# SolverForge/solverforge

Hardware: AMD Instinct MI355X
Metric: moves-evaluated/sec, CVRP-1000 (nearby-list selector, LateAcceptance(400)+AcceptedCount(256)) (higher is better)
Workload: dtype int64 score / int32 trial deltas (u16 matrix copy)

## Files before the change

### solverforge_amd/csrc/sf_api.hip

```cpp
#include <hip/hip_runtime.h>

#include <algorithm>
#include <chrono>
#include <cmath>
#include <cstddef>
#include <cstdio>
#include <cstdlib>
#include <cstring>
#include <map>
#include <string>
#include <vector>

#define SF_TU_MAIN 1
#include "../../include/solverforge_amd.h"
#include "sf_launch.h"
#include "sf_construct.hip"
#include "sf_clarke_wright.hip"
#include "sf_kopt_tw.hip"
#include "sf_precedence.hip"
#include "sf_scalar_construct.h"
#include "sf_mat_facts.h"
#include "sf_nbr_facts.h"

using namespace sf;

static std::string g_create_error;

struct Fact {
    int type = 0;
    void* d0 = nullptr;
    void* d1 = nullptr;
    int rows = 0, cols = 0;
    int64_t max_finite = 0;
    bool symmetric = false;
    bool all_finite = false;
    int64_t abs_sum = 0;
};
struct ConstraintSpec {
    int kind, desc, var, fact;
    int64_t param;
    int level;
    int64_t weight;
    std::vector<sf_pair_term> terms;
    std::vector<sf_uni_term> uterms;
    sf_uni_weight uweight{0, -1, -1, -1};
};
constexpr int SF_C_PAIR_JOIN_ = 100;
constexpr int SF_C_UNI_PROGRAM_ = 101;
struct UniComponent {
    size_t constraint_index;
    std::vector<int64_t> cost;
    std::vector<uint8_t> pass;
};
struct SelectorSpec {
    int kind, desc, var, max_nearby, fact;
    int min_size = 1, max_size = 3;
    int moves_per_step = 10, max_source_len = 0, skip_empty = 0;
    std::string variable_name;
    int value_limit = -1, recreate = 0;
    int64_t limit = -1;
};
struct NearbyScalarSource {
    bool present = false;
    std::vector<uint32_t> off;
    std::vector<int32_t> val;
    uint32_t* d_off = nullptr;
    int32_t* d_val = nullptr;
};
struct PrecSpec {
    bool on = false;
    int desc = 0, var = 0, hard_level = 0, mk_level = 1;
    std::vector<int32_t> dur, owner;
    std::vector<uint32_t> succ_off, succ;
    bool has_owner = false;
};
struct ClassSpec {
    int n_rows = 0;
    bool has_scalar = false;
    int var_index = 0, n_values = 0, allows_unassigned = 0;
    std::vector<int32_t> scalar_init;
    std::vector<uint32_t> value_off;
    std::vector<int32_t> value_list;
    bool has_list = false;
    std::vector<uint32_t> list_off, list_vals;
    int element_capacity = 0, element_bound = 0;
};

struct sf_ctx {
    int device = 0;
    hipStream_t stream = nullptr;
    int levels = 2, hard_levels = 1, R = 1;
    std::string err;
    std::map<int, ClassSpec> classes;
    std::map<int, Fact> facts;
    std::vector<ConstraintSpec> constraints;
    std::vector<SelectorSpec> selectors;
    bool initialized = false;
    bool has_list_model = false;
    int list_desc = -1;
    ListModel lm{};
    NearbyScalarSource nearby_scalar[2];
    int nearby_scalar_dynamic = 0;
    struct TwSpec {
        bool set = false, uploaded = false, force_walk = false, gate_ok = false;
        int desc = -1, n = 0;
        std::vector<int64_t> lo, hi, service, travel;
        int64_t departure = 0;
        int64_t *d_lo = nullptr, *d_hi = nullptr, *d_service = nullptr, *d_travel = nullptr;
        int32_t* d_ran = nullptr;
    } tw;
    PrecSpec prec;
    PrecModel pm{};
    bool prec_policy = false;
    PlfModel plf{};
    NbrIndex nbr{nullptr};
    NbrFacts nbr_facts{};
    ListModel lm_wave{};
    NbrIndex nbr_wave{nullptr};
    bool wave_renumbered = false;
    int32_t mat16_sym = 0;
    int last_wave_mode = -1;
    int32_t wave_spec_state = 0, wave_spec_reason = 0, wave_spec_key[23] = {};
    int n_cus = 0;
    int32_t last_generic_flags = -1;
    int32_t last_scalar_value_bytes = 0;
    int xown_level = -1;
    int64_t xown_weight = 0;
    std::vector<UniComponent> uni_components;
    uint16_t* d_xown_tab = nullptr;
    int64_t* d_xown_delta = nullptr;
    std::vector<std::pair<int, std::string>> providers;
    uint32_t* d_node_tab32 = nullptr;
    struct WaveFix {
        const uint16_t *perm, *inv, *mat16;
        const int32_t* demand;
        int32_t depot;
    } lm_wave_fix{};
    bool lm_small = false;
    int engine = SF_ENGINE_AUTO;
    bool has_scalar_model = false;
    int scalar_desc = -1;
    ScalarModel sm{};
    sf_solver_config cfg{SF_ACCEPT_LATE_ACCEPTANCE, 400, SF_FORAGER_ACCEPTED_COUNT, 256, 1, SF_ORDER_RANDOM, 0};
    SearchParams sp{};
    bool search_alloc = false;
    sf_annealing_config anneal{SF_ANNEAL_CALIBRATED, 0, 128, 0, {0, 0, 0, 0}, 0.999985, 1.0e-9, 0.80, 1.0, 0};
    bool anneal_seed_set = false;
    double dla_tolerance = 0.01;
    double gd_rain_speed = 0.001;
    uint64_t sc_step_count_limit = 100;
    uint64_t tabu_tenure[4] = {0, 0, 10, 0};
    int tabu_aspire = 1;
    bool tabu_configured = false;
    uint64_t* d_tabu_arena = nullptr;
    uint64_t tabu_arena_cap = 0;
    bool vnd = false;
    int vnd_n = -1;
    int64_t union_limit = -1;
    struct HoodTable {
        std::vector<int32_t> first, order;
        std::vector<int64_t> limit;
    } hoods_cfg, hoods;
    int vnd_leaves = -1;
    uint64_t* d_explicit = nullptr;
    int64_t n_explicit = 0;
    int32_t* d_trace_moves = nullptr;
    int64_t* d_trace_scores = nullptr;
    int32_t* d_trace_flags = nullptr;
    int64_t* d_trace_count = nullptr;
    int32_t* d_trace_applied = nullptr;
    int64_t trace_cap = 0;
    int64_t* d_each = nullptr;
    uint64_t* d_kopt_scratch = nullptr;
    uint64_t* d_ruin_rng = nullptr;
    uint64_t* d_sruin_rng = nullptr;
    int32_t* d_sruin_table = nullptr;
    uint32_t* d_mixed_ring = nullptr;
    uint8_t* d_mixed_ringx = nullptr;
    int32_t* d_mixed_ringd = nullptr;
    int union_order = -1;
    std::vector<int32_t> union_weights;
    int64_t* d_scores_out = nullptr;
    int32_t* d_ok = nullptr;
    std::vector<std::pair<hipEvent_t, hipEvent_t>> events;
    double prof_ms = 0;
    int64_t prof_launches = 0;
    std::vector<void*> allocs;
    void* rccl = nullptr;
};

static constexpr size_t SF_LDS_BUDGET = 160 * 1024 - 1024;

#define HIPCHK(ctx, expr)                                                                   \
    do {                                                                                    \
        hipError_t _e = (expr);                                                             \
        if (_e != hipSuccess) {                                                             \
            (ctx)->err = std::string(#expr) + ": " + hipGetErrorString(_e);                 \
            return SF_ERR_HIP;                                                              \
        }                                                                                   \
    } while (0)

struct DeviceGuard {
    int prev = -1;
    bool switched = false;
    explicit DeviceGuard(const sf_ctx* ctx) {
        if (!ctx) return;
        if (hipGetDevice(&prev) != hipSuccess) prev = -1;
        if (prev != ctx->device) switched = hipSetDevice(ctx->device) == hipSuccess;
    }
    ~DeviceGuard() {
        if (switched && prev >= 0) (void)hipSetDevice(prev);
    }
    DeviceGuard(const DeviceGuard&) = delete;
    DeviceGuard& operator=(const DeviceGuard&) = delete;
};

static int fail(sf_ctx* ctx, int code, const std::string& msg) {
    if (ctx) ctx->err = msg;
    return code;
}

template <class T>
static int dalloc(sf_ctx* ctx, T** out, size_t n) {
    void* p = nullptr;
    HIPCHK(ctx, hipMalloc(&p, n * sizeof(T) + 16));
    ctx->allocs.push_back(p);
    HIPCHK(ctx, hipMemsetAsync(p, 0, n * sizeof(T) + 16, ctx->stream));
    *out = (T*)p;
    return SF_OK;
}
template <class T>
static int upload(sf_ctx* ctx, T** out, const T* src, size_t n) {
    int rc = dalloc(ctx, out, n ? n : 1);
    if (rc) return rc;
    if (n) HIPCHK(ctx, hipMemcpyAsync(*out, src, n * sizeof(T), hipMemcpyHostToDevice, ctx->stream));
    HIPCHK(ctx, hipStreamSynchronize(ctx->stream));
    return SF_OK;
}

static int hip_rc(sf_ctx* ctx, hipError_t e) { return e == hipSuccess ? SF_OK : fail(ctx, SF_ERR_HIP, hipGetErrorString(e)); }

template <class T>
struct Scratch {
    T* p = nullptr;
    Scratch() = default;
    Scratch(const Scratch&) = delete;
    Scratch& operator=(const Scratch&) = delete;
    ~Scratch() { (void)hipFree(p); }
    int alloc(sf_ctx* ctx, size_t n) {
        return hip_rc(ctx, hipMalloc((void**)&p, (n ? n : 1) * sizeof(T)));
    }
    int upload(sf_ctx* ctx, const T* src, size_t n) {
        if (int rc = alloc(ctx, n)) return rc;
        return n ? hip_rc(ctx, hipMemcpyAsync(p, src, n * sizeof(T), hipMemcpyHostToDevice, ctx->stream)) : SF_OK;
    }
};

extern "C" {

int32_t sf_device_count(void) {
    int n = 0;
    if (hipGetDeviceCount(&n) != hipSuccess) return 0;
    return n;
}

int32_t sf_ctx_create(int32_t device_id, int32_t score_levels, int32_t hard_levels, int32_t n_replicas,
                      sf_ctx** out) {
    if (!out) return SF_ERR_INVALID;
    *out = nullptr;
    if (score_levels < 1 || score_levels > SF_MAX_LEVELS || hard_levels < 0 || hard_levels > score_levels ||
        n_replicas < 1) {
        g_create_error = "invalid score levels / replica count";
        return SF_ERR_INVALID;
    }
    int n = 0;
// ... 553 lines not shown
        for (auto& cs : ctx->constraints)
            if (cs.kind == SF_C_ROUTE_CAPACITY && cs.desc == d && ctx->facts[cs.fact].rows < m.dim) return false;
        return true;
    };
    for (auto& s : ctx->selectors)
        if ((s.kind == SF_SEL_NEARBY_LIST_CHANGE || s.kind == SF_SEL_NEARBY_LIST_SWAP) && s.desc == d) {
            if (!ctx->facts.count(s.fact) || ctx->facts[s.fact].type != 1) return fail(ctx, SF_ERR_INVALID, "nearby selector needs an i64 matrix meter");
            Fact& f = ctx->facts[s.fact];
            if (f.max_finite >= MAX_PACKED_DISTANCE) return fail(ctx, SF_ERR_UNSUPPORTED, "matrix values >= 2^40 (packed top-k keys)");
            if (m.mat && m.mat != (const int64_t*)f.d0) return fail(ctx, SF_ERR_UNSUPPORTED, "meter matrix must be the distance matrix");
            if (!m.mat) {
                m.mat = (const int64_t*)f.d0;
                m.dim = f.rows;
            }
            if (s.max_nearby < 1 || s.max_nearby > 64) return fail(ctx, SF_ERR_UNSUPPORTED, "max_nearby must be 1..64");
        }
    if (m.dim > 65535 * 16) return fail(ctx, SF_ERR_UNSUPPORTED, "node id bound too large");
    if (!demand_rows_ok()) return fail(ctx, SF_ERR_INVALID, "demand column shorter than the distance matrix (every matrix node needs a demand row)");
    const int R = ctx->R;
    int rc;
    if ((rc = dalloc(ctx, &m.visits, (size_t)R * m.n_cap))) return rc;
    if ((rc = dalloc(ctx, &m.off, (size_t)R * (m.V + 1)))) return rc;
    if ((rc = dalloc(ctx, &m.load, (size_t)R * m.V))) return rc;
    if ((rc = dalloc(ctx, &m.score, (size_t)R * 4))) return rc;
    if ((rc = dalloc(ctx, &m.best_visits, (size_t)R * m.n_cap))) return rc;
    if ((rc = dalloc(ctx, &m.best_off, (size_t)R * (m.V + 1)))) return rc;
    if ((rc = dalloc(ctx, &m.best_score, (size_t)R * 4))) return rc;
    HIPCHK(ctx, hipMemcpyAsync(m.visits, c.list_vals.data(), c.list_vals.size() * 4, hipMemcpyHostToDevice, ctx->stream));
    HIPCHK(ctx, hipMemcpyAsync(m.off, c.list_off.data(), c.list_off.size() * 4, hipMemcpyHostToDevice, ctx->stream));
    for (size_t k = 1; k < (size_t)R; k *= 2) {
        const size_t nrep = std::min(k, (size_t)R - k);
        HIPCHK(ctx, hipMemcpyAsync(m.visits + k * m.n_cap, m.visits, nrep * m.n_cap * 4, hipMemcpyDeviceToDevice, ctx->stream));
        HIPCHK(ctx, hipMemcpyAsync(m.off + k * (m.V + 1), m.off, nrep * (m.V + 1) * 4, hipMemcpyDeviceToDevice, ctx->stream));
    }
    HIPCHK(ctx, hipStreamSynchronize(ctx->stream));
    ctx->has_list_model = true;
    ctx->list_desc = d;
    ctx->pm = PrecModel{};
    if (ctx->prec.on) {
        PrecSpec& ps = ctx->prec;
        if (ps.desc != d) return fail(ctx, SF_ERR_INVALID, "list precedence: descriptor is not the list class");
        const int n = (int)ps.dur.size();
        if (c.element_bound > n) return fail(ctx, SF_ERR_INVALID, "list precedence: element ids must be < node_count");
        std::vector<char> seen((size_t)n, 0);
        for (uint32_t x : c.list_vals) {
            if (seen[x]) return fail(ctx, SF_ERR_UNSUPPORTED, "list precedence: an element appears in more than one list position");
            seen[x] = 1;
        }
        for (auto& sel : ctx->selectors)
            if (sel.kind == SF_SEL_LIST_RUIN && (m.dist_level >= 0 || m.cap_level >= 0))
                return fail(ctx, SF_ERR_UNSUPPORTED, "list ruin leaf on a precedence model with distance / capacity constraints");
        PrecModel& pm = ctx->pm;
        pm.on = 1;
        pm.hard_level = ps.hard_level;
        pm.mk_level = ps.mk_level;
        pm.n = n;
        std::vector<uint32_t> soff((size_t)n + 1, 0), sval, poff((size_t)n + 1, 0), pval;
        std::vector<int32_t> indeg((size_t)n, 0);
        int64_t invalid = 0;
        for (int i = 0; i < n; ++i) {
            for (uint32_t t = ps.succ_off[i]; t < ps.succ_off[i + 1]; ++t) {
                const uint32_t to = ps.succ[t];
                if (to < (uint32_t)n) {
                    sval.push_back(to);
                    indeg[to] += 1;
                } else
                    ++invalid;
            }
            soff[i + 1] = (uint32_t)sval.size();
        }
        pm.const_penalty = invalid;
        pm.n_edges = (int32_t)sval.size();
        {
            for (int i = 0; i < n; ++i) poff[(size_t)i + 1] = poff[(size_t)i] + (uint32_t)indeg[(size_t)i];
            pval.resize(sval.size());
            std::vector<uint32_t> fill(poff.begin(), poff.end() - 1);
            for (int i = 0; i < n; ++i)
                for (uint32_t t = soff[(size_t)i]; t < soff[(size_t)i + 1]; ++t) pval[fill[sval[t]]++] = (uint32_t)i;
        }
        int32_t* d_dur = nullptr;
        uint32_t *d_soff = nullptr, *d_sval = nullptr;
        int32_t *d_indeg = nullptr, *d_owner = nullptr;
        if ((rc = upload(ctx, &d_dur, ps.dur.data(), (size_t)n))) return rc;
        if ((rc = upload(ctx, &d_soff, soff.data(), soff.size()))) return rc;
        if ((rc = upload(ctx, &d_sval, sval.data(), sval.size()))) return rc;
        if ((rc = upload(ctx, &d_indeg, indeg.data(), (size_t)n))) return rc;
        if (ps.has_owner && (rc = upload(ctx, &d_owner, ps.owner.data(), (size_t)n))) return rc;
        pm.dur = d_dur;
        pm.succ_off = d_soff;
        pm.succ = d_sval;
        pm.indeg0 = d_indeg;
        pm.owner = ps.has_owner ? d_owner : nullptr;
        {
            if (n >= 0xFFFFFF) return fail(ctx, SF_ERR_UNSUPPORTED, "list precedence: node ids are 24 bits in the node records");
            std::vector<uint32_t> nd((size_t)n * 2);
            for (int i = 0; i < n; ++i) {
                const uint32_t dg = soff[(size_t)i + 1] - soff[(size_t)i];
                nd[(size_t)i * 2] = (uint32_t)ps.dur[(size_t)i];
                nd[(size_t)i * 2 + 1] = ((dg < 255u ? dg : 255u) << 24) | (dg ? sval[soff[(size_t)i]] : 0xFFFFFFu);
            }
            uint32_t* d_nd = nullptr;
            if ((rc = upload(ctx, &d_nd, nd.data(), nd.size()))) return rc;
            pm.nd = d_nd;
        }
        const size_t words = (size_t)R * (n ? n : 1);
        if ((rc = dalloc(ctx, &pm.earliest, words))) return rc;
        if ((rc = dalloc(ctx, &pm.indeg, words))) return rc;
        if ((rc = dalloc(ctx, &pm.queue, words))) return rc;
        if ((rc = dalloc(ctx, &pm.lsucc, words))) return rc;
        if ((rc = dalloc(ctx, &pm.state, (size_t)R * 2))) return rc;
        uint32_t *d_poff = nullptr, *d_pval = nullptr;
        if ((rc = upload(ctx, &d_poff, poff.data(), poff.size()))) return rc;
        if ((rc = upload(ctx, &d_pval, pval.data(), pval.size()))) return rc;
        pm.pred_off = d_poff;
        pm.pred = d_pval;
        if ((rc = dalloc(ctx, &pm.lpred, words))) return rc;
        if ((rc = dalloc(ctx, &pm.stamp_e, words))) return rc;
        if ((rc = dalloc(ctx, &pm.stamp_q, words))) return rc;
        if ((rc = dalloc(ctx, &pm.changed, words))) return rc;
        if ((rc = dalloc(ctx, &pm.queue2, words))) return rc;
        if ((rc = dalloc(ctx, &pm.pos, words))) return rc;
        if ((rc = dalloc(ctx, &pm.rnd, words))) return rc;
        if ((rc = dalloc(ctx, &pm.rec, words * 16))) return rc;
        if ((rc = dalloc(ctx, &pm.roff, words + (size_t)R))) return rc;
        if ((rc = dalloc(ctx, &pm.pmax, words + (size_t)R))) return rc;
        pm.has_zero_duration = 0;
        {
            int64_t dsum = 0;
            for (int32_t dv : ps.dur) {
                if (dv <= 0) pm.has_zero_duration = 1;
                dsum += dv > 0 ? dv : 0;
            }
            if (dsum >= ((int64_t)1 << 27)) pm.has_zero_duration = 1;
        }
    }
    for (auto& kv : ctx->facts)
        if (kv.second.type == 1 && kv.second.d0 == (void*)m.mat && kv.second.max_finite < 0xFFFFFFFFLL) {
            uint32_t* m32 = nullptr;
            const size_t n = (size_t)m.dim * m.dim;
            if ((rc = dalloc(ctx, &m32, n))) return rc;
            hipLaunchKernelGGL(k_mat_compress, dim3(1024), dim3(256), 0, ctx->stream, m.mat, n, m32);
            HIPCHK(ctx, hipGetLastError());
            m.mat32 = m32;
            static const bool no16 = std::getenv("SF_AMD_NO_MAT16") != nullptr;
            if (kv.second.max_finite < 0xFFFF && !no16) {
                uint16_t* m16 = nullptr;
                if ((rc = dalloc(ctx, &m16, n))) return rc;
                hipLaunchKernelGGL(k_mat_compress16, dim3(1024), dim3(256), 0, ctx->stream, m.mat, n, m16);
                HIPCHK(ctx, hipGetLastError());
                m.mat16 = m16;
            }
        }
    ctx->mat16_sym = 0;
    if (m.mat16 && (size_t)m.dim * m.dim * 2 <= ((size_t)64 << 20)) {
        std::vector<uint16_t> h16((size_t)m.dim * m.dim);
        HIPCHK(ctx, hipMemcpyAsync(h16.data(), m.mat16, h16.size() * 2, hipMemcpyDeviceToHost, ctx->stream));
        HIPCHK(ctx, hipStreamSynchronize(ctx->stream));
        ctx->mat16_sym = mat16_symmetric(h16.data(), m.dim);
    }
    for (auto& kv : ctx->facts)
        if (kv.second.type == 1 && kv.second.d0 == (void*)m.mat) {
            m.mat_symmetric = kv.second.symmetric ? 1 : 0;
            m.leg16 = (kv.second.symmetric && m.mat32 && m.dist_level >= 0 && kv.second.max_finite < 0xFFFF && m.dim <= 65535) ? 1 : 0;
            const bool no16 = std::getenv("SF_AMD_NO_LEG16") != nullptr;
            if (no16) m.leg16 = 0;
        }
    {
        const int64_t lim = (int64_t)1 << 28;
        auto mag = [](int64_t v) { return v < 0 ? (v == INT64_MIN ? INT64_MAX : -v) : v; };
        bool ok = m.mat32 != nullptr && m.dist_level >= 0;
        int64_t max_leg = 0, dem = 0;
        for (auto& kv : ctx->facts) {
            if (kv.second.type == 1 && kv.second.d0 == (void*)m.mat) {
                ok = ok && kv.second.all_finite && kv.second.max_finite < ((int64_t)1 << 26);
                max_leg = kv.second.max_finite;
            }
            if (kv.second.type == 2 && kv.second.d0 == (void*)m.demand) dem = kv.second.abs_sum;
        }
        ok = ok && mag(m.dist_weight) < lim && mag(m.dist_weight) * 8 * (max_leg + 1) < ((int64_t)1 << 29);
        if (m.cap_level >= 0)
            ok = ok && dem < lim && mag(m.capacity) < lim && mag(m.cap_weight) < lim &&
                 mag(m.cap_weight) * 2 * (dem + mag(m.capacity) + 1) < ((int64_t)1 << 29);
        {
            static const bool off = std::getenv("SF_AMD_NO_SMALL") != nullptr;
            if (off) ok = false;
        }
        ctx->lm_small = ok;
        m.small32 = ok ? 1 : 0;
    }
    bool nearby = false;
    for (auto& s : ctx->selectors)
        if ((s.kind == SF_SEL_NEARBY_LIST_CHANGE || s.kind == SF_SEL_NEARBY_LIST_SWAP) && s.desc == d) nearby = true;
    int P = 2;
    while (P < m.dim) P <<= 1;
    if (nearby && m.mat && (size_t)P * 8 <= 128 * 1024) {
        uint16_t* keys = nullptr;
        if ((rc = dalloc(ctx, &keys, (size_t)m.dim * m.dim))) return rc;
        HIPCHK(ctx, hipFuncSetAttribute((const void*)k_nbr_presort, hipFuncAttributeMaxDynamicSharedMemorySize, P * 8));
        hipLaunchKernelGGL(k_nbr_presort, dim3(m.dim), dim3(256), (size_t)P * 8, ctx->stream, m.mat, m.dim, P, keys);
        HIPCHK(ctx, hipGetLastError());
        HIPCHK(ctx, hipStreamSynchronize(ctx->stream));
        ctx->nbr = NbrIndex{keys};
        NbrFacts nf{0, 1};
        const int64_t rows_per = std::max<int64_t>(1, ((int64_t)4 << 20) / m.dim);
        std::vector<uint16_t> part((size_t)std::min<int64_t>(rows_per, m.dim) * m.dim);
        for (int64_t r0 = 0; r0 < m.dim; r0 += rows_per) {
            const int64_t n = std::min<int64_t>(rows_per, m.dim - r0);
            HIPCHK(ctx, hipMemcpyAsync(part.data(), keys + (size_t)r0 * m.dim, (size_t)n * m.dim * 2, hipMemcpyDeviceToHost, ctx->stream));
            HIPCHK(ctx, hipStreamSynchronize(ctx->stream));
            nbr_facts_rows(part.data(), n, m.dim, nf);
        }
        ctx->nbr_facts = nf;
    }
    ctx->wave_renumbered = false;
    {
        const char* env = std::getenv("SF_AMD_RENUMBER");
        const bool want = env ? std::atoi(env) != 0 : (size_t)m.dim * m.dim * 2 > (size_t)1024 * 1024;
        if (want && ctx->nbr.keys && m.mat16 && ctx->lm_small && m.dim <= 0x7FFF && m.depot >= 0 && m.depot < m.dim) {
            const int dim = m.dim;
            std::vector<uint16_t> hk((size_t)dim * dim);
            HIPCHK(ctx, hipMemcpyAsync(hk.data(), ctx->nbr.keys, hk.size() * 2, hipMemcpyDeviceToHost, ctx->stream));
            HIPCHK(ctx, hipStreamSynchronize(ctx->stream));
            std::vector<uint16_t> perm((size_t)dim), inv((size_t)dim);
            std::vector<uint8_t> seen((size_t)dim, 0);
            std::vector<int> ptr((size_t)dim, 0);
            int cur = m.depot, low = 0;
            for (int n = 0; n < dim; ++n) {
                perm[(size_t)cur] = (uint16_t)n;
                inv[(size_t)n] = (uint16_t)cur;
                seen[(size_t)cur] = 1;
                if (n + 1 == dim) break;
                int nx = -1;
                const uint16_t* row = hk.data() + (size_t)cur * dim;
                for (int& t = ptr[(size_t)cur]; t < dim; ++t) {
                    const uint32_t e = row[t];
                    if (e == 0xFFFFu) break;
                    if (!seen[e & 0x7FFFu]) {
                        nx = (int)(e & 0x7FFFu);
                        break;
                    }
                }
                if (nx < 0) {
                    while (seen[(size_t)low]) ++low;
                    nx = low;
                }
                cur = nx;
            }
            uint16_t *d_perm = nullptr, *d_inv = nullptr, *d_m16 = nullptr, *d_keys = nullptr;
            int32_t* d_dem = nullptr;
            if ((rc = upload(ctx, &d_perm, perm.data(), perm.size()))) return rc;
            if ((rc = upload(ctx, &d_inv, inv.data(), inv.size()))) return rc;
            if ((rc = dalloc(ctx, &d_m16, (size_t)dim * dim))) return rc;
            if ((rc = dalloc(ctx, &d_keys, (size_t)dim * dim))) return rc;
            hipLaunchKernelGGL(k_mat16_renumber, dim3(dim), dim3(256), 0, ctx->stream, m.mat16, d_inv, dim, d_m16);
            hipLaunchKernelGGL(k_nbr_renumber, dim3(dim), dim3(256), 0, ctx->stream, ctx->nbr.keys, d_inv, d_perm, dim, d_keys);
            if (m.demand) {
                if ((rc = dalloc(ctx, &d_dem, (size_t)dim))) return rc;
                hipLaunchKernelGGL(k_i32_renumber, dim3((dim + 255) / 256), dim3(256), 0, ctx->stream, m.demand, d_inv, dim, d_dem);
            }
            HIPCHK(ctx, hipGetLastError());
            HIPCHK(ctx, hipStreamSynchronize(ctx->stream));
            ctx->lm_wave_fix = {d_perm, d_inv, d_m16, d_dem, (int32_t)perm[(size_t)m.depot]};
            ctx->nbr_wave = NbrIndex{d_keys};
            ctx->wave_renumbered = true;
        }
    }
    return SF_OK;
}

#include "sf_wave_plan.h"
#include "sf_wave_spec.h"

static WaveShape wave_shape(const sf_ctx* ctx) {
    WaveShape s{};
    const ListModel& m = ctx->lm;
    s.nbr_index = ctx->nbr.keys != nullptr, s.V = m.V, s.n_cap = m.n_cap, s.dim = m.dim, s.max_nearby = 1;
    for (auto& sel : ctx->selectors)
        if (sel.desc == ctx->list_desc && (sel.kind == SF_SEL_NEARBY_LIST_CHANGE || sel.kind == SF_SEL_NEARBY_LIST_SWAP) && sel.max_nearby > s.max_nearby)
            s.max_nearby = sel.max_nearby;
    s.levels = ctx->levels, s.mat32 = m.mat32 != nullptr, s.mat16 = m.mat16 != nullptr, s.small = ctx->lm_small, s.dist_level = m.dist_level;
    return s;
}
static bool wave_engine_possible(sf_ctx* ctx) { return wave_engine_fits(wave_shape(ctx)); }
static bool use_wave_engine(sf_ctx* ctx) {
    if (ctx->engine == SF_ENGINE_BLOCK) return false;
    if (ctx->engine == SF_ENGINE_WAVE) return true;
    return wave_engine_default(wave_shape(ctx));
}

static int build_scalar_model(sf_ctx* ctx, int d);
static size_t scalar_table_bytes(sf_ctx* ctx);
static int launch_scalar_search(sf_ctx* ctx, SearchParams& p, int grid, bool trace);

static int alloc_search(sf_ctx* ctx) {
    if (ctx->search_alloc) return SF_OK;
    SearchParams& p = ctx->sp;
    const int R = ctx->R;
    int rc;
    int la = ctx->cfg.late_acceptance_size > 0 ? ctx->cfg.late_acceptance_size : 1;
    if ((rc = dalloc(ctx, &p.last_step_score, (size_t)R * 4))) return rc;
    if ((rc = dalloc(ctx, &p.la_hist, (size_t)R * la * 4))) return rc;
    if ((rc = dalloc(ctx, &p.la_idx, (size_t)R))) return rc;
    if ((rc = dalloc(ctx, &p.step_index, (size_t)R))) return rc;
    if ((rc = dalloc(ctx, &p.seed_draws, (size_t)R))) return rc;
    if ((rc = dalloc(ctx, &p.stats, (size_t)R * SF_STATS_WORDS))) return rc;
    if ((rc = dalloc(ctx, &p.has_best, (size_t)R))) return rc;
    if ((rc = dalloc(ctx, &ctx->d_trace_count, 1))) return rc;
    if ((rc = dalloc(ctx, &ctx->d_trace_applied, 8))) return rc;
    if ((rc = dalloc(ctx, &ctx->d_ok, 4))) return rc;
    if ((rc = dalloc(ctx, &p.sa.state, (size_t)R * SA_WORDS))) return rc;
    if ((rc = dalloc(ctx, &p.dla_best, (size_t)R * 4))) return rc;
    p.la_size = la;
    ctx->search_alloc = true;
    return SF_OK;
}

static int ensure_trace(sf_ctx* ctx, int64_t cap) {
    if (cap <= ctx->trace_cap) return SF_OK;
    int rc;
    if ((rc = dalloc(ctx, &ctx->d_trace_moves, (size_t)cap * 6))) return rc;
    if ((rc = dalloc(ctx, &ctx->d_trace_scores, (size_t)cap * 4))) return rc;
    if ((rc = dalloc(ctx, &ctx->d_trace_flags, (size_t)cap))) return rc;
    ctx->trace_cap = cap;
    return SF_OK;
}

static int search_kind(const sf_ctx* ctx) { return ctx->vnd ? (int)VND_KIND : ctx->cfg.acceptor; }

static void fill_search_params(sf_ctx* ctx, SearchParams& p) {
    p.acceptor = ctx->cfg.acceptor;
    p.dla_tolerance = ctx->dla_tolerance;
    p.forager = ctx->cfg.forager;
    p.limit = ctx->cfg.accepted_count_limit > 0 ? ctx->cfg.accepted_count_limit : 1;
    if (ctx->cfg.forager == SF_FORAGER_FIRST_LAST_STEP_SCORE_IMPROVING && ctx->cfg.accepted_count_limit <= 0) p.limit = 0;
    p.random_ties = ctx->cfg.random_ties;
    p.order = ctx->cfg.selection_order;
    if (ctx->vnd) {
        p.acceptor = VND_KIND;
        p.forager = SF_FORAGER_BEST_SCORE;
        p.limit = 1;
        p.random_ties = 0;
        p.order = SF_ORDER_ORIGINAL;
    }
    p.random_seed = ctx->cfg.random_seed;
    p.dry_run = 0;
    {
        static const bool legacy = std::getenv("SF_AMD_LEGACY_EVAL") != nullptr;
        p.legacy_eval = legacy ? 1 : 0;
    }
    p.replica_base = 0;
    p.explicit_seeds = ctx->d_explicit;
    p.n_explicit = ctx->n_explicit;
    p.trace_replica = -1;
    p.trace_moves = ctx->d_trace_moves;
    p.trace_scores = ctx->d_trace_scores;
    p.trace_flags = ctx->d_trace_flags;
    p.trace_cap = ctx->trace_cap;
    p.trace_count = ctx->d_trace_count;
    p.trace_applied = ctx->d_trace_applied;
}

static int fill_list_leaves(sf_ctx* ctx, SearchParams& p) {
    p.n_leaves = 0;
    for (int kind : {SF_SEL_NEARBY_LIST_CHANGE, SF_SEL_NEARBY_LIST_SWAP})
        for (auto& s : ctx->selectors)
            if (s.kind == kind && s.desc == ctx->list_desc) {
                if (p.n_leaves >= MAX_LEAVES) return fail(ctx, SF_ERR_UNSUPPORTED, "more than two list leaves");
                p.leaf[p.n_leaves++] = LeafSpec{s.kind, s.max_nearby, s.desc};
            }
    if (p.n_leaves == 0) return fail(ctx, SF_ERR_INVALID, "no list selector configured");
    return SF_OK;
}

static SearchLaunch make_launch(sf_ctx* ctx, const SearchParams* p, int grid, int block, size_t lds, const GLeaves* gl = nullptr) {
    return SearchLaunch{grid, block, lds, ctx->stream, &ctx->lm, &ctx->sm, gl, p, ctx->has_list_model ? 1 : 0, ctx->has_scalar_model ? 1 : 0, ctx->nbr};
}
template <int L>
static int launch_list_search_t(sf_ctx* ctx, const SearchParams& p, int grid, bool trace) {
    Carve<L> cv(ctx->lm.V, ctx->lm.n_cap, ctx->lm.dim);
    size_t lds = cv.total;
    if (lds > SF_LDS_BUDGET) return fail(ctx, SF_ERR_UNSUPPORTED, "problem does not fit the 160 KiB LDS of one CU");
    HIPCHK(ctx, launch_tu_list_block<L>(trace, make_launch(ctx, &p, grid, 1024, lds)));
    return SF_OK;
}
static int launch_list_wave(sf_ctx* ctx, const SearchParams& p, int n_replicas, bool trace) {
    WaveShape s = wave_shape(ctx);
    s.acceptor = p.acceptor, s.forager = p.forager, s.order = p.order, s.dry_run = p.dry_run, s.n_leaves = p.n_leaves;
    for (int l = 0; l < p.n_leaves && l < MAX_LEAVES; ++l) s.kind[l] = p.leaf[l].kind;
    s.n_replicas = n_replicas, s.trace = trace;
    const WavePlan pl = plan_wave_launch(s, wave_knobs());
    if (pl.err) return fail(ctx, pl.err, pl.msg);
    if (pl.nodeg && !ctx->lm.node_tab)
        if (int rc = dalloc(ctx, &ctx->lm.node_tab, (size_t)ctx->R * ctx->lm.dim)) return rc;
    SearchParams q = p;
    q.n_launch = n_replicas;
    SearchLaunch la = make_launch(ctx, &q, pl.grid, pl.block, (size_t)pl.lds);
    ctx->last_wave_mode = pl.mode;
    if (pl.compact && ctx->wave_renumbered) {
        ctx->lm_wave = ctx->lm;
        ctx->lm_wave.perm = ctx->lm_wave_fix.perm, ctx->lm_wave.inv = ctx->lm_wave_fix.inv, ctx->lm_wave.mat16 = ctx->lm_wave_fix.mat16;
        if (ctx->lm.demand) ctx->lm_wave.demand = ctx->lm_wave_fix.demand;
        ctx->lm_wave.depot = ctx->lm_wave_fix.depot;
        la.lm = &ctx->lm_wave;
        la.nb = ctx->nbr_wave;
    }
    if (!ctx->n_cus) HIPCHK(ctx, hipDeviceGetAttribute(&ctx->n_cus, hipDeviceAttributeMultiprocessorCount, ctx->device));
    const WaveSpecGate gate{pl.mode, q.move_budget != 0, (int32_t)std::min<int64_t>(std::max<int64_t>(q.n_steps, 0), INT32_MAX), n_replicas, pl.resident, ctx->n_cus, wave_spec_knob()};
    const WaveSpecKey key = wave_spec_key(pl.levels, pl.wpe, *la.lm, q, ctx->nbr_facts, ctx->mat16_sym, wave_spec_extras());
    ctx->wave_spec_state = SF_WSPEC_AOT, ctx->wave_spec_reason = wave_spec_wanted(gate);
    std::memcpy(ctx->wave_spec_key, &key, sizeof key);
    if (ctx->wave_spec_reason == SF_WSPEC_R_NONE) {
        hipFunction_t fn = nullptr;
        if ((ctx->wave_spec_reason = wave_spec_get(key, ctx->device, la.lds, &fn)) == SF_WSPEC_R_NONE) {
            WaveArgs args{*la.lm, q, la.nb};
            size_t n_args = sizeof args;
            void* cfg[] = {HIP_LAUNCH_PARAM_BUFFER_POINTER, &args, HIP_LAUNCH_PARAM_BUFFER_SIZE, &n_args, HIP_LAUNCH_PARAM_END};
            HIPCHK(ctx, hipModuleLaunchKernel(fn, (unsigned)la.grid, 1, 1, (unsigned)la.block, 1, 1, (unsigned)la.lds, la.stream, nullptr, cfg));
            ctx->wave_spec_state = SF_WSPEC_SPECIALISED;
            return SF_OK;
        }
        ctx->wave_spec_state = SF_WSPEC_FELL_BACK;
    }
    HIPCHK(ctx, pl.levels == 2 ? launch_tu_list_wave<2>(trace, pl.mode, la) : launch_tu_list_wave<4>(trace, pl.mode, la));
    return SF_OK;
}
static int launch_list_search(sf_ctx* ctx, const SearchParams& p, int grid, bool trace) {
    if (use_wave_engine(ctx)) return launch_list_wave(ctx, p, grid, trace);
    if (p.acceptor == SF_ACCEPT_DIVERSIFIED_LATE_ACCEPTANCE) return fail(ctx, SF_ERR_UNSUPPORTED, "DiversifiedLateAcceptance: wave, scalar and generic engines only");
    if (ctx->levels <= 2) return launch_list_search_t<2>(ctx, p, grid, trace);
    return launch_list_search_t<4>(ctx, p, grid, trace);
}

static int download_scores(sf_ctx* ctx, const int64_t* d_src4, int64_t* out) {
    std::vector<int64_t> tmp((size_t)ctx->R * 4);
    HIPCHK(ctx, hipMemcpyAsync(tmp.data(), d_src4, tmp.size() * 8, hipMemcpyDeviceToHost, ctx->stream));
    HIPCHK(ctx, hipStreamSynchronize(ctx->stream));
    for (int r = 0; r < ctx->R; ++r)
        for (int k = 0; k < ctx->levels; ++k) out[(size_t)r * ctx->levels + k] = tmp[(size_t)r * 4 + k];
    return SF_OK;
}

static int run_evaluate_all(sf_ctx* ctx, int64_t* out, int commit, int64_t* d_parts = nullptr) {
    int rc;
    if (!ctx->d_scores_out && (rc = dalloc(ctx, &ctx->d_scores_out, (size_t)ctx->R * 4))) return rc;
    if (!ctx->has_list_model && !ctx->has_scalar_model) return fail(ctx, SF_ERR_INVALID, "no planning variable configured");
    if (ctx->has_list_model) {
        size_t lds = ((size_t)ctx->lm.dim + 31) / 32 * 4 + 16;
        hipLaunchKernelGGL(k_list_evaluate_all, dim3(ctx->R), dim3(256), lds, ctx->stream, ctx->lm,
                           ctx->d_scores_out, commit, d_parts);
    }
    if (ctx->has_scalar_model)
        HIPCHK(ctx, launch_with_lds(k_scalar_evaluate_all, dim3(ctx->R), dim3(256), scalar_table_bytes(ctx), ctx->stream, ctx->sm, ctx->d_scores_out, commit,
                                    ctx->has_list_model ? 1 : 0, d_parts));
    if (ctx->xown_level >= 0)
        hipLaunchKernelGGL(k_cross_owner_evaluate_all, dim3(ctx->R), dim3(256), 0, ctx->stream, ctx->lm, ctx->sm.vals, ctx->sm.n, ctx->xown_level, ctx->xown_weight,
                           ctx->d_scores_out, commit, d_parts);
    if (ctx->has_list_model && ctx->pm.on)
        hipLaunchKernelGGL(k_prec_evaluate_all, dim3(ctx->R), dim3(64), 0, ctx->stream, ctx->lm, ctx->pm, ctx->d_scores_out, commit, d_parts);
    HIPCHK(ctx, hipGetLastError());
    if (out) {
        std::vector<int64_t> tmp((size_t)ctx->R * ctx->levels);
        HIPCHK(ctx, hipMemcpyAsync(tmp.data(), ctx->d_scores_out, tmp.size() * 8, hipMemcpyDeviceToHost, ctx->stream));
        HIPCHK(ctx, hipStreamSynchronize(ctx->stream));
        std::memcpy(out, tmp.data(), tmp.size() * 8);
    } else
        HIPCHK(ctx, hipStreamSynchronize(ctx->stream));
    return SF_OK;
}

static int tw_upload(sf_ctx* ctx) {
    auto& tw = ctx->tw;
    const ListModel& m = ctx->lm;
    if (!ctx->has_list_model || tw.desc != ctx->list_desc) return fail(ctx, SF_ERR_INVALID, "time windows need the list variable's class");
    if (tw.n != m.dim) return fail(ctx, SF_ERR_INVALID, "time windows: n_nodes must equal the list variable's element id bound (the matrix dimension when a matrix is attached)");
    const size_t n = (size_t)tw.n;
    for (int64_t** p : {&tw.d_lo, &tw.d_hi, &tw.d_service, &tw.d_travel}) {
        if (!*p) continue;
        auto it = std::find(ctx->allocs.begin(), ctx->allocs.end(), (void*)*p);
        if (it != ctx->allocs.end()) ctx->allocs.erase(it);
        (void)hipFree(*p);
        *p = nullptr;
    }
    tw.uploaded = false;
    int rc;
    if (!tw.d_ran && (rc = dalloc(ctx, &tw.d_ran, 1))) return rc;
    HIPCHK(ctx, hipMemsetAsync(tw.d_ran, 0, 4, ctx->stream));
    if ((rc = upload(ctx, &tw.d_lo, tw.lo.data(), n))) return rc;
    if ((rc = upload(ctx, &tw.d_hi, tw.hi.data(), n))) return rc;
    if ((rc = upload(ctx, &tw.d_service, tw.service.data(), n))) return rc;
    if ((rc = upload(ctx, &tw.d_travel, tw.travel.data(), n * n))) return rc;
    const auto mag = [](int64_t v) { return v < 0 ? -(__int128)v : (__int128)v; };
    __int128 max_t = 0, max_s = 0, max_w = 0;
    for (int64_t v : tw.travel)
        if (v >= 0 && v != UNREACHABLE && v > max_t) max_t = v;
    for (int64_t v : tw.service)
        if (v > max_s) max_s = v;
    for (size_t i = 0; i < n; ++i) max_w = std::max(max_w, std::max(mag(tw.lo[i]), mag(tw.hi[i])));
    const __int128 bound = mag(tw.departure) + ((__int128)m.n_cap + 1) * (max_t + max_s) + max_w;
    tw.gate_ok = bound < (__int128)TW_GATE;
    tw.uploaded = true;
    std::vector<int64_t>().swap(tw.lo), std::vector<int64_t>().swap(tw.hi), std::vector<int64_t>().swap(tw.service), std::vector<int64_t>().swap(tw.travel);
    return SF_OK;
}
static TwTables tw_tables(const sf_ctx* ctx) {
    const auto& tw = ctx->tw;
    return TwTables{tw.d_lo, tw.d_hi, tw.d_service, tw.d_travel, tw.departure, (tw.gate_ok && !tw.force_walk) ? 1 : 0, tw.d_ran};
}

extern "C" {

int32_t sf_initialize(sf_ctx* ctx, int64_t* out_scores) {
    DeviceGuard _dev(ctx);
    if (!ctx) return SF_ERR_INVALID;
    if (!ctx->initialized) {
        int n_list = 0, n_scalar = 0, ld = -1, sd = -1;
        for (auto& kv : ctx->classes) {
            if (kv.second.has_list) {
                ++n_list;
                ld = kv.first;
            }
            if (kv.second.has_scalar) {
                ++n_scalar;
                sd = kv.first;
            }
        }
        if (n_list + n_scalar == 0) return fail(ctx, SF_ERR_INVALID, "no planning variable configured");
        if (n_list > 1 || n_scalar > 1)
            return fail(ctx, SF_ERR_UNSUPPORTED, "at most one list class and one scalar class per context");
        int rc;
        if (n_list && (rc = build_list_model(ctx, ld))) return rc;
        if (n_scalar && (rc = build_scalar_model(ctx, sd))) return rc;
        if (n_list && n_scalar) {
            ctx->sm.score = ctx->lm.score;
            ctx->sm.best_score = ctx->lm.best_score;
        }
        for (auto& cs : ctx->constraints) {
            if (cs.kind != SF_C_CROSS_OWNER_MATCH) continue;
            if (!n_list || !n_scalar || cs.desc != sd || (int)cs.param != ld)
                return fail(ctx, SF_ERR_INVALID, "owner match: a join of the scalar class (descriptor_index) with the list class (param) of a mixed model");
            if (ctx->xown_level >= 0) return fail(ctx, SF_ERR_UNSUPPORTED, "one join of the two planning classes per context");
            if (ctx->sm.n_values != ctx->lm.V) return fail(ctx, SF_ERR_INVALID, "owner match: the scalar variable's values must be the list owner indices (n_values == owners)");
            if (ctx->lm.dim > ctx->sm.n) return fail(ctx, SF_ERR_INVALID, "owner match: the list elements must be entity ids of the scalar class");
            if (ctx->sm.n > 65534) return fail(ctx, SF_ERR_UNSUPPORTED, "owner match: more than 65534 entities");
            ctx->xown_level = cs.level;
            ctx->xown_weight = cs.weight;
            if ((rc = dalloc(ctx, &ctx->d_xown_tab, (size_t)ctx->R * ctx->sm.n))) return rc;
        }
        if (ctx->tw.set && (rc = tw_upload(ctx))) return rc;
        ctx->initialized = true;
    }
    return run_evaluate_all(ctx, out_scores, 1);
}

int32_t sf_evaluate_all(sf_ctx* ctx, int64_t* out_scores) {
    DeviceGuard _dev(ctx);
    if (!ctx || !ctx->initialized) return fail(ctx, SF_ERR_INVALID, "sf_initialize first");
    return run_evaluate_all(ctx, out_scores, 0);
}

int32_t sf_evaluate_each(sf_ctx* ctx, int32_t replica, int64_t* out_scores, int64_t* out_match_counts) {
    DeviceGuard _dev(ctx);
// ... 776 lines not shown

int32_t sf_get_stats(sf_ctx* ctx, int32_t replica, sf_stats* out) {
    DeviceGuard _dev(ctx);
    if (!ctx || !ctx->search_alloc || !out || replica < 0 || replica >= ctx->R) return fail(ctx, SF_ERR_INVALID, "bad sf_get_stats");
    static_assert(sizeof(sf_stats) == SF_STATS_WORDS * 8, "sf_stats layout");
    HIPCHK(ctx, hipMemcpyAsync(out, ctx->sp.stats + (size_t)replica * SF_STATS_WORDS, sizeof(sf_stats), hipMemcpyDeviceToHost, ctx->stream));
    HIPCHK(ctx, hipStreamSynchronize(ctx->stream));
    return SF_OK;
}

int32_t sf_get_stats_sum(sf_ctx* ctx, sf_stats* out) {
    DeviceGuard _dev(ctx);
    if (!ctx || !ctx->search_alloc || !out) return fail(ctx, SF_ERR_INVALID, "bad sf_get_stats_sum");
    std::vector<uint64_t> all((size_t)ctx->R * SF_STATS_WORDS);
    HIPCHK(ctx, hipMemcpyAsync(all.data(), ctx->sp.stats, all.size() * 8, hipMemcpyDeviceToHost, ctx->stream));
    HIPCHK(ctx, hipStreamSynchronize(ctx->stream));
    uint64_t sum[SF_STATS_WORDS] = {0};
    for (int r = 0; r < ctx->R; ++r)
        for (int k = 0; k < SF_STATS_WORDS; ++k) sum[k] += all[(size_t)r * SF_STATS_WORDS + k];
    std::memcpy(out, sum, sizeof(sf_stats));
    return SF_OK;
}

int32_t sf_get_best_scores(sf_ctx* ctx, int64_t* out) {
    DeviceGuard _dev(ctx);
    if (!ctx || !ctx->initialized || !out) return fail(ctx, SF_ERR_INVALID, "sf_initialize first");
    return download_scores(ctx, ctx->has_list_model ? ctx->lm.best_score : ctx->sm.best_score, out);
}

int32_t sf_portfolio_migrate_local(sf_ctx* ctx, int32_t n_elite, int32_t n_replace, int32_t* out_adopted) {
    DeviceGuard _dev(ctx);
    if (!ctx || !ctx->initialized) return fail(ctx, SF_ERR_INVALID, "sf_initialize first");
    if (!ctx->search_alloc) return fail(ctx, SF_ERR_INVALID, "sf_phase_start first");
    if (!ctx->has_list_model || ctx->has_scalar_model)
        return fail(ctx, SF_ERR_UNSUPPORTED, "elite migration: list-only models (the adopted state is the list class's best solution)");
    if (ctx->vnd)
        return fail(ctx, SF_ERR_UNSUPPORTED, "elite migration: not under variable neighborhood descent");
    if (ctx->cfg.acceptor != SF_ACCEPT_HILL_CLIMBING && ctx->cfg.acceptor != SF_ACCEPT_LATE_ACCEPTANCE &&
        ctx->cfg.acceptor != SF_ACCEPT_DIVERSIFIED_LATE_ACCEPTANCE)
        return fail(ctx, SF_ERR_UNSUPPORTED, "elite migration: HillClimbing / LateAcceptance / DiversifiedLateAcceptance (an annealing replica keeps a temperature schedule, a great deluge its water level, a step count its best step score, a tabu search its memories)");
    if (n_elite < 1 || n_replace < 0 || (int64_t)n_elite + n_replace > ctx->R)
        return fail(ctx, SF_ERR_INVALID, "elite migration: n_elite >= 1, n_replace >= 0, n_elite + n_replace <= replicas");
    if (out_adopted) *out_adopted = 0;
    if (n_replace == 0) return SF_OK;
    HIPCHK(ctx, hipStreamSynchronize(ctx->stream));
    std::vector<int64_t> bs((size_t)ctx->R * ctx->levels);
    if (int rc = download_scores(ctx, ctx->lm.best_score, bs.data())) return rc;
    std::vector<int32_t> order(ctx->R), src(ctx->R);
    for (int r = 0; r < ctx->R; ++r) order[r] = src[r] = r;
    const int L = ctx->levels;
    std::stable_sort(order.begin(), order.end(), [&](int32_t a, int32_t b) {
        for (int k = 0; k < L; ++k) {
            const int64_t x = bs[(size_t)a * L + k], y = bs[(size_t)b * L + k];
            if (x != y) return x > y;
        }
        return false;
    });
    int adopted = 0;
    for (int i = 0; i < n_replace; ++i) {
        const int32_t adopter = order[(size_t)ctx->R - 1 - i], elite = order[(size_t)(i % n_elite)];
        bool same = true;
        for (int k = 0; k < L; ++k) same = same && bs[(size_t)adopter * L + k] == bs[(size_t)elite * L + k];
        if (same) continue;
        src[adopter] = elite;
        adopted += 1;
    }
    if (adopted) {
        Scratch<int32_t> d_src;
        if (int rc = d_src.upload(ctx, src.data(), (size_t)ctx->R)) return rc;
        hipLaunchKernelGGL(k_list_migrate, dim3(ctx->R), dim3(256), 0, ctx->stream, ctx->lm, ctx->sp, d_src.p);
        hipError_t e = hipGetLastError();
        if (e == hipSuccess) e = hipStreamSynchronize(ctx->stream);
        if (int rc = hip_rc(ctx, e)) return rc;
    }
    if (out_adopted) *out_adopted = adopted;
    return SF_OK;
}

int32_t sf_download_list(sf_ctx* ctx, int32_t replica, int32_t d, uint32_t* out_off, uint32_t* out_vals, int32_t best) {
    DeviceGuard _dev(ctx);
    if (!ctx || !ctx->has_list_model || d != ctx->list_desc || replica < 0 || replica >= ctx->R)
        return fail(ctx, SF_ERR_INVALID, "bad sf_download_list");
    const ListModel& m = ctx->lm;
    const uint32_t* so = (best ? m.best_off : m.off) + (size_t)replica * (m.V + 1);
    const uint32_t* sv = (best ? m.best_visits : m.visits) + (size_t)replica * m.n_cap;
    HIPCHK(ctx, hipMemcpyAsync(out_off, so, (size_t)(m.V + 1) * 4, hipMemcpyDeviceToHost, ctx->stream));
    HIPCHK(ctx, hipStreamSynchronize(ctx->stream));
    uint32_t total = out_off[m.V];
    if (total) HIPCHK(ctx, hipMemcpyAsync(out_vals, sv, (size_t)total * 4, hipMemcpyDeviceToHost, ctx->stream));
    HIPCHK(ctx, hipStreamSynchronize(ctx->stream));
    return SF_OK;
}

int32_t sf_download_scalar(sf_ctx* ctx, int32_t replica, int32_t d, int32_t var, int32_t* out, int32_t best) {
    DeviceGuard _dev(ctx);
    if (!ctx || !ctx->has_scalar_model || d != ctx->scalar_desc || replica < 0 || replica >= ctx->R)
        return fail(ctx, SF_ERR_INVALID, "bad sf_download_scalar");
    (void)var;
    const ScalarModel& m = ctx->sm;
    const int32_t* src = (best ? m.best_vals : m.vals) + (size_t)replica * m.n;
    HIPCHK(ctx, hipMemcpyAsync(out, src, (size_t)m.n * 4, hipMemcpyDeviceToHost, ctx->stream));
    HIPCHK(ctx, hipStreamSynchronize(ctx->stream));
    return SF_OK;
}

}

extern "C" int32_t sf_debug_generic_plan(const int32_t* shape, int32_t n_shape, const int32_t* knobs, int32_t n_knobs, int32_t* plan, int32_t n_plan, const char** msg) {
    constexpr size_t plan_bytes = offsetof(GenericPlan, msg);
    if (!shape || !knobs || !plan || n_shape * 4 != (int)sizeof(GenericShape) || n_knobs * 4 != (int)sizeof(GenericKnobs) || n_plan * 4 != (int)plan_bytes)
        return SF_ERR_INVALID;
    GenericShape s;
    GenericKnobs k;
    std::memcpy(&s, shape, sizeof s);
    std::memcpy(&k, knobs, sizeof k);
    if (s.n_leaves < 0 || s.n_leaves > GL) return SF_ERR_INVALID;
    const GenericPlan pl = plan_generic_launch(s, k);
    std::memcpy(plan, &pl, plan_bytes);
    if (msg) *msg = pl.msg;
    return pl.err;
}
extern "C" int32_t sf_debug_wave_plan(const int32_t* shape, int32_t n_shape, const int32_t* knobs, int32_t n_knobs, int32_t* plan, int32_t n_plan, const char** msg, int32_t* fits) {
    constexpr size_t plan_bytes = offsetof(WavePlan, msg);
    if (!shape || !knobs || !plan || n_shape * 4 != (int)sizeof(WaveShape) || n_knobs * 4 != (int)sizeof(WaveKnobs) || n_plan * 4 != (int)plan_bytes)
        return SF_ERR_INVALID;
    WaveShape s;
    WaveKnobs k;
    std::memcpy(&s, shape, sizeof s);
    std::memcpy(&k, knobs, sizeof k);
    const WavePlan pl = plan_wave_launch(s, k);
    std::memcpy(plan, &pl, plan_bytes);
    if (msg) *msg = pl.msg;
    if (fits) fits[0] = wave_engine_fits(s), fits[1] = wave_engine_default(s);
    return pl.err;
}

extern "C" int32_t sf_debug_wave_spec(const sf_ctx* ctx, int32_t* out, int32_t n_out) {
    static_assert(sizeof(WaveSpecKey) == sizeof(sf_ctx::wave_spec_key), "WaveSpecKey");
    if (!out || (n_out != 4 + SF_WSPEC_KEY_WORDS_V2 && n_out != 4 + SF_WSPEC_KEY_WORDS_V1)) return SF_ERR_INVALID;
    std::memset(out, 0, (size_t)n_out * 4);
    if (ctx) out[0] = ctx->wave_spec_state, out[1] = ctx->wave_spec_reason, std::memcpy(out + 4, ctx->wave_spec_key, (size_t)(n_out - 4) * 4);
    WaveSpecCache& c = wave_spec_cache();
    std::lock_guard<std::mutex> lock(c.mu);
    out[2] = c.compiles, out[3] = (int32_t)std::ceil(c.last_ms);
    return SF_OK;
}
extern "C" int32_t sf_debug_wave_spec_legs(const sf_ctx* ctx, int32_t* out, int32_t n_out) {
    if (!ctx || !out || n_out != 2) return SF_ERR_INVALID;
    WaveSpecKey k;
    std::memcpy(&k, ctx->wave_spec_key, sizeof k);
    out[0] = k.mat_sym, out[1] = k.index_x & SF_WSPEC_X_LEG_ALL;
    return SF_OK;
}
extern "C" int32_t sf_debug_mat_sym(const int64_t* mat, int32_t dim, int32_t* out, int32_t n_out) {
    if (!mat || !out || dim < 1 || dim > 16384 || n_out != 1) return SF_ERR_INVALID;
    std::vector<uint16_t> w((size_t)dim * dim);
    for (size_t t = 0; t < w.size(); ++t) w[t] = mat16_word(mat[t]);
    out[0] = mat16_symmetric(w.data(), dim);
    return SF_OK;
}
extern "C" int32_t sf_debug_wave_spec_leg_gate(int32_t mat_sym) { return wave_spec_leg_allowed(mat_sym != 0); }
extern "C" int32_t sf_debug_late_acceptance(sf_ctx* ctx, int32_t replica, int64_t* out, int32_t n_slots, int32_t* cursor) {
    if (!ctx || !out || !cursor || !ctx->search_alloc || replica < 0 || replica >= ctx->R || n_slots != ctx->sp.la_size) return SF_ERR_INVALID;
    DeviceGuard guard(ctx);
    HIPCHK(ctx, hipStreamSynchronize(ctx->stream));
    HIPCHK(ctx, hipMemcpy(out, ctx->sp.la_hist + (size_t)replica * n_slots * 4, (size_t)n_slots * 32, hipMemcpyDeviceToHost));
    HIPCHK(ctx, hipMemcpy(cursor, ctx->sp.la_idx + replica, 4, hipMemcpyDeviceToHost));
    return SF_OK;
}
extern "C" int32_t sf_debug_wave_spec_gate(const int32_t* gate, int32_t n_gate) {
    if (!gate || n_gate * 4 != (int)sizeof(WaveSpecGate)) return SF_ERR_INVALID;
    WaveSpecGate g;
    std::memcpy(&g, gate, sizeof g);
    return wave_spec_wanted(g);
}
extern "C" int32_t sf_debug_nbr_facts(const uint16_t* keys, int32_t rows, int32_t dim, int32_t* out, int32_t n_out) {
    if (!keys || !out || rows < 1 || dim < 1 || n_out != 2) return SF_ERR_INVALID;
    NbrFacts f{0, 1};
    nbr_facts_rows(keys, rows, dim, f);
    out[0] = f.tie_max, out[1] = f.rows_full;
    return SF_OK;
}
extern "C" int32_t sf_debug_wave_spec_index_gate(const int32_t* in, int32_t n_in) {
    if (!in || n_in != 5 || in[0] < 1 || in[1] < 1 || in[2] < 0) return SF_ERR_INVALID;
    return wave_spec_index_allowed(WaveSpecIndexGate{in[0], in[1], in[2], in[3] >= 64, in[3] >= 2, in[4] != 0});
}
extern "C" int32_t sf_debug_wave_spec_compile(const int32_t* key, int32_t n_key, const char* arch, const char* out_path, char* opts, int32_t n_opts, char* log, int32_t n_log, double* ms) {
    if (!key || (n_key * 4 != (int)sizeof(WaveSpecKey) && n_key != SF_WSPEC_KEY_WORDS_V2 && n_key != SF_WSPEC_KEY_WORDS_V1) || !arch) return SF_ERR_INVALID;
    WaveSpecKey k{};
    std::memcpy(&k, key, (size_t)n_key * 4);
    if (!wave_spec_key_ok(k)) return SF_ERR_INVALID;
    const std::string csrc = wave_spec_csrc();
    auto put = [](char* dst, int32_t n, const std::string& s) {
        if (dst && n > 0) std::snprintf(dst, (size_t)n, "%s", s.c_str());
    };
    std::string o;
    for (auto& x : wave_spec_options(k, arch, csrc, wave_spec_rtc().include_dir)) o += x + "\n";
    put(opts, n_opts, o);
    if (!out_path) return SF_WSPEC_R_NONE;
    const WaveSpecBuild b = wave_spec_compile(k, arch, csrc);
    put(log, n_log, b.log);
    if (ms) *ms = b.ms;
    if (!b.reason) {
        std::ofstream f(out_path, std::ios::binary);
        f.write(b.code.data(), (std::streamsize)b.code.size());
        if (!f) return SF_ERR_INVALID;
    }
    return b.reason;
}

extern "C" int32_t sf_debug_step_arith(int32_t what, uint32_t start, uint32_t stride, uint32_t V, const uint32_t* k, int64_t n_k, uint32_t* out) {
    if (!k || !out || n_k < 0 || V < 2 || V > 1022 || (what != 0 && what != 1)) return SF_ERR_INVALID;
    const uint32_t rc = (uint32_t)(0x100000000ull / V);
    const FastMod fm = make_fastmod(V);
    for (int64_t i = 0; i < n_k; ++i)
        out[i] = what == 0 ? perm_index_recip(start, stride, k[i], V, rc) : fastmod_u64((uint64_t)start + (uint64_t)k[i] * stride, fm);
    return SF_OK;
}

#ifdef SF_PHASE_PROFILE
extern "C" int32_t sf_debug_ruin_phases(uint64_t* out8) {
    if (hipMemcpyFromSymbol(out8, HIP_SYMBOL(sf::g_rphase), 64) != hipSuccess) return SF_ERR_HIP;
    uint64_t z[8] = {0, 0, 0, 0, 0, 0, 0, 0};
    (void)hipMemcpyToSymbol(HIP_SYMBOL(sf::g_rphase), z, 64);
    return SF_OK;
}
extern "C" int32_t sf_debug_phases(uint64_t* out8) {
    if (hipMemcpyFromSymbol(out8, HIP_SYMBOL(sf::g_phase), 64) != hipSuccess) return SF_ERR_HIP;
    unsigned long long z[8] = {0};
    (void)hipMemcpyToSymbol(HIP_SYMBOL(sf::g_phase), z, 64);
    return SF_OK;
}
#endif

#include "sf_api_scalar.inc"
#include "sf_api_moves.inc"
#include "sf_api_construct.inc"
#include "sf_api_scalar_construct.inc"
#include "sf_portfolio.inc"
#include "sf_candidate_trace.inc"
#include "sf_api_anneal_debug.inc"
#include "sf_api_acceptor_debug.inc"
#include "sf_api_tabu.inc"
#include "sf_api_vnd.inc"
```

### solverforge_amd/csrc/sf_list_wave.hip

```cpp
#pragma once
#include <hip/hip_runtime.h>
#include <stdint.h>

#include <type_traits>

#include "sf_list_model.h"

namespace sf {

constexpr uint32_t RC_MAX = 128;
constexpr uint32_t RC_SMALL = 64;
constexpr uint32_t NBR_NODE_MASK = 0x7FFFu;
constexpr uint32_t NBR_SAME_FLAG = 0x8000u;
constexpr uint32_t NBR_END = 0xFFFFu;
#ifndef SF_WPB
#define SF_WPB 4
#endif
constexpr int WPB = SF_WPB;

#ifndef SF_SPEC_V
#define SF_SPEC_V(x) (x)
#endif
#ifndef SF_SPEC_DIM
#define SF_SPEC_DIM(x) (x)
#endif
#ifndef SF_SPEC_NCAP
#define SF_SPEC_NCAP(x) (x)
#endif
#ifndef SF_SPEC_K0
#define SF_SPEC_K0(x) (x)
#endif
#ifndef SF_SPEC_K1
#define SF_SPEC_K1(x) (x)
#endif
#ifndef SF_SPEC_LA_SIZE
#define SF_SPEC_LA_SIZE(x) (x)
#endif
#ifndef SF_SPEC_LIMIT
#define SF_SPEC_LIMIT(x) (x)
#endif
#ifndef SF_SPEC_HAS_PERM
#define SF_SPEC_HAS_PERM(x) (x)
#endif
#ifndef SF_SPEC_HAS_EXPLICIT
#define SF_SPEC_HAS_EXPLICIT(x) (x)
#endif
#ifdef SF_SPEC_L
#define SF_SPEC_OWN_LANE(v) asm volatile("" : "+v"(v))
#else
#define SF_SPEC_OWN_LANE(v)
#endif
#ifdef SF_SPEC_NO_WIDE
#define SF_SPEC_WIDE_TIES(x) false
#else
#define SF_SPEC_WIDE_TIES(x) (x)
#endif
#ifdef SF_SPEC_NO_TIES
#define SF_SPEC_TIES(x) 0ULL
#else
#define SF_SPEC_TIES(x) (x)
#endif
#ifdef SF_SPEC_ROWS_FULL
#define SF_SPEC_ROW_HAVE(x) true
#define SF_SPEC_ROW_HAVEMASK(x) (~0ULL)
#else
#define SF_SPEC_ROW_HAVE(x) (x)
#define SF_SPEC_ROW_HAVEMASK(x) (x)
#endif


__device__ __forceinline__ void wave_sync() {
    __builtin_amdgcn_fence(__ATOMIC_RELEASE, "wavefront");
    __builtin_amdgcn_wave_barrier();
    __builtin_amdgcn_fence(__ATOMIC_ACQUIRE, "wavefront");
}

SF_PLAIN_KERNEL
__global__ __launch_bounds__(256) void k_nbr_presort(const int64_t* __restrict__ mat, int dim, int P,
                                                     uint16_t* __restrict__ keys) {
    extern __shared__ __attribute__((aligned(16))) unsigned char smem[];
    uint64_t* sk = (uint64_t*)smem;
    const int row = blockIdx.x;
    const int64_t* rp = mat + (size_t)row * dim;
    for (int t = threadIdx.x; t < P; t += blockDim.x) {
        uint64_t k = ~0ULL;
        if (t < dim) {
            const int64_t v = rp[t];
            if (v >= 0 && v != UNREACHABLE) k = ((uint64_t)v << 24) | (uint64_t)(uint32_t)t;
        }
        sk[t] = k;
    }
    __syncthreads();
    for (int size = 2; size <= P; size <<= 1)
        for (int stride = size >> 1; stride > 0; stride >>= 1) {
            for (int t = threadIdx.x; t < (P >> 1); t += blockDim.x) {
                const int lo = (t / stride) * 2 * stride + (t % stride);
                const int hi = lo + stride;
                const bool up = (lo & size) == 0;
                const uint64_t a = sk[lo], b = sk[hi];
                if ((a > b) == up) {
                    sk[lo] = b;
                    sk[hi] = a;
                }
            }
            __syncthreads();
        }
    for (int t = threadIdx.x; t < dim; t += blockDim.x) {
        const uint64_t k = sk[t];
        uint32_t e = NBR_END;
        if (k != ~0ULL) {
            e = (uint32_t)k & NBR_NODE_MASK;
            if (t > 0 && (sk[t - 1] >> 24) == (k >> 24)) e |= NBR_SAME_FLAG;
        }
        keys[(size_t)row * dim + t] = (uint16_t)e;
    }
}

struct WCarve {
    size_t load, off, node, ring, visits, rtab, routeat, total;
    uint32_t rc;
    __host__ __device__ WCarve(int V, int n_cap, int dim, int max_k, bool compact = false, bool node_global = false) {
        rc = max_k <= 32 ? RC_SMALL : RC_MAX;
        size_t o = 0;
        load = o;
        o = align_up(o + (compact ? sizeof(int32_t) : sizeof(int64_t)) * V, 16);
        off = o;
        o = align_up(o + (node_global ? sizeof(uint16_t) : sizeof(uint32_t)) * (V + 1), 16);
        node = o;
        o = align_up(o + (node_global ? 0 : (compact ? sizeof(uint16_t) : sizeof(uint32_t)) * dim), 16);
        ring = o;
        o = align_up(o + sizeof(uint32_t) * 2 * rc * MAX_LEAVES, 16);
        visits = o;
        o = align_up(o + sizeof(uint16_t) * n_cap, 16);
        rtab = o;
        o = align_up(o + (node_global ? 0 : sizeof(uint32_t) * V * MAX_LEAVES), 16);
        routeat = o;
        o = align_up(o + (compact ? 0 : sizeof(uint16_t) * V * MAX_LEAVES), 16);
        total = o;
    }
};

template <bool COMPACT>
struct NodeSlotT;
template <>
struct NodeSlotT<false> {
    uint32_t* p;
    __device__ __forceinline__ NodeSlotT(unsigned char* base, int, const uint16_t*, const void*, bool = false) : p((uint32_t*)base) {}
    __device__ __forceinline__ void clear(uint32_t node) const { p[node] = NODE_NONE; }
    __device__ __forceinline__ void set(uint32_t node, uint32_t route, uint32_t pos) const { p[node] = (route << 16) | pos; }
    __device__ __forceinline__ uint32_t get(uint32_t node) const { return p[node]; }
    __device__ __forceinline__ uint32_t word(uint32_t node) const { return p[node]; }
    __device__ __forceinline__ uint32_t wide(uint32_t s, uint32_t) const { return s; }
    __device__ __forceinline__ uint32_t wide_short(uint32_t s) const { return s; }
};
template <>
struct NodeSlotT<true> {
    uint16_t* p;
    const uint16_t* visits;
    const void* off;
    bool off16;
    uint32_t pb, pmax;
    __device__ __forceinline__ uint32_t off_at(uint32_t i) const { return off16 ? (uint32_t)((const uint16_t*)off)[i] : ((const uint32_t*)off)[i]; }
    __device__ __forceinline__ NodeSlotT(unsigned char* base, int V, const uint16_t* visits_, const void* off_, bool off16_ = false)
        : p((uint16_t*)base), visits(visits_), off(off_), off16(off16_) {
        uint32_t rb = 1;
        while ((1u << rb) - 1u < (uint32_t)V) ++rb;
        pb = 16u - rb;
        pmax = (1u << pb) - 1u;
    }
    __device__ __forceinline__ void clear(uint32_t node) const { p[node] = 0xFFFFu; }
    __device__ __forceinline__ void set(uint32_t node, uint32_t route, uint32_t pos) const {
        p[node] = (uint16_t)((route << pb) | (pos < pmax ? pos : pmax));
    }
    __device__ __forceinline__ uint32_t get(uint32_t node) const { return wide(p[node], node); }
    __device__ __forceinline__ uint32_t word(uint32_t node) const { return p[node]; }
    __device__ __forceinline__ uint32_t wide(uint32_t s, uint32_t node) const {
        const bool none = s == 0xFFFFu;
        const uint32_t route = s >> pb;
        uint32_t pos = s & pmax;
        if (__ballot(!none && pos == pmax) != 0ull) {
            if (!none && pos == pmax) {
                const uint32_t o = off_at(route), len = off_at(route + 1) - o;
                while (pos + 1 < len && (uint32_t)visits[o + pos] != node) ++pos;
            }
        }
        return none ? NODE_NONE : ((route << 16) | pos);
    }
    __device__ __forceinline__ uint32_t wide_short(uint32_t s) const {
        const uint32_t w = ((s >> pb) << 16) | (s & pmax);
        return s == 0xFFFFu ? NODE_NONE : w;
    }
};
__host__ __device__ inline bool node_slot_compact_ok(int V) { return V >= 1 && V <= 1022; }

struct NearbyItem {
    uint32_t w;
    uint32_t ord;
    uint32_t pay0;
    uint32_t pay1;
};

__device__ __forceinline__ NearbyItem nearby_item(bool is_change, uint32_t slot, uint32_t se, uint32_t sp,
                                                  uint32_t len, uint32_t k, const uint32_t* s_off,
                                                  const uint16_t* sb, const uint16_t* ro) {
    const bool some = slot != NODE_NONE;
    const uint32_t r2 = some ? slot >> 16 : 0u, dp = slot & 0xFFFFu;
    const uint32_t len2 = s_off[r2 + 1] - s_off[r2];
    const uint32_t rk = ro[r2];
    const uint32_t inter_ord = ORD_INTER_BASE + (uint32_t)sb[rk] + dp;
    const bool intra = r2 == se;
    const uint32_t end_pay = (r2 << 16) | len2;
    NearbyItem it;
    if (is_change) {
        const bool v0 = !intra || (dp != sp && dp != sp + 1);
        const bool v1 = dp + 1 == len2 && (!intra || len != sp + 1);
        it.w = some ? (uint32_t)v0 + (uint32_t)v1 : 0u;
        it.ord = intra ? (v0 ? dp : len) : inter_ord;
        it.pay0 = v0 ? slot : end_pay;
        it.pay1 = end_pay;
    } else {
        const bool v = intra ? dp > sp : rk > k;
        it.w = (some && v) ? 1u : 0u;
        it.ord = intra ? dp : inter_ord;
        it.pay0 = slot;
        it.pay1 = 0;
    }
    return it;
}

struct RouteTab {
    const uint32_t* rt;
    static constexpr int KEY_SHIFT = 24;
    __device__ __forceinline__ uint32_t word(uint32_t route) const { return rt[route]; }
    __device__ __forceinline__ static uint32_t rank(uint32_t w) { return w & 0xFFFFu; }
    __device__ __forceinline__ static uint32_t inter_ord(uint32_t w, uint32_t dp) { return ORD_INTER_BASE + (w >> 16) + dp; }
};
#ifdef SF_SPEC_TIE_KEY
static_assert(SF_SPEC_RB >= 1 && SF_SPEC_PB >= 1 && SF_SPEC_RB + SF_SPEC_PB <= 22, "SF_SPEC_TIE_KEY: the packed word does not fit 32 bits");
constexpr uint32_t ORD_ARITH_BASE = 1u << (SF_SPEC_RB + SF_SPEC_PB);
constexpr int ORD_ARITH_SHIFT = SF_SPEC_PB;
#else
constexpr uint32_t ORD_ARITH_BASE = 1u << 26;
constexpr int ORD_ARITH_SHIFT = 16;
#endif
struct RouteArith {
    uint32_t st, inv, V, recip;
    static constexpr int KEY_SHIFT = 28;
    __device__ __forceinline__ uint32_t word(uint32_t route) const {
        uint32_t x = route + V - st;
        x = x >= V ? x - V : x;
        const uint32_t y = x * inv;
        uint32_t rk = y - __umulhi(y, recip) * V;
        return rk >= V ? rk - V : rk;
    }
    __device__ __forceinline__ static uint32_t rank(uint32_t w) { return w; }
    __device__ __forceinline__ static uint32_t inter_ord(uint32_t w, uint32_t dp) { return ORD_ARITH_BASE + (w << ORD_ARITH_SHIFT) + dp; }
};
struct RouteRank {
    const uint32_t* rt;
    static constexpr int KEY_SHIFT = RouteArith::KEY_SHIFT;
    __device__ __forceinline__ uint32_t word(uint32_t route) const { return rt[route]; }
    __device__ __forceinline__ static uint32_t rank(uint32_t w) { return w; }
    __device__ __forceinline__ static uint32_t inter_ord(uint32_t w, uint32_t dp) { return RouteArith::inter_ord(w, dp); }
};
template <class OT, class RT>
__device__ __forceinline__ NearbyItem nearby_item_rt(bool is_change, uint32_t slot, uint32_t se, uint32_t sp,
                                                     uint32_t len, uint32_t k, const OT* s_off, const RT& rt) {
    const bool some = slot != NODE_NONE;
    const uint32_t r2 = some ? slot >> 16 : 0u, dp = slot & 0xFFFFu;
    const uint32_t len2 = s_off[r2 + 1] - s_off[r2];
    const uint32_t t = rt.word(r2);
    const uint32_t rk = RT::rank(t);
    const uint32_t inter_ord = RT::inter_ord(t, dp);
    const bool intra = r2 == se;
    const uint32_t end_pay = (r2 << 16) | len2;
    NearbyItem it;
    if (is_change) {
        const bool v0 = !intra || (dp != sp && dp != sp + 1);
        const bool v1 = dp + 1 == len2 && (!intra || len != sp + 1);
        it.w = some ? (uint32_t)v0 + (uint32_t)v1 : 0u;
        it.ord = intra ? (v0 ? dp : len) : inter_ord;
        it.pay0 = v0 ? slot : end_pay;
        it.pay1 = end_pay;
    } else {
        const bool v = intra ? dp > sp : rk > k;
        it.w = (some && v) ? 1u : 0u;
        it.ord = intra ? dp : inter_ord;
        it.pay0 = slot;
        it.pay1 = 0;
    }
    return it;
}

__device__ __forceinline__ uint32_t mbcnt64(uint64_t mask) {
    return __builtin_amdgcn_mbcnt_hi((uint32_t)(mask >> 32), __builtin_amdgcn_mbcnt_lo((uint32_t)mask, 0u));
}
#ifdef SF_SPEC_TIE_KEY
__device__ __forceinline__ int32_t tie_key_fix(uint64_t startmask, uint64_t nonstart, uint32_t ord, uint32_t wc) {
    const uint32_t q = (mbcnt64(startmask >> 1) << (SF_SPEC_RB + SF_SPEC_PB + 3)) | (ord << 2) | wc;
    uint32_t q_dn = q, q_up = q;
    int32_t fix = 0;
    uint64_t run = nonstart;
    for (uint32_t d = 1; run != 0; ++d) {
        q_dn = (uint32_t)__builtin_amdgcn_update_dpp(0, (int)q_dn, 0x130, 0xf, 0xf, true);
        q_up = (uint32_t)__builtin_amdgcn_update_dpp(0, (int)q_up, 0x138, 0xf, 0xf, true);
        fix += q_dn < q ? (int32_t)(q_dn & 3u) : 0;
        fix -= q_up > q ? (int32_t)(q_up & 3u) : 0;
        run &= nonstart << d;
    }
    return fix;
}
#endif

template <class LT, class OT, bool OWN_LANE = false>
__device__ __forceinline__ void apply_list_move_wave(const ListModel& m, uint16_t* visits, OT* off,
                                                     LT* load, int kind, uint32_t a, uint32_t i, uint32_t b,
                                                     uint32_t j, uint32_t ext = 0) {
    uint32_t lane = threadIdx.x & 63u;
    if constexpr (OWN_LANE) asm volatile("" : "+v"(lane));
    if (kind == 2) {
        const uint32_t P = off[a] + i, Q = off[b] + j;
        const uint32_t x = visits[P];
        wave_sync();
        if (P < Q) {
            for (uint32_t t0 = P; t0 < Q; t0 += 64) {
                const uint32_t t = t0 + lane;
                uint32_t nv = 0;
                if (t < Q) nv = (t + 1 < Q) ? (uint32_t)visits[t + 1] : x;
                wave_sync();
                if (t < Q) visits[t] = (uint16_t)nv;
                wave_sync();
            }
        } else if (P > Q) {
            for (uint32_t c0 = 0; c0 <= P - Q; c0 += 64) {
                const uint32_t dd = c0 + lane;
                const bool in = dd <= P - Q;
                const uint32_t t = P - (in ? dd : 0u);
                uint32_t nv = 0;
                if (in) nv = t > Q ? (uint32_t)visits[t - 1] : x;
                wave_sync();
                if (in) visits[t] = (uint16_t)nv;
                wave_sync();
            }
        }
        if (a != b) {
            for (uint32_t rr = lane; rr <= (uint32_t)SF_SPEC_V(m.V); rr += 64) {
                if (a < b && rr > a && rr <= b) off[rr] -= 1;
                if (a > b && rr > b && rr <= a) off[rr] += 1;
            }
            if (lane == 0 && m.demand) {
                const int64_t dx = (int64_t)m.demand[x];
                load[a] = (LT)wsub(load[a], dx);
                load[b] = (LT)wadd(load[b], dx);
            }
        }
    } else if (kind == 6) {
        const uint32_t za = ext & 0xFFFFu, zb = ext >> 16;
        const uint32_t PA = off[a] + i, PB = off[b] + j;
        const bool a_first = PA < PB;
        const uint32_t PX = a_first ? PA : PB, zx = a_first ? za : zb, PY = a_first ? PB : PA, zy = a_first ? zb : za;
        const uint32_t ox = a_first ? a : b, oy = a_first ? b : a;
        int64_t da = 0, db = 0;
        if (a != b && m.demand) {
            for (uint32_t t = 0; t < za; ++t) da = wadd(da, (int64_t)m.demand[visits[PA + t]]);
            for (uint32_t t = 0; t < zb; ++t) db = wadd(db, (int64_t)m.demand[visits[PB + t]]);
        }
        wave_sync();
        relocate_flat_segment(visits, PY, zy, PX, lane, 64u, [] { wave_sync(); });
        relocate_flat_segment(visits, PX + zy, zx, PY + zy, lane, 64u, [] { wave_sync(); });
        if (a != b) {
            for (uint32_t rr = lane; rr <= (uint32_t)SF_SPEC_V(m.V); rr += 64)
                if (rr > ox && rr <= oy) off[rr] = off[rr] + zy - zx;
            if (lane == 0 && m.demand) {
                load[a] = (LT)wadd(wsub(load[a], da), db);
                load[b] = (LT)wadd(wsub(load[b], db), da);
            }
        }
    } else if (kind == 5) {
        const uint32_t z = ext - i, P = off[a] + i;
        const uint32_t Q = a != b ? off[b] + j : (j <= i ? off[a] + j : off[a] + j + z);
        int64_t dsum = 0;
        if (a != b && m.demand)
            for (uint32_t t = 0; t < z; ++t) dsum = wadd(dsum, (int64_t)m.demand[visits[P + t]]);
        wave_sync();
        relocate_flat_segment(visits, P, z, Q, lane, 64u, [] { wave_sync(); });
        if (a != b) {
            for (uint32_t rr = lane; rr <= (uint32_t)SF_SPEC_V(m.V); rr += 64) {
                if (a < b && rr > a && rr <= b) off[rr] -= z;
                if (a > b && rr > b && rr <= a) off[rr] += z;
            }
            if (lane == 0 && m.demand) {
                load[a] = (LT)wsub(load[a], dsum);
                load[b] = (LT)wadd(load[b], dsum);
            }
        }
    } else if (kind == 4) {
        const uint32_t lo = off[a] + i, hi = off[a] + j;
        for (uint32_t t = lane; t < (hi - lo) / 2; t += 64) {
            const uint16_t x = visits[lo + t], y = visits[hi - 1 - t];
            visits[lo + t] = y;
            visits[hi - 1 - t] = x;
        }
    } else if (kind == 9) {
        const uint32_t base = off[a] + i, size = j - i;
        const uint32_t perm = nth_permutation_nibbles(size, ext);
        uint32_t nv = 0;
        if (lane < size) nv = visits[base + ((perm >> (4u * lane)) & 15u)];
        wave_sync();
        if (lane < size) visits[base + lane] = (uint16_t)nv;
    } else if (kind == 7) {
        const uint32_t base = off[a], c1 = i, c2 = b, c3 = j;
        const uint32_t mask = kopt_reverse_mask(ext);
        const bool rb = (mask >> 1) & 1u, rc = (mask >> 2) & 1u;
        auto reverse_range = [&](uint32_t lo, uint32_t hi) {
            for (uint32_t t = lane; t < (hi - lo) / 2; t += 64) {
                const uint16_t x = visits[base + lo + t], y = visits[base + hi - 1 - t];
                visits[base + lo + t] = y;
                visits[base + hi - 1 - t] = x;
            }
            wave_sync();
        };
        if (!kopt_swaps_segments(ext)) {
            if (rb) reverse_range(c1, c2);
            if (rc) reverse_range(c2, c3);
        } else {
            const uint32_t zc = c3 - c2;
            reverse_range(c1, c3);
            if (!rc) reverse_range(c1, c1 + zc);
            if (!rb) reverse_range(c1 + zc, c3);
        }
    } else if (kind == 3) {
        if (lane == 0) {
            const uint32_t pa = off[a] + i, pb = off[b] + j;
            const uint16_t x = visits[pa], y = visits[pb];
            visits[pa] = y;
            visits[pb] = x;
            if (a != b && m.demand) {
                const int64_t dx = (int64_t)m.demand[x], dy = (int64_t)m.demand[y];
                load[a] = (LT)wadd(wsub(load[a], dx), dy);
                load[b] = (LT)wadd(wsub(load[b], dy), dx);
            }
        }
    }
    wave_sync();
}

__device__ __forceinline__ uint32_t nearby_source_to_ring(const ListModel& m, const NbrIndex& nb, bool is_change, uint32_t se,
                                                          uint32_t sp, uint32_t len, uint32_t k, uint32_t sx,
                                                          const uint32_t* node_slot, const uint32_t* s_off, const uint16_t* sb,
                                                          const uint16_t* ro, uint32_t* rq, uint32_t RCM, uint32_t tl,
                                                          uint32_t key, uint32_t base, uint32_t need, uint32_t emitted) {
    const uint32_t lane = threadIdx.x & 63u;
    const uint64_t lanebit = 1ULL << lane;
    const uint32_t dim = (uint32_t)m.dim;
    const uint16_t* rowk = nb.keys + (size_t)sx * dim;
    const uint32_t mv0 = (se << 16) | sp;
    for (;;) {
        const bool have = key != NBR_END;
        const uint64_t havemask = __ballot(have);
        if (havemask == 0) break;
        NearbyItem it{0u, 0u, 0u, 0u};
        if (have) it = nearby_item(is_change, node_slot[key & NBR_NODE_MASK], se, sp, len, k, s_off, sb, ro);
        const uint64_t startmask = __ballot(have && (lane == 0 || !(key & NBR_SAME_FLAG)));
        const bool more = havemask == ~0ULL && base + 64 < dim;
        const uint32_t fo = 63u - (uint32_t)__clzll((unsigned long long)startmask);
        if (more && fo == 0) {
            TopK tk{~0ULL, 0u, ~0ULL};
            for (uint32_t b2 = base; b2 < dim; b2 += 64) {
                const uint32_t j2 = b2 + lane;
                const uint32_t ky = j2 < dim ? (uint32_t)rowk[j2] : NBR_END;
                NearbyItem i2{0u, 0u, 0u, 0u};
                uint64_t hk = 0;
                if (ky != NBR_END) {
                    const uint32_t y2 = ky & NBR_NODE_MASK;
                    i2 = nearby_item(is_change, node_slot[y2], se, sp, len, k, s_off, sb, ro);
                    hk = (uint64_t)m.mat[(size_t)sx * dim + y2] << 24;
                }
                if (!__ballot(ky != NBR_END)) break;
                topk_offer(tk, need, i2.w >= 1 ? (hk | i2.ord) : ~0ULL, i2.pay0);
                topk_offer(tk, need, i2.w == 2 ? (hk | (i2.ord + 1)) : ~0ULL, i2.pay1);
            }
            const uint32_t cnt = (uint32_t)__popcll(__ballot(lane < need && tk.key != ~0ULL));
            if (lane < cnt) {
                const uint32_t qi = (tl + emitted + lane) & RCM;
                rq[qi * 2] = mv0;
                rq[qi * 2 + 1] = tk.pay;
            }
            emitted += cnt;
            break;
        }
        const uint32_t nclosed = more ? fo : (uint32_t)__popcll(havemask);
        const uint64_t closedmask = nclosed >= 64 ? ~0ULL : ((1ULL << nclosed) - 1ULL);
        const bool closed = (closedmask & lanebit) != 0;
        const uint32_t wc = closed ? it.w : 0u;
        const uint64_t w1 = __ballot(wc == 1), w2 = __ballot(wc == 2);
        const uint32_t Wc = (uint32_t)__popcll(w1) + 2u * (uint32_t)__popcll(w2);
        if (Wc > 0) {
            int32_t pos = (int32_t)(mbcnt64(w1) + 2u * mbcnt64(w2));
            const uint64_t nonstart = ~startmask & closedmask;
            if (nonstart) {
                const uint32_t packed = (it.ord << 2) | wc;
                uint64_t run = nonstart;
                for (uint32_t d = 1; run != 0; ++d) {
                    const uint32_t p_dn = __shfl_down(packed, d), p_up = __shfl_up(packed, d);
                    const bool same_up = (run & lanebit) != 0;
                    const bool same_dn = ((run >> d) & lanebit) != 0;
                    if (same_dn && (p_dn >> 2) < it.ord) pos += (int32_t)(p_dn & 3u);
                    if (same_up && (p_up >> 2) > it.ord) pos -= (int32_t)(p_up & 3u);
                    run &= nonstart << d;
                }
            }
            if (wc >= 1 && (uint32_t)pos < need) {
                const uint32_t qi = (tl + emitted + (uint32_t)pos) & RCM;
                rq[qi * 2] = mv0;
                rq[qi * 2 + 1] = it.pay0;
            }
            if (wc == 2 && (uint32_t)pos + 1 < need) {
                const uint32_t qi = (tl + emitted + (uint32_t)pos + 1) & RCM;
                rq[qi * 2] = mv0;
                rq[qi * 2 + 1] = it.pay1;
            }
            const uint32_t ne = Wc < need ? Wc : need;
            emitted += ne;
            need -= ne;
        }
        if (need == 0 || !more) break;
        base += nclosed;
        const uint32_t jj = base + lane;
        key = jj < dim ? (uint32_t)rowk[jj] : NBR_END;
    }
    return emitted;
}

#ifndef SF_WAVE_SYM
#define SF_WAVE_SYM 1
#endif

#if defined(SF_PHASE_PROFILE) || defined(SF_GEN_COUNT)
#ifdef SF_GEN_COUNT
#define SF_PHASE_WORDS 10
#else
#define SF_PHASE_WORDS 8
#endif
__device__ unsigned long long g_phase[SF_PHASE_WORDS];
#endif
#ifdef SF_ISA_MARK
#define ISA_MARK(name) asm volatile("; SF_MARK " name)
#else
#define ISA_MARK(name)
#endif
#if defined(SF_PHASE_PROFILE) && !defined(SF_PHASE_PGRP)
#define PH_DECL uint64_t ph_t = clock64(), ph_acc[8] = {0, 0, 0, 0, 0, 0, 0, 0};
#define PH(i)                          \
    {                                  \
        const uint64_t _t = clock64(); \
        ph_acc[i] += _t - ph_t;        \
        ph_t = _t;                     \
    }
#define PH_DUMP \
    if (lane == 0) for (int _k = 0; _k < 8; ++_k) atomicAdd(&g_phase[_k], (unsigned long long)ph_acc[_k]);
#elif defined(SF_GEN_COUNT)
#define PH_DECL uint64_t ph_acc[SF_PHASE_WORDS] = {0, 0, 0, 0, 0, 0, 0, 0, 0, 0};
#define PH(i)
#define GC(i) ph_acc[i] += 1;
#define PH_DUMP \
    if (lane == 0) for (int _k = 0; _k < SF_PHASE_WORDS; ++_k) atomicAdd(&g_phase[_k], (unsigned long long)ph_acc[_k]);
#else
#define PH_DECL
#define PH(i)
#define PH_DUMP
#endif
#ifndef GC
#define GC(i)
#endif

__device__ __forceinline__ int32_t wave_max_i32(int32_t v) {
    const int lo = (int)0x80000000;
    v = max(v, __builtin_amdgcn_update_dpp(lo, v, 0x111, 0xf, 0xf, false));
    v = max(v, __builtin_amdgcn_update_dpp(lo, v, 0x112, 0xf, 0xf, false));
    v = max(v, __builtin_amdgcn_update_dpp(lo, v, 0x114, 0xf, 0xf, false));
    v = max(v, __builtin_amdgcn_update_dpp(lo, v, 0x118, 0xf, 0xf, false));
    v = max(v, __builtin_amdgcn_update_dpp(lo, v, 0x142, 0xa, 0xf, false));
    v = max(v, __builtin_amdgcn_update_dpp(lo, v, 0x143, 0xc, 0xf, false));
    return __builtin_amdgcn_readlane(v, 63);
}
template <int L>
__device__ __forceinline__ bool small_ge(const int32_t (&a)[L], const int32_t (&b)[L]) {
    bool ge = true;
#pragma unroll
    for (int k = L - 1; k >= 0; --k) ge = a[k] > b[k] || (a[k] == b[k] && ge);
    return ge;
}
template <int L>
__device__ __forceinline__ bool small_ge0(const int32_t (&a)[L]) {
    bool ge = true;
#pragma unroll
    for (int k = L - 1; k >= 0; --k) ge = a[k] > 0 || (a[k] == 0 && ge);
    return ge;
}
__device__ __forceinline__ int32_t clamp_i64_to_i32(int64_t v) {
    return v > 0x7FFFFFFFll ? 0x7FFFFFFF : v < -0x7FFFFFFFll - 1 ? (int32_t)0x80000000 : (int32_t)v;
}

template <int L, class LT, bool M16 = false, class OT = uint32_t>
__device__ __forceinline__ bool eval_list_move_small(const ListModel& m, const uint16_t* visits, const OT* off, const LT* load,
                                                     bool chg, uint32_t a, uint32_t i, uint32_t b, uint32_t j, int32_t (&dv)[L]) {
    const uint32_t oa = off[a], la = off[a + 1] - oa;
    const uint32_t ob = off[b], lb = off[b + 1] - ob;
    const bool intra = a == b;
    bool ok = i < la && (chg ? j <= lb : j < lb) && !(intra && (j == i || (chg && j == i + 1)));
    const bool flip = !chg && intra && i > j;
    const uint32_t i2 = ok ? (flip ? j : i) : 0u, j2 = ok ? (flip ? i : j) : 0u;
    const uint32_t la_ = ok ? la : 0u, lb_ = ok ? lb : 0u;
    const uint32_t depot = (uint32_t)m.depot;
    const uint32_t P = oa + i2, Q = ob + j2;
    const bool has_pa = i2 > 0, has_na = i2 + 1 < la_, has_q = j2 < lb_, has_pb = j2 > 0, has_nb = j2 + 1 < lb_;
    const uint32_t r_x = visits[P];
    const uint32_t x = ok ? r_x : depot;
    const uint32_t r_pa = visits[has_pa ? P - 1 : P], r_na = visits[has_na ? P + 1 : P];
    const uint32_t r_q = visits[has_q ? Q : P], r_pb = visits[has_pb ? Q - 1 : P], r_nb = visits[has_nb ? Q + 1 : P];
    const uint32_t pa = has_pa ? r_pa : depot, na = has_na ? r_na : depot;
    const uint32_t vq = has_q ? r_q : depot;
    const uint32_t pb = has_pb ? r_pb : depot, nb = has_nb ? r_nb : depot;
    ok = ok && (chg || x != vq);
    const bool adj = !chg && intra && j2 == i2 + 1;
    const bool ca = chg || adj;
    const bool src_single = la == 1, dst_empty = !intra && lb == 0;
    const uint32_t dim4 = (uint32_t)SF_SPEC_DIM(m.dim) * (M16 ? 2u : 4u);
    auto leg = [&](uint32_t f, uint32_t t) -> uint32_t {
        const uint32_t byte_off = f * dim4 + t * (M16 ? 2u : 4u);
        if (M16) return *(const uint16_t*)((const char*)m.mat16 + byte_off);
        return *(const uint32_t*)((const char*)m.mat32 + byte_off);
    };
    const uint32_t p0 = leg(pa, chg ? na : vq);
    const uint32_t p1 = leg(chg ? pb : vq, ca ? x : na);
    const uint32_t p2 = leg(ca ? x : pb, chg ? vq : (adj ? nb : x));
    const uint32_t p3 = leg(x, nb);
    const uint32_t m0 = leg(pa, x);
    const uint32_t m1 = leg(x, adj ? vq : na);
    const uint32_t m3 = leg(vq, nb);
    const uint32_t m2 = leg(adj ? vq : pb, adj ? nb : vq);
    int32_t d_cap = 0;
    if (m.cap_level >= 0) {
        const int32_t dx = m.demand[x];
        const int32_t dyq = m.demand[vq];
        const int32_t dy = chg ? 0 : dyq;
        const int32_t cap = (int32_t)m.capacity;
        const int32_t la0 = (int32_t)load[a], lb0 = (int32_t)load[b];
        const int32_t la1 = la0 - dx + dy, lb1 = lb0 - dy + dx;
        d_cap = max(la1 - cap, 0) + max(lb1 - cap, 0) - max(la0 - cap, 0) - max(lb0 - cap, 0);
        d_cap = intra ? 0 : d_cap;
    }
    const uint32_t plus = ((chg && src_single) ? 0u : p0) + p1 + p2 + (ca ? 0u : p3);
    const uint32_t minus = m0 + m1 + ((chg && dst_empty) ? 0u : m2) + (ca ? 0u : m3);
    const int32_t d_dist = (int32_t)(plus - minus);
    const int32_t cw = (int32_t)m.cap_weight, dw = (int32_t)m.dist_weight;
#pragma unroll
    for (int k = 0; k < L; ++k) {
        int32_t v = 0;
        if (k == m.cap_level) v -= cw * d_cap;
        if (k == m.dist_level) v -= dw * d_dist;
        dv[k] = ok ? v : 0;
    }
    return ok;
}

template <int L>
struct LevelWords {
    uint32_t wc[L], wd[L];
    uint32_t has_cap;
    int32_t cap, cw, dw;
    uint32_t depot;
};
template <int L, bool USED, bool KW>
__device__ __forceinline__ LevelWords<L> level_words(const ListModel& m) {
    LevelWords<L> w;
    w.cap = w.cw = w.dw = 0;
    w.depot = 0;
#ifdef SF_SPEC_MODEL_WORDS
    w.cap = SF_SPEC_CAPACITY, w.cw = SF_SPEC_CAP_WEIGHT, w.dw = SF_SPEC_DIST_WEIGHT, w.depot = SF_SPEC_DEPOT;
#pragma unroll
    for (int k = 0; k < L; ++k) w.wc[k] = k == SF_SPEC_CAP_LEVEL ? 0xFFFFFFFFu : 0u, w.wd[k] = k == SF_SPEC_DIST_LEVEL ? 0xFFFFFFFFu : 0u;
    w.has_cap = SF_SPEC_CAP_LEVEL >= 0 ? 1u : 0u;
    return w;
#endif
    if constexpr (KW) {
        auto word = [](uint32_t v) -> uint32_t {
            asm volatile("" : "+v"(v));
            return uni(v);
        };
        w.cap = (int32_t)word((uint32_t)m.capacity);
        w.cw = (int32_t)word((uint32_t)m.cap_weight);
        w.dw = (int32_t)word((uint32_t)m.dist_weight);
        w.depot = word((uint32_t)m.depot);
    }
#pragma unroll
    for (int k = 0; k < L; ++k) {
        w.wc[k] = uni(k == m.cap_level ? 0xFFFFFFFFu : 0u);
        w.wd[k] = uni(k == m.dist_level ? 0xFFFFFFFFu : 0u);
        if constexpr (USED) {
            asm volatile("" : "+s"(w.wc[k]));
            asm volatile("" : "+s"(w.wd[k]));
        }
    }
    w.has_cap = uni(m.cap_level >= 0 ? 1u : 0u);
    if constexpr (USED) asm volatile("" : "+s"(w.has_cap));
    return w;
}
template <int L, class LT, bool M16 = false, class OT = uint32_t, bool KW = false>
__device__ __forceinline__ void eval_generated_small(const ListModel& m, const LevelWords<L>& lw, const uint16_t* visits, const OT* off, const LT* load, uint32_t c,
                                                     uint32_t a, uint32_t i, uint32_t b, uint32_t j, int32_t (&dv)[L]) {
    const uint32_t oa = off[a], la = off[a + 1] - oa;
    const uint32_t ob = off[b], lb = off[b + 1] - ob;
    const uint32_t depot = KW ? lw.depot : (uint32_t)m.depot;
    const uint32_t P = oa + i, Q = ob + j;
    const uint32_t h_pa = min(i, 1u), h_na = min(la - 1u - i, 1u);
    const uint32_t h_q = min(lb - j, 1u), h_pb = min(j, 1u);
    const uint32_t h_nb = min(max(lb, j + 1u) - (j + 1u), 1u);
    const uint32_t x = visits[P];
    const uint32_t r_pa = visits[P - h_pa], r_na = visits[P + h_na];
    const uint32_t r_q = visits[Q - (1u - h_q)], r_pb = visits[Q - h_pb], r_nb = visits[Q + h_nb];
    const uint32_t pa = h_pa ? r_pa : depot, na = h_na ? r_na : depot;
    const uint32_t vq = h_q ? r_q : depot;
    const uint32_t pb = h_pb ? r_pb : depot, nb = h_nb ? r_nb : depot;
    const bool chg = c != 0;
    const bool intra = a == b;
    const bool adj = !chg && intra && j == i + 1;
    const bool ca = chg || adj;
    const uint32_t dim4 = (uint32_t)SF_SPEC_DIM(m.dim) * (M16 ? 2u : 4u);
    auto leg = [&](uint32_t f, uint32_t t) -> uint32_t {
        const uint32_t byte_off = __umul24(f, dim4) + t * (M16 ? 2u : 4u);
        if (M16) return *(const uint16_t*)((const char*)m.mat16 + byte_off);
        return *(const uint32_t*)((const char*)m.mat32 + byte_off);
    };
    const uint32_t p0 = leg(pa, chg ? na : vq);
#ifdef SF_SPEC_SYM_ROWS
    const uint32_t p1 = leg(ca ? x : na, chg ? pb : vq);
    const uint32_t p2 = leg(x, chg ? vq : (adj ? nb : pb));
#else
    const uint32_t p1 = leg(chg ? pb : vq, ca ? x : na);
    const uint32_t p2 = leg(ca ? x : pb, chg ? vq : (adj ? nb : x));
#endif
#ifdef SF_SPEC_LEG_REAIM
    const uint32_t o_m1 = __umul24(x, dim4) + (adj ? vq : na) * (M16 ? 2u : 4u);
    auto leg_at = [&](uint32_t byte_off) -> uint32_t {
        if (M16) return *(const uint16_t*)((const char*)m.mat16 + byte_off);
        return *(const uint32_t*)((const char*)m.mat32 + byte_off);
    };
    const uint32_t p3 = leg_at(ca ? o_m1 : __umul24(x, dim4) + nb * (M16 ? 2u : 4u));
    const uint32_t m0 = leg(pa, x);
    const uint32_t m1 = leg_at(o_m1);
    const uint32_t m3 = leg_at(ca ? o_m1 : __umul24(vq, dim4) + nb * (M16 ? 2u : 4u));
#else
    const uint32_t p3 = leg(x, nb);
    const uint32_t m0 = leg(pa, x);
    const uint32_t m1 = leg(x, adj ? vq : na);
    const uint32_t m3 = leg(vq, nb);
#endif
    const uint32_t m2 = leg(adj ? vq : pb, adj ? nb : vq);
    int32_t d_cap = 0;
    if (lw.has_cap != 0u) {
        const int32_t dx = m.demand[x];
#ifdef SF_SPEC_LEG_REAIM
        const int32_t dyq = m.demand[(chg || intra) ? x : vq];
#else
        const int32_t dyq = m.demand[vq];
#endif
        const int32_t dy = chg ? 0 : dyq;
        const int32_t cap = KW ? lw.cap : (int32_t)m.capacity;
        const int32_t la0 = (int32_t)load[a] - cap, lb0 = (int32_t)load[b] - cap;
        const int32_t sh = dx - dy;
        d_cap = max(la0 - sh, 0) + max(lb0 + sh, 0) - max(la0, 0) - max(lb0, 0);
        d_cap = intra ? 0 : d_cap;
    }
    const uint32_t plus = ((chg && la == 1) ? 0u : p0) + p1 + p2 + (ca ? 0u : p3);
    const uint32_t minus = m0 + m1 + ((chg && !intra && lb == 0) ? 0u : m2) + (ca ? 0u : m3);
    const int32_t d_dist = (int32_t)(plus - minus);
    const int32_t tc = -((KW ? lw.cw : (int32_t)m.cap_weight) * d_cap), td = -((KW ? lw.dw : (int32_t)m.dist_weight) * d_dist);
#pragma unroll
    for (int k = 0; k < L; ++k) dv[k] = (int32_t)(((uint32_t)tc & lw.wc[k]) + ((uint32_t)td & lw.wd[k]));
}

struct LeafCursor {
    uint32_t head, tail;
    uint32_t left;
    uint32_t k, o;
    uint32_t se, len, sp, sx;
    uint32_t vk, vbase;
    int ex;
    uint32_t pk;
    uint32_t pv;
    uint32_t cend;
};

struct WaveArgs {
    ListModel m;
    SearchParams p;
    NbrIndex nb;
};
typedef const __attribute__((address_space(4))) WaveArgs* ColdArgs;
__device__ __forceinline__ ColdArgs cold_args() {
    uint64_t u = (uint64_t)__builtin_amdgcn_kernarg_segment_ptr();
    asm volatile("" : "+s"(u));
    return (ColdArgs)u;
}

#ifndef SF_WAVES_PER_EU
#define SF_WAVES_PER_EU 4
#endif
template <int L, bool TRACE, int MODE, bool COMPACT = false, int WPE = SF_WAVES_PER_EU, bool NODEG = false>
__global__ __launch_bounds__(64 * WPB, WPE) void k_list_search_wave(ListModel m, SearchParams p, NbrIndex nb) {
    constexpr bool FAST = MODE >= 1, SMALL = MODE == 2;
    constexpr bool LEAN = FAST && SMALL;
    constexpr bool SAT = LEAN && COMPACT, RANKTAB = LEAN && COMPACT && !NODEG;
    constexpr bool RBATCH = LEAN && !NODEG;
#define SF_COLD_P(f) (SMALL ? cold_args()->p.f : p.f)
#define SF_COLD_M(f) (SMALL ? cold_args()->m.f : m.f)
    static_assert(!COMPACT || SMALL, "COMPACT stores loads in 32 bits: MODE 2 only");
    static_assert(!NODEG || COMPACT, "NODEG: the 16-bit table of the COMPACT layout");
    using LT = typename std::conditional<COMPACT, int32_t, int64_t>::type;
    using OT = typename std::conditional<NODEG, uint16_t, uint32_t>::type;
    extern __shared__ __attribute__((aligned(16))) unsigned char smem[];
    const uint32_t lane = threadIdx.x & 63u;
    const uint32_t wave_in_group = uni(threadIdx.x >> 6);
    const int rr = (int)(blockIdx.x * (blockDim.x >> 6) + wave_in_group);
    if (rr >= p.n_launch) return;
    const int r = rr + p.replica_base;
    const int V = SF_SPEC_V(m.V);
    const uint32_t dim = (uint32_t)SF_SPEC_DIM(m.dim);

    const int n_leaves = FAST ? 2 : p.n_leaves;
    const uint32_t K0 = (uint32_t)SF_SPEC_K0(p.leaf[0].max_nearby), K1 = n_leaves > 1 ? (uint32_t)SF_SPEC_K1(p.leaf[1].max_nearby) : 1u;
    const bool chg0 = FAST ? true : p.leaf[0].kind == 16, chg1 = FAST ? false : (n_leaves > 1 && p.leaf[1].kind == 16);
    const int acceptor = FAST ? 1 : p.acceptor, forager = FAST ? 0 : p.forager;
    const bool dry_run = FAST ? false : p.dry_run != 0;
    __shared__ uint64_t s_sa[FAST ? 1 : WPB][FAST ? 1 : SA_WORDS];
    uint64_t* saw = s_sa[FAST ? 0 : wave_in_group];
    const bool annealing = !FAST && acceptor == 3;
    if constexpr (!FAST)
        if (annealing) sa_load(saw, p.sa, r, lane);
    const int32_t desc0_w = p.leaf[0].descriptor, desc1_w = n_leaves > 1 ? p.leaf[1].descriptor : 0;
    const uint64_t desc0_q = SMALL ? 0 : (uint64_t)p.leaf[0].descriptor, desc1_q = (!SMALL && n_leaves > 1) ? (uint64_t)p.leaf[1].descriptor : 0;
    auto desc0 = [&]() -> uint64_t { return SMALL ? (uint64_t)(int64_t)desc0_w : desc0_q; };
    auto desc1 = [&]() -> uint64_t { return SMALL ? (uint64_t)(int64_t)desc1_w : desc1_q; };

    const WCarve cv(V, SF_SPEC_NCAP(m.n_cap), (int)dim, (int)(K0 > K1 ? K0 : K1), COMPACT, NODEG);
    const uint32_t RCM = cv.rc - 1;
    unsigned char* mem = smem + (size_t)wave_in_group * cv.total;
    LT* s_load = (LT*)(mem + cv.load);
    OT* s_off = (OT*)(mem + cv.off);
    uint32_t* ring = (uint32_t*)(mem + cv.ring);
    uint16_t* s_visits = (uint16_t*)(mem + cv.visits);
    const NodeSlotT<COMPACT> node_slot(NODEG ? (unsigned char*)(m.node_tab + (size_t)r * dim) : mem + cv.node, V, s_visits, (const void*)s_off, NODEG);
    auto node_sync = [&]() {
        if constexpr (NODEG) {
            __builtin_amdgcn_fence(__ATOMIC_RELEASE, "workgroup");
            __builtin_amdgcn_wave_barrier();
            __builtin_amdgcn_fence(__ATOMIC_ACQUIRE, "workgroup");
        } else {
            wave_sync();
        }
    };
    constexpr bool ARANK = NODEG;
    using RT = typename std::conditional<ARANK, RouteArith, typename std::conditional<RANKTAB, RouteRank, RouteTab>::type>::type;
    uint32_t* rtab = (uint32_t*)(mem + cv.rtab);
    uint16_t* route_at = (uint16_t*)(mem + cv.routeat);

    uint32_t* g_visits = m.visits + (size_t)r * SF_SPEC_NCAP(m.n_cap);
    uint32_t* g_off = m.off + (size_t)r * (V + 1);
    int64_t* g_load = m.load + (size_t)r * V;
    int64_t* g_score = m.score + (size_t)r * 4;
    const bool tracing = TRACE && r == p.trace_replica;

    for (uint32_t t = lane; t <= (uint32_t)V; t += 64) s_off[t] = (OT)g_off[t];
    for (uint32_t t = lane; t < (uint32_t)V; t += 64) s_load[t] = (LT)g_load[t];
    for (uint32_t t = lane; t < dim; t += 64) node_slot.clear(t);
    node_sync();
    const uint32_t total0 = uni(s_off[V]);
    if (COMPACT && SF_SPEC_HAS_PERM(m.perm != nullptr)) {
        for (uint32_t t = lane; t < total0; t += 64) s_visits[t] = m.perm[g_visits[t]];
    } else {
        for (uint32_t t = lane; t < total0; t += 64) s_visits[t] = (uint16_t)g_visits[t];
    }
    wave_sync();
    for (uint32_t v = lane; v < (uint32_t)V; v += 64) {
        const uint32_t o = s_off[v], len = s_off[v + 1] - o;
        for (uint32_t q = 0; q < len; ++q) node_slot.set(s_visits[o + q], v, q);
    }
    node_sync();

    uint32_t nsat = 0;
    if constexpr (SAT) {
        for (uint32_t base = 0; base < (uint32_t)V; base += 64) {
            const uint32_t v = base + lane;
            const bool lg = v < (uint32_t)V && (uint32_t)(s_off[v + 1] - s_off[v]) > node_slot.pmax;
            nsat += (uint32_t)__popcll(__ballot(lg));
        }
    }
    auto ext_id = [&](uint32_t x) -> uint32_t { return (COMPACT && SF_SPEC_HAS_PERM(m.inv != nullptr)) ? (uint32_t)m.inv[x] : x; };
    int64_t cur[L], best_sol[L];
#pragma unroll
    for (int k = 0; k < L; ++k) {
        cur[k] = (int64_t)uni64((uint64_t)g_score[k]);
        best_sol[k] = (int64_t)uni64((uint64_t)m.best_score[(size_t)r * 4 + k]);
    }
    uint32_t st_steps = 0, st_gen = 0, st_acc = 0, st_applied = 0, st_calc = 0, st_scored = 0, st_sources = 0;
    uint64_t steps_run = 0;
    auto flush_stats = [&]() {
        if (lane == 0) {
            uint64_t* gs = SF_COLD_P(stats) + (size_t)r * SF_STATS_WORDS;
            gs[0] += st_steps;
            gs[1] += st_gen;
            gs[2] += st_gen;
            gs[3] += st_acc;
            gs[4] += st_applied;
            gs[5] += st_calc;
            gs[6] += st_gen - st_calc;
            gs[7] += st_scored;
            gs[8] += st_sources;
        }
        if constexpr (!SMALL) steps_run += st_steps;
        st_steps = st_gen = st_acc = st_applied = st_calc = st_scored = st_sources = 0;
    };
    uint64_t trace_n = 0;
    const uint64_t step_index0 = dry_run ? 0 : p.step_index[r];
    const uint64_t seed_draws0 = dry_run ? 0 : p.seed_draws[r];
    const int la_idx0 = dry_run ? 0 : p.la_idx[r];
    int la_cursor = la_idx0;
    const uint64_t lanebit = 1ULL << lane;
    uint32_t hm = 0;
    if constexpr (LEAN) {
        hm = (uint32_t)((int32_t)(lane << 26) >> 31);
        asm volatile("" : "+v"(hm));
    }
    auto half = [&](uint32_t lo, uint32_t up) -> uint32_t { return (lo & ~hm) | (up & hm); };
    PH_DECL

    const LevelWords<L> lvl = level_words<L, SMALL, RBATCH>(m);
    bool best_pending = false;
    const FastMod fm_V = make_fastmod(V > 0 ? (uint32_t)V : 1u);
    const FastMod fm_V1 = make_fastmod(V > 1 ? (uint32_t)V - 1u : 1u);
    const uint32_t v_recip32 = V > 1 ? (uint32_t)(0x100000000ull / (uint32_t)V) : 0u;
    const bool use_cm = V >= 2 && V <= 128;
    const uint64_t cm_lo = use_cm ? __ballot(lane >= 1 && lane < (uint32_t)V && gcd_u32(lane, (uint32_t)V) == 1) : 0ull;
    const uint64_t cm_hi = use_cm ? __ballot(lane + 64 < (uint32_t)V && gcd_u32(lane + 64, (uint32_t)V) == 1) : 0ull;
    int64_t step = 0;
    for (; step < SF_COLD_P(n_steps); ++step) {
        PH(7)
        ISA_MARK("prologue_begin");
        uint64_t sidx, sseed;
        if (dry_run) {
            sidx = p.dry_step_index;
            sseed = p.dry_step_seed;
        } else {
            sidx = step_index0 + (uint64_t)step;
            const uint64_t draw = seed_draws0 + (uint64_t)step;
            const uint64_t* const explicit_seeds = SF_COLD_P(explicit_seeds);
            const int64_t n_explicit = SF_COLD_P(n_explicit);
            if (SF_SPEC_HAS_EXPLICIT(explicit_seeds != nullptr) && (int64_t)draw < n_explicit)
                sseed = explicit_seeds[(size_t)r * n_explicit + draw];
            else
                sseed = step_seed(SF_COLD_P(random_seed) + (uint64_t)r, draw);
        }
        sidx = uni64(sidx);
        sseed = uni64(sseed);
        const StreamCtx ctx{sidx, sseed, FAST ? 3 : p.order};
        ScoreV<L> late;
#pragma unroll
        for (int k = 0; k < L; ++k) late.v[k] = 0;
        const int la_slot = la_cursor;
        if (acceptor == 1 || acceptor == 4) {
            const int64_t* const lh = SF_COLD_P(la_hist) + ((size_t)r * SF_SPEC_LA_SIZE(SF_COLD_P(la_size)) + la_slot) * 4;
#pragma unroll
            for (int k = 0; k < L; ++k) late.v[k] = (int64_t)uni64((uint64_t)lh[k]);
        }
        ScoreV<L> dla_thr = late;
        if (acceptor == 4) {
            ScoreV<L> db;
#pragma unroll
            for (int k = 0; k < L; ++k) db.v[k] = (int64_t)uni64((uint64_t)p.dla_best[(size_t)r * 4 + k]);
            dla_thr = dla_threshold<L>(db, p.dla_tolerance);
        }
        [[maybe_unused]] bool thr_on = true;
        if constexpr (TRACE)
            if (acceptor == 5 || acceptor == 6) ax_step_begin<L>(acceptor, p.sa.state + (size_t)r * SA_WORDS, late, thr_on);
        [[maybe_unused]] TabuStep<L> tabu;
        [[maybe_unused]] const TabuScope tabu_scope{0u, 0u, 0u};
        if constexpr (TRACE)
            if (acceptor == 7) tabu_step_begin<L>(p.sa.state + (size_t)r * SA_WORDS, tabu);
        int has_best = 0;
        typename std::conditional<SMALL, uint32_t, uint64_t>::type equal_count = 0;
        uint32_t accepted = 0, pulls = 0;
        ScoreV<L> best;
#pragma unroll
        for (int k = 0; k < L; ++k) best.v[k] = 0;
        uint32_t best_m0 = 0, best_m1 = 0;
        int best_leaf = 0;
        uint64_t best_ti = 0;
        int32_t late_d[L], best_d[L];
#pragma unroll
        for (int k = 0; k < L; ++k) {
            late_d[k] = SMALL ? clamp_i64_to_i32(wsub(late.v[k], cur[k])) : 0;
            best_d[k] = 0;
        }
        int64_t acc_thr = 0, best_key = 0;
        if constexpr (SMALL && L == 2) {
            const int64_t lh = late_d[0] < -(1 << 30) ? -(int64_t)(1 << 30) : (int64_t)late_d[0];
            const int64_t late_key = lh * 4294967296ll + (int64_t)late_d[1];
            acc_thr = late_key < 0 ? late_key : 0;
        }
        const uint32_t total = uni(s_off[V]);
        uint32_t hashed = 0;
        const bool lane_hash = FAST && use_cm;
        if (lane_hash) {
            const uint64_t es0 = SALT_NEARBY_CHANGE_ENTITY ^ desc0(), es1 = SALT_NEARBY_SWAP_ENTITY ^ desc1();
            if constexpr (RBATCH && SF_WAVE_SYM != 0) {
                uint32_t hl = lane;
                asm volatile("" : "+v"(hl));
                const uint64_t salt = hl == 0 ? SALT_UNION_OFFSET : hl == 1 ? es0 : hl == 2 ? (es0 ^ STRIDE_SALT_MIX) : hl == 3 ? es1 : (es1 ^ STRIDE_SALT_MIX);
                const FastMod fm2 = make_fastmod(2u);
                FastMod f;
                f.M = hl == 0 ? fm2.M : ((hl & 1u) ? fm_V.M : fm_V1.M);
                f.n = hl == 0 ? fm2.n : ((hl & 1u) ? fm_V.n : fm_V1.n);
                hashed = fastmod_u64(ctx.mixed_seed(salt), f);
            } else {
                const uint64_t salt = lane == 0 ? SALT_UNION_OFFSET : lane == 1 ? es0 : lane == 2 ? (es0 ^ STRIDE_SALT_MIX) : lane == 3 ? es1 : (es1 ^ STRIDE_SALT_MIX);
                const FastMod fm2 = make_fastmod(2u);
                FastMod f;
                f.M = lane == 0 ? fm2.M : ((lane & 1u) ? fm_V.M : fm_V1.M);
                f.n = lane == 0 ? fm2.n : ((lane & 1u) ? fm_V.n : fm_V1.n);
                hashed = fastmod_u64(ctx.mixed_seed(salt), f);
            }
        }
        const uint32_t first_leaf = lane_hash ? (uint32_t)__builtin_amdgcn_readlane((int)hashed, 0)
                                              : (n_leaves > 1 ? ctx.random_index((uint32_t)n_leaves, SALT_UNION_OFFSET) : 0u);

        uint32_t perm_st0 = 0, perm_sd0 = 1, perm_st1 = 0, perm_sd1 = 1;
        uint32_t perm_inv0 = 0, perm_inv1 = 0;
        auto route_facts = [&](int l) -> RT {
            if constexpr (ARANK)
                return RouteArith{l ? perm_st1 : perm_st0, l ? perm_inv1 : perm_inv0, (uint32_t)V, v_recip32};
            else
                return RT{rtab + l * V};
        };
        auto resolve = [&](LeafCursor& c, int l) {
            const uint16_t* ra = route_at + l * V;
            uint32_t k = c.k, o = c.o, se = c.se, len = c.len;
            if (o >= c.cend) {
            ISA_MARK("resolve_slow_begin");
            if (k != c.vk || o >= len) {
                for (;;) {
                    if constexpr (COMPACT) {
                        const uint32_t xx = (l ? perm_st1 : perm_st0) + k * (l ? perm_sd1 : perm_sd0);
                        uint32_t rr_ = xx - __umulhi(xx, v_recip32) * (uint32_t)V;
                        rr_ = rr_ >= (uint32_t)V ? rr_ - (uint32_t)V : rr_;
                        se = uni(rr_);
                    } else
                        se = uni((uint32_t)ra[k]);
                    len = uni(s_off[se + 1] - s_off[se]);
                    if (o < len) break;
                    ++k;
                    o = 0;
                }
            }
            if (k != c.vk || (o & ~63u) != c.vbase) {
                const uint64_t src_salt = ((l ? chg1 : chg0) ? SALT_NEARBY_CHANGE_SOURCE : SALT_NEARBY_SWAP_SOURCE) ^
                                          (uint64_t)se ^ (l ? desc1() : desc0());
                const uint32_t oo = (o & ~63u) + lane;
                const uint32_t spl = oo < len ? ctx.selection_index(oo, len, src_salt) : 0u;
                const uint32_t sxl = oo < len ? (uint32_t)s_visits[s_off[se] + spl] : 0u;
                c.pv = spl | (sxl << 16);
                c.vk = k;
                c.vbase = o & ~63u;
            }
            c.cend = len < (o & ~63u) + 64u ? len : (o & ~63u) + 64u;
            c.k = k;
            c.se = se;
            c.len = len;
            ISA_MARK("resolve_slow_end");
            }
            const uint32_t pvv = (uint32_t)__builtin_amdgcn_readlane((int)c.pv, (int)(o & 63u));
            const uint32_t sp = pvv & 0xFFFFu, sx = pvv >> 16;
            c.o = o;
            c.sp = sp;
            c.sx = sx;
            const uint32_t ent = l ? ((lane + 32u) & 63u) : lane;
            const uint32_t entc = ent < dim ? ent : dim - 1u;
            const uint32_t pk_any = (uint32_t) * (const uint16_t*)((const char*)nb.keys + ((sx * dim + entc) << 1));
            if constexpr (LEAN)
                c.pk = pk_any;
            else
                c.pk = ent < dim ? pk_any : NBR_END;
        };
        auto row_key = [&](uint32_t raw, uint32_t e) -> uint32_t { return LEAN ? (e < dim ? raw : NBR_END) : raw; };

        PH(0)
        LeafCursor C0{0, 0, total, 0, 0, 0, 0, 0, 0, 0xFFFFFFFFu, 0, 0, NBR_END, 0, 0};
        LeafCursor C1{0, 0, n_leaves > 1 ? total : 0u, 0, 0, 0, 0, 0, 0, 0xFFFFFFFFu, 0, n_leaves > 1 ? 0 : 1, NBR_END, 0, 0};
        for (int l = 0; l < n_leaves; ++l) {
            const uint64_t ent_salt = ((l ? chg1 : chg0) ? SALT_NEARBY_CHANGE_ENTITY : SALT_NEARBY_SWAP_ENTITY) ^ (l ? desc1() : desc0());
            uint32_t pst, psd;
            if (lane_hash) {
                pst = (uint32_t)__builtin_amdgcn_readlane((int)hashed, l ? 3 : 1);
                psd = StreamCtx::first_coprime_from((uint32_t)__builtin_amdgcn_readlane((int)hashed, l ? 4 : 2) + 1u, cm_lo, cm_hi);
            } else if (use_cm)
                ctx.perm_params_fm(fm_V, fm_V1, ent_salt, pst, psd, cm_lo, cm_hi);
            else
                ctx.perm_params((uint32_t)V, ent_salt, pst, psd);
            pst = uni(pst);
            psd = uni(psd);
            if (l)
                perm_st1 = pst, perm_sd1 = psd;
            else
                perm_st0 = pst, perm_sd0 = psd;
            if constexpr (ARANK) {
                uint32_t inv = 0;
                for (uint32_t base = 0; base < (uint32_t)V; base += 64) {
                    const uint32_t c = base + lane;
                    const uint32_t xx = psd * c;
                    uint32_t rm = xx - __umulhi(xx, v_recip32) * (uint32_t)V;
                    rm = rm >= (uint32_t)V ? rm - (uint32_t)V : rm;
                    const uint64_t hit = __ballot(c < (uint32_t)V && rm == 1u);
                    if (hit) {
                        inv = base + (uint32_t)__ffsll((unsigned long long)hit) - 1u;
                        break;
                    }
                }
                if (l)
                    perm_inv1 = inv;
                else
                    perm_inv0 = inv;
                continue;
            }
            uint16_t* ra = route_at + l * V;
            uint32_t* rt = rtab + l * V;
            [[maybe_unused]] uint32_t carry = 0;
            for (uint32_t base = 0; base < (uint32_t)V; base += 64) {
                const uint32_t k = base + lane;
                if constexpr (RANKTAB) {
                    if (k < (uint32_t)V) rt[perm_index_recip(pst, psd, k, (uint32_t)V, v_recip32)] = k;
                } else {
                    uint32_t v = 0, e = 0;
                    if (k < (uint32_t)V) {
                        e = fastmod_u64((uint64_t)pst + (uint64_t)k * psd, fm_V);
                        if constexpr (!COMPACT) ra[k] = (uint16_t)e;
                        v = s_off[e + 1] - s_off[e] + 1;
                    }
                    const uint32_t inc = wave_incl_scan(v);
                    if (k < (uint32_t)V) rt[e] = k | ((carry + inc - v) << 16);
                    carry += __shfl(inc, 63);
                }
            }
        }
        wave_sync();
        if constexpr (SMALL) st_sources += C0.left + C1.left;
        if (total > 0) {
            resolve(C0, 0);
            if (n_leaves > 1) resolve(C1, 1);
        }
        ISA_MARK("prologue_end");

        PH(1)
        int done = 0;
        constexpr bool SYM = RBATCH && SF_WAVE_SYM != 0;
        [[maybe_unused]] bool lockstep = SYM && K0 == K1 && K0 <= 32u && total > 0;
        while (!done) {
            PH(4)
            auto gen_rest = [&](int l, uint32_t se, uint32_t sp, uint32_t len, uint32_t k, uint32_t sx, uint32_t tl,
                                uint32_t key, uint32_t base, uint32_t need, uint32_t emitted) -> uint32_t {
                const bool is_change = l ? chg1 : chg0;
                const RT rt = route_facts(l);
                uint32_t* rq = ring + (size_t)l * cv.rc * 2;
                const uint16_t* rowk = nb.keys + (size_t)sx * dim;
                const uint32_t mv0 = (se << 16) | sp;
                for (;;) {
                    const bool have = key != NBR_END;
                    const uint64_t havemask = __ballot(have);
                    if (havemask == 0) break;
                    NearbyItem it{0u, 0u, 0u, 0u};
                    if (have) it = nearby_item_rt(is_change, node_slot.get(key & NBR_NODE_MASK), se, sp, len, k, s_off, rt);
                    const uint64_t startmask = __ballot(have && (lane == 0 || !(key & NBR_SAME_FLAG)));
                    const bool more = havemask == ~0ULL && base + 64 < dim;
                    const uint32_t fo = 63u - (uint32_t)__clzll((unsigned long long)startmask);
                    if (SF_SPEC_WIDE_TIES(more && fo == 0)) {
                        TopK tk{~0ULL, 0u, ~0ULL};
                        for (uint32_t b2 = base; b2 < dim; b2 += 64) {
                            const uint32_t j2 = b2 + lane;
                            const uint32_t ky = j2 < dim ? (uint32_t)rowk[j2] : NBR_END;
                            NearbyItem i2{0u, 0u, 0u, 0u};
                            uint64_t hk = 0;
                            if (ky != NBR_END) {
                                const uint32_t y2 = ky & NBR_NODE_MASK;
                                i2 = nearby_item_rt(is_change, node_slot.get(y2), se, sp, len, k, s_off, rt);
                                hk = (uint64_t)m.mat[(size_t)ext_id(sx) * dim + ext_id(y2)] << RT::KEY_SHIFT;
                            }
                            if (!__ballot(ky != NBR_END)) break;
                            topk_offer(tk, need, i2.w >= 1 ? (hk | i2.ord) : ~0ULL, i2.pay0);
                            topk_offer(tk, need, i2.w == 2 ? (hk | (i2.ord + 1)) : ~0ULL, i2.pay1);
                        }
                        const uint32_t cnt = (uint32_t)__popcll(__ballot(lane < need && tk.key != ~0ULL));
                        if (lane < cnt) {
                            const uint32_t qi = (tl + emitted + lane) & RCM;
                            rq[qi * 2] = mv0;
                            rq[qi * 2 + 1] = tk.pay;
                        }
                        emitted += cnt;
                        break;
                    }
                    const uint32_t nclosed = more ? fo : (uint32_t)__popcll(havemask);
                    const uint64_t closedmask = nclosed >= 64 ? ~0ULL : ((1ULL << nclosed) - 1ULL);
                    const bool closed = (closedmask & lanebit) != 0;
                    const uint32_t wc = closed ? it.w : 0u;
                    const uint64_t w1 = __ballot(wc == 1), w2 = __ballot(wc == 2);
                    const uint32_t Wc = (uint32_t)__popcll(w1) + 2u * (uint32_t)__popcll(w2);
                    GC(l ? 6 : 5)
                    if (Wc == 0) { GC(7) }
                    if (Wc > 0) {
                        int32_t pos = (int32_t)(mbcnt64(w1) + 2u * mbcnt64(w2));
                        const uint64_t nonstart = SF_SPEC_TIES(~startmask & closedmask);
#ifdef SF_SPEC_TIE_KEY
                        if (nonstart) pos += tie_key_fix(startmask, nonstart, it.ord, wc);
#else
                        if (nonstart) {
                            const uint32_t packed = (it.ord << 2) | wc;
                            uint64_t run = nonstart;
                            uint32_t p_dn = packed, p_up = packed;
                            for (uint32_t d = 1; run != 0; ++d) {
                                p_dn = (uint32_t)__builtin_amdgcn_update_dpp(0, (int)p_dn, 0x130, 0xf, 0xf, false);
                                p_up = (uint32_t)__builtin_amdgcn_update_dpp(0, (int)p_up, 0x138, 0xf, 0xf, false);
                                const bool same_up = (run & lanebit) != 0;
                                const bool same_dn = ((run >> d) & lanebit) != 0;
                                if (same_dn && (p_dn >> 2) < it.ord) pos += (int32_t)(p_dn & 3u);
                                if (same_up && (p_up >> 2) > it.ord) pos -= (int32_t)(p_up & 3u);
                                run &= nonstart << d;
                            }
                        }
#endif
                        if (wc >= 1 && (uint32_t)pos < need) {
                            const uint32_t qi = (tl + emitted + (uint32_t)pos) & RCM;
                            rq[qi * 2] = mv0;
                            rq[qi * 2 + 1] = it.pay0;
                        }
                        if (wc == 2 && (uint32_t)pos + 1 < need) {
                            const uint32_t qi = (tl + emitted + (uint32_t)pos + 1) & RCM;
                            rq[qi * 2] = mv0;
                            rq[qi * 2 + 1] = it.pay1;
                        }
                        const uint32_t ne = Wc < need ? Wc : need;
                        emitted += ne;
                        need -= ne;
                    }
                    if (need == 0 || !more) break;
                    base += nclosed;
                    const uint32_t jj = base + lane;
                    key = jj < dim ? (uint32_t)rowk[jj] : NBR_END;
                }
                return emitted;
            };
            auto slot_of = [&](uint32_t word, uint32_t node) -> uint32_t {
                if constexpr (SAT) {
                    uint32_t ns = nsat;
                    asm volatile("" : "+s"(ns));
                    if (ns != 0) return node_slot.wide(word, node);
                    return node_slot.wide_short(word);
                } else
                    return node_slot.wide(word, node);
            };
            if constexpr (SYM) {
                if (lockstep) {
                    lockstep = false;
                    uint32_t sym_h = 0, sym_t = 0, sym_left = total, tA = 0, tB = 0;
                    for (;;) {
                        ISA_MARK("sym_fill_begin");
                        bool leave = false;
                        while (sym_t - sym_h < 32u) {
                            tA = tB = sym_t;
                            if (sym_left == 0) {
                                leave = true;
                                break;
                            }
                            ISA_MARK("pair_begin");
                            GC(0)
                            GC(8)
                            uint32_t sym_left1 = sym_left;
#define SF_PAIR_TAIL0 sym_t
#define SF_PAIR_TAIL1 sym_t
#define SF_PAIR_LEFT0 sym_left
#define SF_PAIR_LEFT1 sym_left1
#include "sf_wave_pair_pass.inc"
#undef SF_PAIR_TAIL0
#undef SF_PAIR_TAIL1
#undef SF_PAIR_LEFT0
#undef SF_PAIR_LEFT1
// ... 139 lines not shown
                        if (acceptor == 0)
                            acc = score_cmp<L>(sc, curv) > 0;
                        else if (acceptor == 1)
                            acc = score_cmp<L>(sc, curv) >= 0 || score_cmp<L>(sc, late) >= 0;
                        else if (acceptor == 4)
                            acc = score_cmp<L>(sc, curv) >= 0 || score_cmp<L>(sc, late) >= 0 || score_cmp<L>(sc, dla_thr) >= 0;
                    }
                    if constexpr (TRACE)
                        if (acceptor == 5 || acceptor == 6) acc = ax_accepts<L>(doable, sc, curv, late, thr_on);
                    if constexpr (TRACE)
                        if (acceptor == 7) {
                            TabuSig sig{{TABU_NO_TOKEN, TABU_NO_TOKEN}, {TABU_NO_TOKEN, TABU_NO_TOKEN}, {0, 0}, {0, 0}};
                            if (doable) {
                                const uint32_t a = m0 >> 16, i = m0 & 0xFFFFu, b = m1 >> 16, j = m1 & 0xFFFFu;
                                const uint32_t u = ext_id(s_visits[s_off[a] + i]);
                                if (lf ? chg1 : chg0)
                                    tabu_sig_list_change(tabu_scope, a, i, b, (a == b && j > i) ? j - 1 : j, u, sig);
                                else
                                    tabu_sig_list_swap(tabu_scope, a, i, u, b, j, ext_id(s_visits[s_off[b] + j]), sig);
                            }
                            acc = tabu_accepts<L>(tabu, doable, sc, sig);
                        }
                    SaChunk sach;
                    if constexpr (!FAST)
                        if (annealing) acc = sa_decide<L>(saw, p.sa, doable, sc, curv, lane, sach);
                    accmask = __ballot(acc);
                    ScoreV<L> forager_thr = curv;
                    if (forager == FORAGER_FIRST_BEST_IMPROVING) {
    #pragma unroll
                        for (int kk = 0; kk < L; ++kk) forager_thr.v[kk] = best_sol[kk];
                    }
                    nconsumed = forager_chunk_cut<L>(forager, (uint32_t)SF_SPEC_LIMIT(p.limit), accepted, acc, sc, forager_thr, nvalid, improving_pick);
                    consumed = lane < nconsumed;
                    if constexpr (!FAST)
                        if (annealing) sa_commit<L>(saw, p.sa, sach, nconsumed, lane);
                    acc = acc && consumed;
                    accmask = __ballot(acc);
                    if (accmask) {
                        if (improving_pick) {
                            const int sel = (int)nconsumed - 1;
    #pragma unroll
                            for (int kk = 0; kk < L; ++kk) best.v[kk] = (int64_t)uni64(shfl_u64((uint64_t)sc.v[kk], sel));
                            best_m0 = __shfl(m0, sel);
                            best_m1 = __shfl(m1, sel);
                            best_leaf = (int)__shfl(lf, sel);
                            if (TRACE) best_ti = trace_n + (uint64_t)sel;
                            equal_count = 1;
                            has_best = 1;
                        } else if (forager == 1) {
                            if (!has_best) {
                                const int sel = __ffsll((unsigned long long)accmask) - 1;
    #pragma unroll
                                for (int kk = 0; kk < L; ++kk) best.v[kk] = (int64_t)uni64(shfl_u64((uint64_t)sc.v[kk], sel));
                                best_m0 = __shfl(m0, sel);
                                best_m1 = __shfl(m1, sel);
                                best_leaf = (int)__shfl(lf, sel);
                                if (TRACE) best_ti = trace_n + (uint64_t)sel;
                                has_best = 1;
                            }
                        } else if (!has_best || __ballot(acc && score_cmp<L>(sc, best) >= 0)) {
                            const ScoreV<L> M = wave_max_score<L>(sc, acc);
                            const int cm = has_best ? score_cmp<L>(M, best) : 1;
                            if (cm >= 0) {
                                const bool newmax = cm > 0;
                                const uint64_t eq_base = newmax ? 0 : equal_count;
                                const bool in_eq = acc && score_cmp<L>(sc, M) == 0;
                                const uint64_t eq = __ballot(in_eq);
                                const uint32_t rank = mbcnt64(eq) + 1u;
                                const uint64_t cntq = eq_base + rank;
                                const bool pick = in_eq && ((newmax && rank == 1) ||
                                                            (p.random_ties && cntq > 1 && reservoir_pick(sseed, cntq)));
                                const uint64_t pm = __ballot(pick);
                                if (pm) {
                                    const int sel = 63 - __clzll((unsigned long long)pm);
                                    best_m0 = __shfl(m0, sel);
                                    best_m1 = __shfl(m1, sel);
                                    best_leaf = (int)__shfl(lf, sel);
                                    if (TRACE) best_ti = trace_n + (uint64_t)sel;
                                }
    #pragma unroll
                                for (int kk = 0; kk < L; ++kk) best.v[kk] = (int64_t)uni64((uint64_t)M.v[kk]);
                                equal_count = eq_base + (uint64_t)__popcll(eq);
                                has_best = 1;
                            }
                        }
                    }
                }
                const uint32_t nacc = (uint32_t)__popcll(accmask);
                accepted += nacc;
                if constexpr (!RBATCH) st_scored += nvalid;
                if constexpr (!SMALL) {
                    st_gen += nconsumed;
                    st_acc += nacc;
                    const uint32_t ndo = (uint32_t)__popcll(__ballot(consumed && doable));
                    st_calc += ndo;
                }
                if (tracing && consumed) {
                    const uint64_t ti = trace_n + lane;
                    if ((int64_t)ti < p.trace_cap) {
                        int32_t* tm = p.trace_moves + ti * 6;
                        tm[0] = (lf ? chg1 : chg0) ? 2 : 3;
                        tm[1] = (int32_t)(m0 >> 16);
                        tm[2] = (int32_t)(m0 & 0xFFFFu);
                        tm[3] = (int32_t)(m1 >> 16);
                        tm[4] = (int32_t)(m1 & 0xFFFFu);
                        tm[5] = -1;
                        for (int kk = 0; kk < L && kk < m.levels; ++kk) p.trace_scores[ti * m.levels + kk] = doable ? sc.v[kk] : 0;
                        p.trace_flags[ti] = (doable ? 1 : 0) | (acc ? 2 : 0) | ((int32_t)lf << 8);
                    }
                }
                if (tracing) trace_n += nconsumed;
                uint32_t c1;
                if constexpr (SMALL) {
                    const uint32_t lfirst = (uint32_t)__builtin_amdgcn_readfirstlane((int)lf);
                    c1 = both ? ((nconsumed + lfirst) >> 1) : (lfirst ? nconsumed : 0u);
                } else {
                    c1 = (uint32_t)__popcll(__ballot(consumed && lf == 1u));
                }
                C1.head += c1;
                C0.head += nconsumed - c1;
                pulls += nconsumed;
                if constexpr (!RBATCH)
                    if (forager_quits(forager, (uint32_t)SF_SPEC_LIMIT(p.limit), accepted, has_best, improving_pick)) done = 1;
            }
            ISA_MARK("replay_end");
            PH(3)
        }
        PH(4)

        ISA_MARK("commit_begin");
        if constexpr (SMALL) st_sources -= C0.left + C1.left;
        if constexpr (SMALL) {
            if constexpr (L == 2) {
                const int32_t soft = (int32_t)(uint32_t)(uint64_t)best_key;
                best_d[1] = soft;
                best_d[0] = (int32_t)(uint32_t)((uint64_t)wsub(best_key, (int64_t)soft) >> 32);
            }
#pragma unroll
            for (int kk = 0; kk < L; ++kk) best.v[kk] = wadd(cur[kk], (int64_t)best_d[kk]);
        }
        const bool applied = has_best && !dry_run;
        [[maybe_unused]] TabuSig pick_sig;
        if (applied) {
            if (best_pending) {
                ScoreV<L> bs;
#pragma unroll
                for (int kk = 0; kk < L; ++kk) bs.v[kk] = best_sol[kk];
                if (!(score_cmp<L>(best, bs) > 0)) {
                    const uint32_t tot = uni(s_off[V]);
                    uint32_t* const bv = SF_COLD_M(best_visits) + (size_t)r * SF_SPEC_NCAP(SF_COLD_M(n_cap));
                    uint32_t* const bo = SF_COLD_M(best_off) + (size_t)r * (V + 1);
                    uint32_t ln = lane;
                    if constexpr (RANKTAB) asm volatile("" : "+v"(ln));
                    for (uint32_t t = ln; t < tot; t += 64) bv[t] = ext_id(s_visits[t]);
                    for (uint32_t t = ln; t <= (uint32_t)V; t += 64) bo[t] = s_off[t];
                    best_pending = false;
                }
            }
            const int kind = (best_leaf ? chg1 : chg0) ? 2 : 3;
            const uint32_t a = uni(best_m0 >> 16), i = uni(best_m0 & 0xFFFFu);
            const uint32_t b = uni(best_m1 >> 16), j = uni(best_m1 & 0xFFFFu);
            if (tracing && lane == 0) {
                p.trace_applied[0] = 1;
                if ((int64_t)best_ti < p.trace_cap) p.trace_flags[best_ti] |= 4;
                p.trace_applied[1] = kind;
                p.trace_applied[2] = (int32_t)a;
                p.trace_applied[3] = (int32_t)i;
                p.trace_applied[4] = (int32_t)b;
                p.trace_applied[5] = (int32_t)j;
                p.trace_applied[6] = -1;
            }
            if constexpr (SAT) {
                if (kind == 2 && a != b) {
                    const uint32_t la0 = uni(s_off[a + 1] - s_off[a]), lb0 = uni(s_off[b + 1] - s_off[b]);
                    nsat += (lb0 == node_slot.pmax ? 1u : 0u);
                    nsat -= (la0 == node_slot.pmax + 1u ? 1u : 0u);
                }
                nsat = uni(nsat);
            }
            if constexpr (TRACE)
                if (acceptor == 7) {
                    const uint32_t u = ext_id(s_visits[s_off[a] + i]);
                    if (kind == 2)
                        tabu_sig_list_change(tabu_scope, a, i, b, (a == b && j > i) ? j - 1 : j, u, pick_sig);
                    else
                        tabu_sig_list_swap(tabu_scope, a, i, u, b, j, ext_id(s_visits[s_off[b] + j]), pick_sig);
                }
            apply_list_move_wave<LT, OT, RANKTAB && L == 4>(m, s_visits, s_off, s_load, kind, a, i, b, j);
            {
                const uint32_t oa = s_off[a], la = s_off[a + 1] - oa;
                const uint32_t ob = s_off[b], lb = s_off[b + 1] - ob;
                for (uint32_t t = lane; t < la + (a != b ? lb : 0u); t += 64) {
                    if (t < la)
                        node_slot.set(s_visits[oa + t], a, t);
                    else
                        node_slot.set(s_visits[ob + (t - la)], b, t - la);
                }
            }
            node_sync();
#pragma unroll
            for (int kk = 0; kk < L; ++kk) cur[kk] = best.v[kk];
            st_applied += 1;
        } else if (tracing && lane == 0) {
            p.trace_applied[0] = 0;
        }
        if (!dry_run) {
            bool improved = false;
            if (applied) {
                ScoreV<L> cs, bs;
#pragma unroll
                for (int kk = 0; kk < L; ++kk) {
                    cs.v[kk] = cur[kk];
                    bs.v[kk] = best_sol[kk];
                }
                improved = score_cmp<L>(cs, bs) > 0;
            }
            if (improved) {
                best_pending = true;
#pragma unroll
                for (int kk = 0; kk < L; ++kk) best_sol[kk] = cur[kk];
            }
            const int la_size = SF_SPEC_LA_SIZE(SF_COLD_P(la_size));
            if ((acceptor == 1 || acceptor == 4) && lane == 0) {
                int64_t* const lh = SF_COLD_P(la_hist) + ((size_t)r * la_size + la_slot) * 4;
#pragma unroll
                for (int kk = 0; kk < L; ++kk) lh[kk] = cur[kk];
            }
            if (acceptor == 4 && lane == 0) {
                ScoreV<L> cs, db;
#pragma unroll
                for (int kk = 0; kk < L; ++kk) {
                    cs.v[kk] = cur[kk];
                    db.v[kk] = p.dla_best[(size_t)r * 4 + kk];
                }
                if (score_cmp<L>(cs, db) > 0) {
#pragma unroll
                    for (int kk = 0; kk < L; ++kk) p.dla_best[(size_t)r * 4 + kk] = cur[kk];
                }
            }
            if constexpr (TRACE)
                if (acceptor == 5 || acceptor == 6) ax_step_ended<L>(acceptor, lane == 0, cur, p.sa.state + (size_t)r * SA_WORDS);
            if constexpr (TRACE)
                if (acceptor == 7) tabu_step_ended<L>(p.sa.state + (size_t)r * SA_WORDS, lane == 0, cur, applied ? &pick_sig : nullptr);
            if constexpr (!FAST)
                if (annealing) sa_step_ended(saw, p.sa, lane);
            wave_sync();
            st_steps += 1;
            if constexpr (SMALL) {
                st_gen += pulls;
                st_calc += pulls;
                st_acc += accepted;
                if constexpr (RBATCH) st_scored += pulls;
            }
            la_cursor = la_cursor + 1 >= la_size ? 0 : la_cursor + 1;
            const int64_t move_budget = SF_COLD_P(move_budget);
            if (move_budget > 0 && (int64_t)st_gen >= move_budget) {
                if constexpr (SMALL) ++step;
                break;
            }
            if (move_budget == 0 && st_scored >= 0x70000000u) flush_stats();
        }
        ISA_MARK("commit_end");
        PH(5)
    }
    PH_DUMP

    if (!dry_run) {
        if constexpr (!FAST)
            if (annealing) sa_store(saw, p.sa, r, lane);
        const uint32_t tot = uni(s_off[V]);
        uint32_t wlane = lane;
        SF_SPEC_OWN_LANE(wlane);
        const size_t n_cap = (size_t)SF_SPEC_NCAP(SF_COLD_M(n_cap));
        uint32_t* const w_visits = SMALL ? SF_COLD_M(visits) + (size_t)r * n_cap : g_visits;
        uint32_t* const w_off = SMALL ? SF_COLD_M(off) + (size_t)r * (V + 1) : g_off;
        int64_t* const w_load = SMALL ? SF_COLD_M(load) + (size_t)r * V : g_load;
        int64_t* const w_score = SMALL ? SF_COLD_M(score) + (size_t)r * 4 : g_score;
        if (best_pending) {
            uint32_t* const bv = SF_COLD_M(best_visits) + (size_t)r * n_cap;
            uint32_t* const bo = SF_COLD_M(best_off) + (size_t)r * (V + 1);
            for (uint32_t t = wlane; t < tot; t += 64) bv[t] = ext_id(s_visits[t]);
            for (uint32_t t = wlane; t <= (uint32_t)V; t += 64) bo[t] = s_off[t];
        }
        for (uint32_t t = wlane; t < tot; t += 64) w_visits[t] = ext_id(s_visits[t]);
        for (uint32_t t = wlane; t <= (uint32_t)V; t += 64) w_off[t] = s_off[t];
        for (uint32_t t = wlane; t < (uint32_t)V; t += 64) w_load[t] = (int64_t)s_load[t];
        if (lane == 0) {
#pragma unroll
            for (int kk = 0; kk < L; ++kk) {
                w_score[kk] = cur[kk];
                SF_COLD_P(last_step_score)[(size_t)r * 4 + kk] = cur[kk];
                SF_COLD_M(best_score)[(size_t)r * 4 + kk] = best_sol[kk];
            }
            SF_COLD_P(la_idx)[r] = la_cursor;
            const uint64_t ran = SMALL ? (uint64_t)step : steps_run + (uint64_t)st_steps;
            SF_COLD_P(step_index)[r] = step_index0 + ran;
            SF_COLD_P(seed_draws)[r] = seed_draws0 + ran;
        }
        flush_stats();
    }
    if (tracing && lane == 0) *p.trace_count = (int64_t)trace_n;
}

#undef SF_COLD_P
#undef SF_COLD_M

template <class F>
struct wave_args_are : std::false_type {};
template <>
struct wave_args_are<void (*)(decltype(WaveArgs::m), decltype(WaveArgs::p), decltype(WaveArgs::nb))> : std::true_type {};
static_assert(wave_args_are<decltype(&k_list_search_wave<2, false, 2>)>::value && std::is_standard_layout<WaveArgs>::value,
              "WaveArgs must list k_list_search_wave's parameters, in order: cold_args() reads the kernarg segment through it");

}
```

### solverforge_amd/csrc/sf_mat_facts.h

```cpp
#pragma once
#include <stdint.h>

static inline uint16_t mat16_word(int64_t v) { return (v >= 0 && v < 0xFFFF) ? (uint16_t)v : (uint16_t)0xFFFFu; }

static inline int32_t mat16_symmetric(const uint16_t* mat, int32_t dim) {
    constexpr int32_t T = 64;
    for (int32_t a0 = 0; a0 < dim; a0 += T)
        for (int32_t b0 = a0; b0 < dim; b0 += T) {
            const int32_t a1 = a0 + T < dim ? a0 + T : dim, b1 = b0 + T < dim ? b0 + T : dim;
            for (int32_t a = a0; a < a1; ++a)
                for (int32_t b = (b0 > a + 1 ? b0 : a + 1); b < b1; ++b)
                    if (mat[(size_t)a * dim + b] != mat[(size_t)b * dim + a]) return 0;
        }
    return 1;
}
```

### solverforge_amd/csrc/sf_wave_spec.h

```cpp
#pragma once
#include <dlfcn.h>

#include "sf_nbr_facts.h"

#include <fstream>
#include <mutex>
#include <sstream>

struct WaveSpecKey {
    int32_t levels, wpe;
    int32_t V, dim, n_cap, k0, k1;
    int32_t extras;
    int32_t capacity, cap_weight, dist_weight, depot, cap_level, dist_level;
    int32_t la_size, limit, has_perm, has_explicit;
    int32_t wide_ties, ties, rows_full;
    int32_t index_x;
    int32_t mat_sym;
};
constexpr int32_t SF_WSPEC_KEY_WORDS_V2 = 22;
constexpr int32_t SF_WSPEC_KEY_WORDS_V1 = 18;
enum { SF_WSPEC_X_MODEL = 1, SF_WSPEC_X_LA = 2, SF_WSPEC_X_LIMIT = 4, SF_WSPEC_X_PERM = 8, SF_WSPEC_X_EXPLICIT = 16, SF_WSPEC_X_ALL = 31 };
enum { SF_WSPEC_X_NO_WIDE = 32, SF_WSPEC_X_TIE_KEY = 64, SF_WSPEC_X_NO_TIES = 128, SF_WSPEC_X_ROWS_FULL = 256, SF_WSPEC_X_INDEX_ALL = 480 };
enum { SF_WSPEC_X_SYM_ROWS = 512, SF_WSPEC_X_LEG_REAIM = 1024, SF_WSPEC_X_LEG_ALL = 1536 };
constexpr int32_t SF_WSPEC_X_DEFAULT = SF_WSPEC_X_MODEL | SF_WSPEC_X_LA | SF_WSPEC_X_PERM;
constexpr int32_t SF_WSPEC_X_INDEX_DEFAULT = SF_WSPEC_X_NO_WIDE | SF_WSPEC_X_TIE_KEY | SF_WSPEC_X_ROWS_FULL;
constexpr int32_t SF_WSPEC_X_LEG_DEFAULT = SF_WSPEC_X_SYM_ROWS;
static int32_t wave_spec_extras() {
    const char* e = std::getenv("SF_AMD_WAVE_SPEC_EXTRAS");
    return e ? (std::atoi(e) & (SF_WSPEC_X_ALL | SF_WSPEC_X_INDEX_ALL | SF_WSPEC_X_LEG_ALL)) : (SF_WSPEC_X_DEFAULT | SF_WSPEC_X_INDEX_DEFAULT | SF_WSPEC_X_LEG_DEFAULT);
}

struct WaveSpecIndexGate {
    int32_t V, dim, n_cap;
    int32_t wide_ties, ties, rows_full;
};
static int32_t wave_spec_bits(uint32_t v) {
    int32_t b = 1;
    while (v >> b) ++b;
    return b;
}
static int32_t wave_spec_rb(int32_t V) { return wave_spec_bits((uint32_t)(V > 1 ? V - 1 : 0)); }
static int32_t wave_spec_pb(int32_t n_cap) { return wave_spec_bits((uint32_t)(n_cap > 0 ? n_cap : 0)); }
static int32_t wave_spec_index_allowed(const WaveSpecIndexGate& g) {
    int32_t a = 0;
    if (!g.wide_ties) a |= SF_WSPEC_X_NO_WIDE;
    if (wave_spec_rb(g.V) + wave_spec_pb(g.n_cap) <= 22) a |= SF_WSPEC_X_TIE_KEY;
    if (!g.ties) a |= SF_WSPEC_X_NO_TIES;
    if (g.rows_full && g.dim >= 32) a |= SF_WSPEC_X_ROWS_FULL;
    return a;
}
static int32_t wave_spec_leg_allowed(int32_t mat_sym) { return SF_WSPEC_X_LEG_REAIM | (mat_sym ? SF_WSPEC_X_SYM_ROWS : 0); }
template <class Model, class Params>
static WaveSpecKey wave_spec_key(int32_t levels, int32_t wpe, const Model& m, const Params& q, const NbrFacts& nf, int32_t mat_sym, int32_t extras) {
    WaveSpecKey k{};
    k.levels = levels, k.wpe = wpe, k.V = m.V, k.dim = m.dim, k.n_cap = m.n_cap, k.k0 = q.leaf[0].max_nearby, k.k1 = q.leaf[1].max_nearby;
    k.wide_ties = nf.tie_max >= 64, k.ties = nf.tie_max >= 2, k.rows_full = nf.rows_full != 0;
    k.index_x = extras & SF_WSPEC_X_INDEX_ALL & wave_spec_index_allowed(WaveSpecIndexGate{k.V, k.dim, k.n_cap, k.wide_ties, k.ties, k.rows_full});
    k.mat_sym = mat_sym != 0;
    k.index_x |= extras & SF_WSPEC_X_LEG_ALL & wave_spec_leg_allowed(k.mat_sym);
    extras &= SF_WSPEC_X_ALL;
    auto fits = [](int64_t v) { return v >= INT32_MIN && v <= INT32_MAX; };
    if ((extras & SF_WSPEC_X_MODEL) && !(fits(m.capacity) && fits(m.cap_weight) && fits(m.dist_weight))) extras &= ~SF_WSPEC_X_MODEL;
    if ((m.perm != nullptr) != (m.inv != nullptr)) extras &= ~SF_WSPEC_X_PERM;
    k.extras = extras;
    if (extras & SF_WSPEC_X_MODEL)
        k.capacity = (int32_t)m.capacity, k.cap_weight = (int32_t)m.cap_weight, k.dist_weight = (int32_t)m.dist_weight, k.depot = m.depot, k.cap_level = m.cap_level,
        k.dist_level = m.dist_level;
    if (extras & SF_WSPEC_X_LA) k.la_size = q.la_size;
    if (extras & SF_WSPEC_X_LIMIT) k.limit = q.limit;
    if (extras & SF_WSPEC_X_PERM) k.has_perm = m.perm != nullptr && m.inv != nullptr;
    if (extras & SF_WSPEC_X_EXPLICIT) k.has_explicit = q.explicit_seeds != nullptr;
    return k;
}
struct WaveSpecGate {
    int32_t mode, move_budget, n_steps;
    int32_t n_replicas, resident, cus;
    int32_t knob;
};
enum {
    SF_WSPEC_AOT = 0, SF_WSPEC_SPECIALISED = 1, SF_WSPEC_FELL_BACK = 2,
    SF_WSPEC_R_NONE = 0,
    SF_WSPEC_R_KNOB = 1, SF_WSPEC_R_MODE = 2, SF_WSPEC_R_BUDGET = 3, SF_WSPEC_R_STEPS = 4, SF_WSPEC_R_RESIDENCY = 5,
    SF_WSPEC_R_NO_HIPRTC = 10, SF_WSPEC_R_NO_SOURCES = 11, SF_WSPEC_R_COMPILE = 12, SF_WSPEC_R_LOAD = 13, SF_WSPEC_R_LDS = 14,
};
constexpr int32_t SF_WSPEC_MIN_STEPS = 50;

static int32_t wave_spec_wanted(const WaveSpecGate& g) {
    if (g.knob == 0) return SF_WSPEC_R_KNOB;
    if (g.mode < 3 || g.mode > 5) return SF_WSPEC_R_MODE;
    if (g.knob == 1) return SF_WSPEC_R_NONE;
    if (g.move_budget != 0) return SF_WSPEC_R_BUDGET;
    if (g.n_steps < SF_WSPEC_MIN_STEPS) return SF_WSPEC_R_STEPS;
    if ((int64_t)g.n_replicas < (int64_t)g.resident * g.cus) return SF_WSPEC_R_RESIDENCY;
    return SF_WSPEC_R_NONE;
}
static int32_t wave_spec_knob() {
    const char* e = std::getenv("SF_AMD_WAVE_SPEC");
    return e ? (std::atoi(e) != 0 ? 1 : 0) : -1;
}

static bool wave_spec_no_sym() {
    static const bool once = std::getenv("SF_AMD_NO_WAVE_SYM") != nullptr;
    return once;
}

static std::vector<std::string> wave_spec_options(const WaveSpecKey& k, const std::string& arch, const std::string& csrc, const std::string& rocm_include) {
    auto def = [](const char* name, int32_t v) { return std::string("-D") + name + "(x)=" + std::to_string(v); };
    std::vector<std::string> o{"--offload-arch=" + arch, "-O3", "-std=c++17", "-ffp-contract=off"};
    o.push_back("-I" + csrc);
    if (!rocm_include.empty()) o.push_back("-I" + rocm_include);
    o.push_back("-DSF_SPEC_L=" + std::to_string(k.levels));
    o.push_back("-DSF_SPEC_WPE=" + std::to_string(k.wpe));
    o.push_back(def("SF_SPEC_V", k.V));
    o.push_back(def("SF_SPEC_DIM", k.dim));
    o.push_back(def("SF_SPEC_NCAP", k.n_cap));
    o.push_back(def("SF_SPEC_K0", k.k0));
    o.push_back(def("SF_SPEC_K1", k.k1));
    auto word = [](const char* name, int32_t v) { return std::string("-D") + name + "=(" + std::to_string(v) + ")"; };
    if (k.extras & SF_WSPEC_X_MODEL)
        for (auto& x : {word("SF_SPEC_MODEL_WORDS", 1), word("SF_SPEC_CAPACITY", k.capacity), word("SF_SPEC_CAP_WEIGHT", k.cap_weight), word("SF_SPEC_DIST_WEIGHT", k.dist_weight),
                        word("SF_SPEC_DEPOT", k.depot), word("SF_SPEC_CAP_LEVEL", k.cap_level), word("SF_SPEC_DIST_LEVEL", k.dist_level)})
            o.push_back(x);
    if (k.extras & SF_WSPEC_X_LA) o.push_back(def("SF_SPEC_LA_SIZE", k.la_size));
    if (k.extras & SF_WSPEC_X_LIMIT) o.push_back(def("SF_SPEC_LIMIT", k.limit));
    if (k.extras & SF_WSPEC_X_PERM) o.push_back(def("SF_SPEC_HAS_PERM", k.has_perm));
    if (k.extras & SF_WSPEC_X_EXPLICIT) o.push_back(def("SF_SPEC_HAS_EXPLICIT", k.has_explicit));
    if (k.index_x & SF_WSPEC_X_NO_WIDE) o.push_back(word("SF_SPEC_NO_WIDE", 1));
    if (k.index_x & SF_WSPEC_X_TIE_KEY)
        for (auto& x : {word("SF_SPEC_TIE_KEY", 1), word("SF_SPEC_RB", wave_spec_rb(k.V)), word("SF_SPEC_PB", wave_spec_pb(k.n_cap))}) o.push_back(x);
    if (k.index_x & SF_WSPEC_X_NO_TIES) o.push_back(word("SF_SPEC_NO_TIES", 1));
    if (k.index_x & SF_WSPEC_X_ROWS_FULL) o.push_back(word("SF_SPEC_ROWS_FULL", 1));
    if (k.index_x & SF_WSPEC_X_SYM_ROWS) o.push_back(word("SF_SPEC_SYM_ROWS", 1));
    if (k.index_x & SF_WSPEC_X_LEG_REAIM) o.push_back(word("SF_SPEC_LEG_REAIM", 1));
    if (wave_spec_no_sym()) o.push_back("-DSF_WAVE_SYM=0");
    return o;
}
static std::string wave_spec_kernel_expr(const WaveSpecKey& k) {
    return "sf::k_list_search_wave<" + std::to_string(k.levels) + ", false, 2, true, " + std::to_string(k.wpe) + ", false>";
}
static bool wave_spec_key_ok(const WaveSpecKey& k) {
    return (k.levels == 2 || k.levels == 4) && k.wpe >= 4 && k.wpe <= 6 && k.V >= 1 && k.dim >= 1 && k.n_cap >= 0 && k.k0 >= 1 && k.k1 >= 1 && (k.extras & ~SF_WSPEC_X_ALL) == 0 &&
           (!(k.extras & SF_WSPEC_X_LA) || k.la_size >= 1) && (!(k.extras & SF_WSPEC_X_LIMIT) || k.limit >= 1) &&
           (k.wide_ties | k.ties | k.rows_full | 1) == 1 && (!k.wide_ties || k.ties) &&
           (k.mat_sym | 1) == 1 &&
           (k.index_x & ~(wave_spec_index_allowed(WaveSpecIndexGate{k.V, k.dim, k.n_cap, k.wide_ties, k.ties, k.rows_full}) | wave_spec_leg_allowed(k.mat_sym))) == 0;
}

struct WaveSpecRtc {
    void* lib = nullptr;
    std::string include_dir;
    int (*create)(void**, const char*, const char*, int, const char**, const char**) = nullptr;
    int (*compile)(void*, int, const char**) = nullptr;
    int (*destroy)(void**) = nullptr;
    int (*add_name)(void*, const char*) = nullptr;
    int (*lowered)(void*, const char*, const char**) = nullptr;
    int (*code_size)(void*, size_t*) = nullptr;
    int (*code)(void*, char*) = nullptr;
    int (*log_size)(void*, size_t*) = nullptr;
    int (*log)(void*, char*) = nullptr;
    bool ok() const { return lib && create && compile && destroy && add_name && lowered && code_size && code && log_size && log; }
};
static std::string wave_spec_dirname(const std::string& p) {
    const size_t s = p.find_last_of('/');
    return s == std::string::npos ? std::string(".") : p.substr(0, s);
}
static const WaveSpecRtc& wave_spec_rtc() {
    static const WaveSpecRtc once = [] {
        WaveSpecRtc r;
        for (const char* n : {"libhiprtc.so.7", "libhiprtc.so.6", "libhiprtc.so.5", "libhiprtc.so"})
            if ((r.lib = dlopen(n, RTLD_NOW | RTLD_LOCAL))) break;
        if (!r.lib) return r;
        auto sym = [&](const char* n) { return dlsym(r.lib, n); };
        r.create = (decltype(r.create))sym("hiprtcCreateProgram");
        r.compile = (decltype(r.compile))sym("hiprtcCompileProgram");
        r.destroy = (decltype(r.destroy))sym("hiprtcDestroyProgram");
        r.add_name = (decltype(r.add_name))sym("hiprtcAddNameExpression");
        r.lowered = (decltype(r.lowered))sym("hiprtcGetLoweredName");
        r.code_size = (decltype(r.code_size))sym("hiprtcGetCodeSize");
        r.code = (decltype(r.code))sym("hiprtcGetCode");
        r.log_size = (decltype(r.log_size))sym("hiprtcGetProgramLogSize");
        r.log = (decltype(r.log))sym("hiprtcGetProgramLog");
        Dl_info di;
        if (r.create && dladdr((void*)r.create, &di) && di.dli_fname) r.include_dir = wave_spec_dirname(wave_spec_dirname(di.dli_fname)) + "/include";
        return r;
    }();
    return once;
}
static std::string wave_spec_csrc() {
    if (const char* e = std::getenv("SF_AMD_CSRC")) return e;
    Dl_info di;
    if (dladdr((void*)&wave_spec_csrc, &di) && di.dli_fname) return wave_spec_dirname(di.dli_fname) + "/csrc";
    return "csrc";
}

struct WaveSpecBuild {
    int32_t reason = SF_WSPEC_R_NONE;
    std::vector<char> code;
    std::string kernel, log;
    double ms = 0;
};
static WaveSpecBuild wave_spec_compile(const WaveSpecKey& k, const std::string& arch, const std::string& csrc) {
    WaveSpecBuild b;
    const WaveSpecRtc& rtc = wave_spec_rtc();
    if (!rtc.ok()) return b.reason = SF_WSPEC_R_NO_HIPRTC, b;
    static const char* unit = "sf_tu_list_wave_spec.hip";
    std::ifstream f(csrc + "/" + unit, std::ios::binary);
    if (!f) return b.reason = SF_WSPEC_R_NO_SOURCES, b;
    std::stringstream src;
    src << f.rdbuf();
    const std::string text = src.str();
    const auto t0 = std::chrono::steady_clock::now();
    void* prog = nullptr;
    if (rtc.create(&prog, text.c_str(), unit, 0, nullptr, nullptr) != 0 || !prog) return b.reason = SF_WSPEC_R_COMPILE, b;
    const std::string expr = wave_spec_kernel_expr(k);
    const std::vector<std::string> opts = wave_spec_options(k, arch, csrc, rtc.include_dir);
    std::vector<const char*> argv;
    for (auto& o : opts) argv.push_back(o.c_str());
    int rc = rtc.add_name(prog, expr.c_str());
    if (rc == 0) rc = rtc.compile(prog, (int)argv.size(), argv.data());
    size_t n = 0;
    if (rtc.log_size(prog, &n) == 0 && n > 1) {
        b.log.resize(n);
        if (rtc.log(prog, &b.log[0]) != 0) b.log.clear();
    }
    const char* low = nullptr;
    if (rc == 0) rc = rtc.lowered(prog, expr.c_str(), &low);
    if (rc == 0 && low) b.kernel = low;
    if (rc == 0) rc = rtc.code_size(prog, &n);
    if (rc == 0) {
        b.code.resize(n);
        rc = rtc.code(prog, b.code.data());
    }
    (void)rtc.destroy(&prog);
    b.ms = std::chrono::duration<double, std::milli>(std::chrono::steady_clock::now() - t0).count();
    if (rc != 0 || b.kernel.empty() || b.code.empty()) b.reason = SF_WSPEC_R_COMPILE, b.code.clear();
    return b;
}

struct WaveSpecEntry {
    int32_t reason = SF_WSPEC_R_NONE;
    hipModule_t module = nullptr;
    hipFunction_t fn = nullptr;
    int lds_ok = 0;
};
struct WaveSpecCache {
    std::mutex mu;
    std::map<std::string, WaveSpecEntry> entries;
    int32_t compiles = 0;
    double last_ms = 0;
};
static WaveSpecCache& wave_spec_cache() {
    static WaveSpecCache c;
    return c;
}
static int32_t wave_spec_get(const WaveSpecKey& k, int device, size_t lds, hipFunction_t* fn) {
    WaveSpecCache& c = wave_spec_cache();
    const std::string csrc = wave_spec_csrc();
    std::string id = std::to_string(device) + "|" + csrc;
    const int32_t* w = &k.levels;
    for (size_t i = 0; i < sizeof(WaveSpecKey) / 4; ++i) id += "|" + std::to_string(w[i]);
    std::lock_guard<std::mutex> lock(c.mu);
    auto it = c.entries.find(id);
    if (it == c.entries.end()) {
        WaveSpecEntry e;
        hipDeviceProp_t prop;
        if (!wave_spec_key_ok(k) || hipGetDeviceProperties(&prop, device) != hipSuccess) {
            e.reason = SF_WSPEC_R_COMPILE;
        } else {
            std::string arch = prop.gcnArchName;
            arch = arch.substr(0, arch.find(':'));
            WaveSpecBuild b = wave_spec_compile(k, arch, csrc);
            if (b.reason != SF_WSPEC_R_NO_HIPRTC && b.reason != SF_WSPEC_R_NO_SOURCES) c.compiles += 1, c.last_ms = b.ms;
            e.reason = b.reason;
            if (!e.reason && (hipModuleLoadData(&e.module, b.code.data()) != hipSuccess || hipModuleGetFunction(&e.fn, e.module, b.kernel.c_str()) != hipSuccess)) {
                (void)hipGetLastError();
                e.reason = SF_WSPEC_R_LOAD, e.fn = nullptr;
            }
        }
        it = c.entries.emplace(id, e).first;
    }
    WaveSpecEntry& e = it->second;
    if (e.reason) return e.reason;
    if ((int)lds > e.lds_ok) {
        if (hipFuncSetAttribute((const void*)e.fn, hipFuncAttributeMaxDynamicSharedMemorySize, (int)lds) == hipSuccess) e.lds_ok = (int)lds;
        else {
            (void)hipGetLastError();
            if (lds > 64 * 1024) return SF_WSPEC_R_LDS;
        }
    }
    *fn = e.fn;
    return SF_WSPEC_R_NONE;
}
```

Measured before the change: 88.15 billion.

## Add sentinel depot slots and packed demand route words to specialised wave kernel

Adds two layout options to the runtime-specialised wave kernel. The sentinel option stores a depot entry before and after each route in shared memory, so neighbour lookups in move evaluation need no boundary checks or depot substitution, and the route-rank table shrinks to 16-bit entries. The demand-word option packs each node's demand into the upper bits of its 16-bit route entry, which removes global demand loads during capacity delta evaluation. Only sentinel is on by default, gated on a zero depot diagonal and on the shared-memory slice not growing; the price is extra index arithmetic, a host-side matrix and demand scan, and a wider spec key.

```diff
diff --git a/solverforge_amd/csrc/sf_api.hip b/solverforge_amd/csrc/sf_api.hip
--- a/solverforge_amd/csrc/sf_api.hip
+++ b/solverforge_amd/csrc/sf_api.hip
@@ -118,9 +118,10 @@
     ListModel lm_wave{};
     NbrIndex nbr_wave{nullptr};
     bool wave_renumbered = false;
+    RouteWordFacts route_word{0, 0, 0};
     int32_t mat16_sym = 0;
     int last_wave_mode = -1;
-    int32_t wave_spec_state = 0, wave_spec_reason = 0, wave_spec_key[23] = {};
+    int32_t wave_spec_state = 0, wave_spec_reason = 0, wave_spec_key[27] = {};
     int n_cus = 0;
     int32_t last_generic_flags = -1;
     int32_t last_scalar_value_bytes = 0;
@@ -980,11 +981,20 @@
             }
         }
     ctx->mat16_sym = 0;
+    ctx->route_word = RouteWordFacts{0, 0, 0};
     if (m.mat16 && (size_t)m.dim * m.dim * 2 <= ((size_t)64 << 20)) {
         std::vector<uint16_t> h16((size_t)m.dim * m.dim);
         HIPCHK(ctx, hipMemcpyAsync(h16.data(), m.mat16, h16.size() * 2, hipMemcpyDeviceToHost, ctx->stream));
         HIPCHK(ctx, hipStreamSynchronize(ctx->stream));
         ctx->mat16_sym = mat16_symmetric(h16.data(), m.dim);
+        std::vector<int32_t> hdem;
+        for (auto& kv : ctx->facts)
+            if (m.demand && kv.second.type == 2 && kv.second.d0 == (void*)m.demand && kv.second.rows >= m.dim) {
+                hdem.resize((size_t)m.dim);
+                HIPCHK(ctx, hipMemcpyAsync(hdem.data(), m.demand, hdem.size() * 4, hipMemcpyDeviceToHost, ctx->stream));
+                HIPCHK(ctx, hipStreamSynchronize(ctx->stream));
+            }
+        ctx->route_word = route_word_facts(h16.data(), m.dim, m.depot, hdem.empty() ? nullptr : hdem.data(), (int32_t)hdem.size());
     }
     for (auto& kv : ctx->facts)
         if (kv.second.type == 1 && kv.second.d0 == (void*)m.mat) {
@@ -1234,7 +1244,7 @@
     }
     if (!ctx->n_cus) HIPCHK(ctx, hipDeviceGetAttribute(&ctx->n_cus, hipDeviceAttributeMultiprocessorCount, ctx->device));
     const WaveSpecGate gate{pl.mode, q.move_budget != 0, (int32_t)std::min<int64_t>(std::max<int64_t>(q.n_steps, 0), INT32_MAX), n_replicas, pl.resident, ctx->n_cus, wave_spec_knob()};
-    const WaveSpecKey key = wave_spec_key(pl.levels, pl.wpe, *la.lm, q, ctx->nbr_facts, ctx->mat16_sym, wave_spec_extras());
+    const WaveSpecKey key = wave_spec_key(pl.levels, pl.wpe, *la.lm, q, ctx->nbr_facts, ctx->mat16_sym, ctx->route_word, wave_spec_extras());
     ctx->wave_spec_state = SF_WSPEC_AOT, ctx->wave_spec_reason = wave_spec_wanted(gate);
     std::memcpy(ctx->wave_spec_key, &key, sizeof key);
     if (ctx->wave_spec_reason == SF_WSPEC_R_NONE) {
@@ -2317,6 +2327,27 @@
     out[0] = k.mat_sym, out[1] = k.index_x & SF_WSPEC_X_LEG_ALL;
     return SF_OK;
 }
+extern "C" int32_t sf_debug_wave_spec_layout(const sf_ctx* ctx, int32_t* out, int32_t n_out) {
+    if (!ctx || !out || n_out != 4) return SF_ERR_INVALID;
+    WaveSpecKey k;
+    std::memcpy(&k, ctx->wave_spec_key, sizeof k);
+    out[0] = k.depot_diag0, out[1] = k.id_bits, out[2] = k.dem_bits, out[3] = k.layout_x;
+    return SF_OK;
+}
+extern "C" int32_t sf_debug_route_word_facts(const int64_t* mat, int32_t dim, int32_t depot, const int32_t* demand, int32_t n_demand, int32_t* out, int32_t n_out) {
+    if (!mat || !out || dim < 1 || dim > 16384 || n_out != 3 || n_demand < 0) return SF_ERR_INVALID;
+    std::vector<uint16_t> w((size_t)dim * dim);
+    for (size_t t = 0; t < w.size(); ++t) w[t] = mat16_word(mat[t]);
+    const RouteWordFacts f = route_word_facts(w.data(), dim, depot, demand, n_demand);
+    out[0] = f.depot_diag0, out[1] = f.id_bits, out[2] = f.dem_bits;
+    return SF_OK;
+}
+extern "C" int32_t sf_debug_wave_spec_layout_gate(const int32_t* in, int32_t n_in, int32_t* slices) {
+    if (!in || n_in != 8 || in[0] < 1 || in[1] < 1 || in[2] < 0 || in[3] < 1 || in[4] < 1) return SF_ERR_INVALID;
+    const int32_t max_k = in[3] > in[4] ? in[3] : in[4];
+    if (slices) slices[0] = (int32_t)wave_spec_sentinel_slice(in[0], in[2], in[1], max_k), slices[1] = (int32_t)wave_spec_planned_slice(in[0], in[2], in[1], max_k);
+    return wave_spec_layout_allowed(WaveSpecLayoutGate{in[0], in[1], in[2], in[3], in[4], in[5], in[6], in[7]});
+}
 extern "C" int32_t sf_debug_mat_sym(const int64_t* mat, int32_t dim, int32_t* out, int32_t n_out) {
     if (!mat || !out || dim < 1 || dim > 16384 || n_out != 1) return SF_ERR_INVALID;
     std::vector<uint16_t> w((size_t)dim * dim);
@@ -2351,7 +2382,7 @@
     return wave_spec_index_allowed(WaveSpecIndexGate{in[0], in[1], in[2], in[3] >= 64, in[3] >= 2, in[4] != 0});
 }
 extern "C" int32_t sf_debug_wave_spec_compile(const int32_t* key, int32_t n_key, const char* arch, const char* out_path, char* opts, int32_t n_opts, char* log, int32_t n_log, double* ms) {
-    if (!key || (n_key * 4 != (int)sizeof(WaveSpecKey) && n_key != SF_WSPEC_KEY_WORDS_V2 && n_key != SF_WSPEC_KEY_WORDS_V1) || !arch) return SF_ERR_INVALID;
+    if (!key || (n_key * 4 != (int)sizeof(WaveSpecKey) && n_key != SF_WSPEC_KEY_WORDS_V3 && n_key != SF_WSPEC_KEY_WORDS_V2 && n_key != SF_WSPEC_KEY_WORDS_V1) || !arch) return SF_ERR_INVALID;
     WaveSpecKey k{};
     std::memcpy(&k, key, (size_t)n_key * 4);
     if (!wave_spec_key_ok(k)) return SF_ERR_INVALID;
diff --git a/solverforge_amd/csrc/sf_list_wave.hip b/solverforge_amd/csrc/sf_list_wave.hip
--- a/solverforge_amd/csrc/sf_list_wave.hip
+++ b/solverforge_amd/csrc/sf_list_wave.hip
@@ -66,6 +66,21 @@
 #else
 #define SF_SPEC_ROW_HAVE(x) (x)
 #define SF_SPEC_ROW_HAVEMASK(x) (x)
+#endif
+#ifdef SF_SPEC_SENTINEL
+constexpr bool SF_SENTINEL = true;
+#define SF_SPEC_SLOT0(o, r) ((o) + (r) + 1u)
+#else
+constexpr bool SF_SENTINEL = false;
+#define SF_SPEC_SLOT0(o, r) (o)
+#endif
+#ifdef SF_SPEC_DEMAND_WORD
+static_assert(SF_SPEC_DEMAND_WORD >= 1 && SF_SPEC_DEMAND_WORD <= 15, "SF_SPEC_DEMAND_WORD: node bits of a 16-bit route entry");
+constexpr uint32_t SF_ROUTE_NODE_MASK = (1u << SF_SPEC_DEMAND_WORD) - 1u;
+#define SF_SPEC_NODE(w) ((w) & SF_ROUTE_NODE_MASK)
+#else
+constexpr uint32_t SF_ROUTE_NODE_MASK = 0xFFFFFFFFu;
+#define SF_SPEC_NODE(w) (w)
 #endif
 
 
@@ -119,7 +134,7 @@
 struct WCarve {
     size_t load, off, node, ring, visits, rtab, routeat, total;
     uint32_t rc;
-    __host__ __device__ WCarve(int V, int n_cap, int dim, int max_k, bool compact = false, bool node_global = false) {
+    __host__ __device__ WCarve(int V, int n_cap, int dim, int max_k, bool compact = false, bool node_global = false, bool sentinel = false) {
         rc = max_k <= 32 ? RC_SMALL : RC_MAX;
         size_t o = 0;
         load = o;
@@ -131,9 +146,9 @@
         ring = o;
         o = align_up(o + sizeof(uint32_t) * 2 * rc * MAX_LEAVES, 16);
         visits = o;
-        o = align_up(o + sizeof(uint16_t) * n_cap, 16);
+        o = align_up(o + sizeof(uint16_t) * (n_cap + (sentinel ? V + 2 : 0)), 16);
         rtab = o;
-        o = align_up(o + (node_global ? 0 : sizeof(uint32_t) * V * MAX_LEAVES), 16);
+        o = align_up(o + (node_global ? 0 : (sentinel ? sizeof(uint16_t) : sizeof(uint32_t)) * V * MAX_LEAVES), 16);
         routeat = o;
         o = align_up(o + (compact ? 0 : sizeof(uint16_t) * V * MAX_LEAVES), 16);
         total = o;
@@ -181,7 +196,7 @@
         if (__ballot(!none && pos == pmax) != 0ull) {
             if (!none && pos == pmax) {
                 const uint32_t o = off_at(route), len = off_at(route + 1) - o;
-                while (pos + 1 < len && (uint32_t)visits[o + pos] != node) ++pos;
+                while (pos + 1 < len && SF_SPEC_NODE((uint32_t)visits[SF_SPEC_SLOT0(o, route) + pos]) != node) ++pos;
             }
         }
         return none ? NODE_NONE : ((route << 16) | pos);
@@ -256,13 +271,15 @@
     __device__ __forceinline__ static uint32_t rank(uint32_t w) { return w; }
     __device__ __forceinline__ static uint32_t inter_ord(uint32_t w, uint32_t dp) { return ORD_ARITH_BASE + (w << ORD_ARITH_SHIFT) + dp; }
 };
-struct RouteRank {
-    const uint32_t* rt;
+template <class W>
+struct RouteRankT {
+    const W* rt;
     static constexpr int KEY_SHIFT = RouteArith::KEY_SHIFT;
     __device__ __forceinline__ uint32_t word(uint32_t route) const { return rt[route]; }
     __device__ __forceinline__ static uint32_t rank(uint32_t w) { return w; }
     __device__ __forceinline__ static uint32_t inter_ord(uint32_t w, uint32_t dp) { return RouteArith::inter_ord(w, dp); }
 };
+using RouteRank = RouteRankT<uint32_t>;
 template <class OT, class RT>
 __device__ __forceinline__ NearbyItem nearby_item_rt(bool is_change, uint32_t slot, uint32_t se, uint32_t sp,
                                                      uint32_t len, uint32_t k, const OT* s_off, const RT& rt) {
@@ -312,14 +329,14 @@
 }
 #endif
 
-template <class LT, class OT, bool OWN_LANE = false>
+template <class LT, class OT, bool OWN_LANE = false, bool SENT = false, uint32_t NMASK = 0xFFFFFFFFu>
 __device__ __forceinline__ void apply_list_move_wave(const ListModel& m, uint16_t* visits, OT* off,
                                                      LT* load, int kind, uint32_t a, uint32_t i, uint32_t b,
                                                      uint32_t j, uint32_t ext = 0) {
     uint32_t lane = threadIdx.x & 63u;
     if constexpr (OWN_LANE) asm volatile("" : "+v"(lane));
     if (kind == 2) {
-        const uint32_t P = off[a] + i, Q = off[b] + j;
+        const uint32_t P = off[a] + i + (SENT ? a + 1u : 0u), Q = off[b] + j + (SENT ? b + 1u : 0u);
         const uint32_t x = visits[P];
         wave_sync();
         if (P < Q) {
@@ -349,7 +366,7 @@
                 if (a > b && rr > b && rr <= a) off[rr] += 1;
             }
             if (lane == 0 && m.demand) {
-                const int64_t dx = (int64_t)m.demand[x];
+                const int64_t dx = (int64_t)m.demand[x & NMASK];
                 load[a] = (LT)wsub(load[a], dx);
                 load[b] = (LT)wadd(load[b], dx);
             }
@@ -431,12 +448,12 @@
         }
     } else if (kind == 3) {
         if (lane == 0) {
-            const uint32_t pa = off[a] + i, pb = off[b] + j;
+            const uint32_t pa = off[a] + i + (SENT ? a + 1u : 0u), pb = off[b] + j + (SENT ? b + 1u : 0u);
             const uint16_t x = visits[pa], y = visits[pb];
             visits[pa] = y;
             visits[pb] = x;
             if (a != b && m.demand) {
-                const int64_t dx = (int64_t)m.demand[x], dy = (int64_t)m.demand[y];
+                const int64_t dx = (int64_t)m.demand[x & NMASK], dy = (int64_t)m.demand[y & NMASK];
                 load[a] = (LT)wadd(wsub(load[a], dx), dy);
                 load[b] = (LT)wadd(wsub(load[b], dy), dx);
             }
@@ -710,6 +727,13 @@
 template <int L, class LT, bool M16 = false, class OT = uint32_t, bool KW = false>
 __device__ __forceinline__ void eval_generated_small(const ListModel& m, const LevelWords<L>& lw, const uint16_t* visits, const OT* off, const LT* load, uint32_t c,
                                                      uint32_t a, uint32_t i, uint32_t b, uint32_t j, int32_t (&dv)[L]) {
+#ifdef SF_SPEC_SENTINEL
+    const uint32_t P = off[a] + a + 1u + i, Q = off[b] + b + 1u + j;
+    const uint32_t xw = visits[P], vqw = visits[Q];
+    const uint32_t x = SF_SPEC_NODE(xw), vq = SF_SPEC_NODE(vqw);
+    const uint32_t pa = SF_SPEC_NODE((uint32_t)visits[P - 1u]), na = SF_SPEC_NODE((uint32_t)visits[P + 1u]);
+    const uint32_t pb = SF_SPEC_NODE((uint32_t)visits[Q - 1u]), nb = SF_SPEC_NODE((uint32_t)visits[Q + 1u]);
+#else
     const uint32_t oa = off[a], la = off[a + 1] - oa;
     const uint32_t ob = off[b], lb = off[b + 1] - ob;
     const uint32_t depot = KW ? lw.depot : (uint32_t)m.depot;
@@ -717,12 +741,15 @@
     const uint32_t h_pa = min(i, 1u), h_na = min(la - 1u - i, 1u);
     const uint32_t h_q = min(lb - j, 1u), h_pb = min(j, 1u);
     const uint32_t h_nb = min(max(lb, j + 1u) - (j + 1u), 1u);
-    const uint32_t x = visits[P];
+    [[maybe_unused]] const uint32_t xw = visits[P];
+    const uint32_t x = SF_SPEC_NODE(xw);
     const uint32_t r_pa = visits[P - h_pa], r_na = visits[P + h_na];
     const uint32_t r_q = visits[Q - (1u - h_q)], r_pb = visits[Q - h_pb], r_nb = visits[Q + h_nb];
-    const uint32_t pa = h_pa ? r_pa : depot, na = h_na ? r_na : depot;
-    const uint32_t vq = h_q ? r_q : depot;
-    const uint32_t pb = h_pb ? r_pb : depot, nb = h_nb ? r_nb : depot;
+    [[maybe_unused]] const uint32_t vqw = r_q;
+    const uint32_t pa = SF_SPEC_NODE(h_pa ? r_pa : depot), na = SF_SPEC_NODE(h_na ? r_na : depot);
+    const uint32_t vq = SF_SPEC_NODE(h_q ? r_q : depot);
+    const uint32_t pb = SF_SPEC_NODE(h_pb ? r_pb : depot), nb = SF_SPEC_NODE(h_nb ? r_nb : depot);
+#endif
     const bool chg = c != 0;
     const bool intra = a == b;
     const bool adj = !chg && intra && j == i + 1;
@@ -760,11 +787,16 @@
     const uint32_t m2 = leg(adj ? vq : pb, adj ? nb : vq);
     int32_t d_cap = 0;
     if (lw.has_cap != 0u) {
+#ifdef SF_SPEC_DEMAND_WORD
+        const int32_t dx = (int32_t)(xw >> SF_SPEC_DEMAND_WORD);
+        const int32_t dyq = (int32_t)(vqw >> SF_SPEC_DEMAND_WORD);
+#else
         const int32_t dx = m.demand[x];
 #ifdef SF_SPEC_LEG_REAIM
         const int32_t dyq = m.demand[(chg || intra) ? x : vq];
 #else
         const int32_t dyq = m.demand[vq];
+#endif
 #endif
         const int32_t dy = chg ? 0 : dyq;
         const int32_t cap = KW ? lw.cap : (int32_t)m.capacity;
@@ -773,8 +805,13 @@
         d_cap = max(la0 - sh, 0) + max(lb0 + sh, 0) - max(la0, 0) - max(lb0, 0);
         d_cap = intra ? 0 : d_cap;
     }
+#ifdef SF_SPEC_SENTINEL
+    const uint32_t plus = p0 + p1 + p2 + (ca ? 0u : p3);
+    const uint32_t minus = m0 + m1 + m2 + (ca ? 0u : m3);
+#else
     const uint32_t plus = ((chg && la == 1) ? 0u : p0) + p1 + p2 + (ca ? 0u : p3);
     const uint32_t minus = m0 + m1 + ((chg && !intra && lb == 0) ? 0u : m2) + (ca ? 0u : m3);
+#endif
     const int32_t d_dist = (int32_t)(plus - minus);
     const int32_t tc = -((KW ? lw.cw : (int32_t)m.cap_weight) * d_cap), td = -((KW ? lw.dw : (int32_t)m.dist_weight) * d_dist);
 #pragma unroll
@@ -844,7 +881,8 @@
     auto desc0 = [&]() -> uint64_t { return SMALL ? (uint64_t)(int64_t)desc0_w : desc0_q; };
     auto desc1 = [&]() -> uint64_t { return SMALL ? (uint64_t)(int64_t)desc1_w : desc1_q; };
 
-    const WCarve cv(V, SF_SPEC_NCAP(m.n_cap), (int)dim, (int)(K0 > K1 ? K0 : K1), COMPACT, NODEG);
+    static_assert(!(SF_SENTINEL || SF_ROUTE_NODE_MASK != 0xFFFFFFFFu) || (LEAN && COMPACT && !NODEG && !TRACE), "SF_SPEC_SENTINEL / SF_SPEC_DEMAND_WORD: the COMPACT FAST + SMALL kernel only");
+    const WCarve cv(V, SF_SPEC_NCAP(m.n_cap), (int)dim, (int)(K0 > K1 ? K0 : K1), COMPACT, NODEG, SF_SENTINEL);
     const uint32_t RCM = cv.rc - 1;
     unsigned char* mem = smem + (size_t)wave_in_group * cv.total;
     LT* s_load = (LT*)(mem + cv.load);
@@ -862,8 +900,9 @@
         }
     };
     constexpr bool ARANK = NODEG;
-    using RT = typename std::conditional<ARANK, RouteArith, typename std::conditional<RANKTAB, RouteRank, RouteTab>::type>::type;
-    uint32_t* rtab = (uint32_t*)(mem + cv.rtab);
+    using RTW = typename std::conditional<RANKTAB && SF_SENTINEL, uint16_t, uint32_t>::type;
+    using RT = typename std::conditional<ARANK, RouteArith, typename std::conditional<RANKTAB, RouteRankT<RTW>, RouteTab>::type>::type;
+    RTW* rtab = (RTW*)(mem + cv.rtab);
     uint16_t* route_at = (uint16_t*)(mem + cv.routeat);
 
     uint32_t* g_visits = m.visits + (size_t)r * SF_SPEC_NCAP(m.n_cap);
@@ -877,15 +916,39 @@
     for (uint32_t t = lane; t < dim; t += 64) node_slot.clear(t);
     node_sync();
     const uint32_t total0 = uni(s_off[V]);
+#if defined(SF_SPEC_SENTINEL) || defined(SF_SPEC_DEMAND_WORD)
+    {
+        auto route_word = [&](uint32_t node) -> uint32_t {
+#ifdef SF_SPEC_DEMAND_WORD
+            return node | ((uint32_t)m.demand[node] << SF_SPEC_DEMAND_WORD);
+#else
+            return node;
+#endif
+        };
+        auto int_id = [&](uint32_t g) -> uint32_t { return (COMPACT && SF_SPEC_HAS_PERM(m.perm != nullptr)) ? (uint32_t)m.perm[g] : g; };
+#ifdef SF_SPEC_SENTINEL
+        const uint32_t depot_word = route_word((uint32_t)m.depot);
+        for (uint32_t t = lane; t < (uint32_t)SF_SPEC_NCAP(m.n_cap) + (uint32_t)V + 2u; t += 64) s_visits[t] = (uint16_t)depot_word;
+        wave_sync();
+        for (uint32_t v = lane; v < (uint32_t)V; v += 64) {
+            const uint32_t o = s_off[v], len = s_off[v + 1] - o;
+            for (uint32_t q = 0; q < len; ++q) s_visits[SF_SPEC_SLOT0(o, v) + q] = (uint16_t)route_word(int_id(g_visits[o + q]));
+        }
+#else
+        for (uint32_t t = lane; t < total0; t += 64) s_visits[t] = (uint16_t)route_word(int_id(g_visits[t]));
+#endif
+    }
+#else
     if (COMPACT && SF_SPEC_HAS_PERM(m.perm != nullptr)) {
         for (uint32_t t = lane; t < total0; t += 64) s_visits[t] = m.perm[g_visits[t]];
     } else {
         for (uint32_t t = lane; t < total0; t += 64) s_visits[t] = (uint16_t)g_visits[t];
     }
+#endif
     wave_sync();
     for (uint32_t v = lane; v < (uint32_t)V; v += 64) {
         const uint32_t o = s_off[v], len = s_off[v + 1] - o;
-        for (uint32_t q = 0; q < len; ++q) node_slot.set(s_visits[o + q], v, q);
+        for (uint32_t q = 0; q < len; ++q) node_slot.set(SF_SPEC_NODE((uint32_t)s_visits[SF_SPEC_SLOT0(o, v) + q]), v, q);
     }
     node_sync();
 
@@ -898,6 +961,14 @@
         }
     }
     auto ext_id = [&](uint32_t x) -> uint32_t { return (COMPACT && SF_SPEC_HAS_PERM(m.inv != nullptr)) ? (uint32_t)m.inv[x] : x; };
+#ifdef SF_SPEC_SENTINEL
+    auto lists_out = [&](uint32_t* dst, uint32_t ln) {
+        for (uint32_t v = ln; v < (uint32_t)V; v += 64) {
+            const uint32_t o = s_off[v], len = s_off[v + 1] - o;
+            for (uint32_t q = 0; q < len; ++q) dst[o + q] = ext_id(SF_SPEC_NODE((uint32_t)s_visits[SF_SPEC_SLOT0(o, v) + q]));
+        }
+    };
+#endif
     int64_t cur[L], best_sol[L];
 #pragma unroll
     for (int k = 0; k < L; ++k) {
@@ -1068,7 +1139,7 @@
                                           (uint64_t)se ^ (l ? desc1() : desc0());
                 const uint32_t oo = (o & ~63u) + lane;
                 const uint32_t spl = oo < len ? ctx.selection_index(oo, len, src_salt) : 0u;
-                const uint32_t sxl = oo < len ? (uint32_t)s_visits[s_off[se] + spl] : 0u;
+                const uint32_t sxl = oo < len ? SF_SPEC_NODE((uint32_t)s_visits[SF_SPEC_SLOT0(s_off[se], se) + spl]) : 0u;
                 c.pv = spl | (sxl << 16);
                 c.vk = k;
                 c.vbase = o & ~63u;
@@ -1133,12 +1204,12 @@
                 continue;
             }
             uint16_t* ra = route_at + l * V;
-            uint32_t* rt = rtab + l * V;
+            RTW* rt = rtab + l * V;
             [[maybe_unused]] uint32_t carry = 0;
             for (uint32_t base = 0; base < (uint32_t)V; base += 64) {
                 const uint32_t k = base + lane;
                 if constexpr (RANKTAB) {
-                    if (k < (uint32_t)V) rt[perm_index_recip(pst, psd, k, (uint32_t)V, v_recip32)] = k;
+                    if (k < (uint32_t)V) rt[perm_index_recip(pst, psd, k, (uint32_t)V, v_recip32)] = (RTW)k;
                 } else {
                     uint32_t v = 0, e = 0;
                     if (k < (uint32_t)V) {
@@ -1584,7 +1655,11 @@
                     uint32_t* const bo = SF_COLD_M(best_off) + (size_t)r * (V + 1);
                     uint32_t ln = lane;
                     if constexpr (RANKTAB) asm volatile("" : "+v"(ln));
-                    for (uint32_t t = ln; t < tot; t += 64) bv[t] = ext_id(s_visits[t]);
+#ifdef SF_SPEC_SENTINEL
+                    lists_out(bv, ln);
+#else
+                    for (uint32_t t = ln; t < tot; t += 64) bv[t] = ext_id(SF_SPEC_NODE((uint32_t)s_visits[t]));
+#endif
                     for (uint32_t t = ln; t <= (uint32_t)V; t += 64) bo[t] = s_off[t];
                     best_pending = false;
                 }
@@ -1618,15 +1693,15 @@
                     else
                         tabu_sig_list_swap(tabu_scope, a, i, u, b, j, ext_id(s_visits[s_off[b] + j]), pick_sig);
                 }
-            apply_list_move_wave<LT, OT, RANKTAB && L == 4>(m, s_visits, s_off, s_load, kind, a, i, b, j);
+            apply_list_move_wave<LT, OT, RANKTAB && L == 4, SF_SENTINEL, SF_ROUTE_NODE_MASK>(m, s_visits, s_off, s_load, kind, a, i, b, j);
             {
                 const uint32_t oa = s_off[a], la = s_off[a + 1] - oa;
                 const uint32_t ob = s_off[b], lb = s_off[b + 1] - ob;
                 for (uint32_t t = lane; t < la + (a != b ? lb : 0u); t += 64) {
                     if (t < la)
-                        node_slot.set(s_visits[oa + t], a, t);
+                        node_slot.set(SF_SPEC_NODE((uint32_t)s_visits[SF_SPEC_SLOT0(oa, a) + t]), a, t);
                     else
-                        node_slot.set(s_visits[ob + (t - la)], b, t - la);
+                        node_slot.set(SF_SPEC_NODE((uint32_t)s_visits[SF_SPEC_SLOT0(ob, b) + (t - la)]), b, t - la);
                 }
             }
             node_sync();
@@ -1711,10 +1786,18 @@
         if (best_pending) {
             uint32_t* const bv = SF_COLD_M(best_visits) + (size_t)r * n_cap;
             uint32_t* const bo = SF_COLD_M(best_off) + (size_t)r * (V + 1);
-            for (uint32_t t = wlane; t < tot; t += 64) bv[t] = ext_id(s_visits[t]);
+#ifdef SF_SPEC_SENTINEL
+            lists_out(bv, wlane);
+#else
+            for (uint32_t t = wlane; t < tot; t += 64) bv[t] = ext_id(SF_SPEC_NODE((uint32_t)s_visits[t]));
+#endif
             for (uint32_t t = wlane; t <= (uint32_t)V; t += 64) bo[t] = s_off[t];
         }
-        for (uint32_t t = wlane; t < tot; t += 64) w_visits[t] = ext_id(s_visits[t]);
+#ifdef SF_SPEC_SENTINEL
+        lists_out(w_visits, wlane);
+#else
+        for (uint32_t t = wlane; t < tot; t += 64) w_visits[t] = ext_id(SF_SPEC_NODE((uint32_t)s_visits[t]));
+#endif
         for (uint32_t t = wlane; t <= (uint32_t)V; t += 64) w_off[t] = s_off[t];
         for (uint32_t t = wlane; t < (uint32_t)V; t += 64) w_load[t] = (int64_t)s_load[t];
         if (lane == 0) {
diff --git a/solverforge_amd/csrc/sf_mat_facts.h b/solverforge_amd/csrc/sf_mat_facts.h
--- a/solverforge_amd/csrc/sf_mat_facts.h
+++ b/solverforge_amd/csrc/sf_mat_facts.h
@@ -14,3 +14,27 @@
         }
     return 1;
 }
+
+struct RouteWordFacts {
+    int32_t depot_diag0, id_bits, dem_bits;
+};
+static inline int32_t route_word_bits(uint32_t v) {
+    int32_t b = 1;
+    while (b < 32 && (v >> b)) ++b;
+    return b;
+}
+static inline RouteWordFacts route_word_facts(const uint16_t* mat, int32_t dim, int32_t depot, const int32_t* demand, int32_t n_demand) {
+    RouteWordFacts f{0, 0, 0};
+    if (dim < 1) return f;
+    f.id_bits = route_word_bits((uint32_t)(dim - 1));
+    f.depot_diag0 = (mat && depot >= 0 && depot < dim && mat[(size_t)depot * dim + depot] == 0) ? 1 : 0;
+    if (demand && n_demand >= dim) {
+        int32_t mx = 0;
+        for (int32_t t = 0; t < dim; ++t) {
+            if (demand[t] < 0) return f;
+            mx = demand[t] > mx ? demand[t] : mx;
+        }
+        f.dem_bits = route_word_bits((uint32_t)mx);
+    }
+    return f;
+}
diff --git a/solverforge_amd/csrc/sf_wave_spec.h b/solverforge_amd/csrc/sf_wave_spec.h
--- a/solverforge_amd/csrc/sf_wave_spec.h
+++ b/solverforge_amd/csrc/sf_wave_spec.h
@@ -1,6 +1,7 @@
 #pragma once
 #include <dlfcn.h>
 
+#include "sf_mat_facts.h"
 #include "sf_nbr_facts.h"
 
 #include <fstream>
@@ -16,18 +17,24 @@
     int32_t wide_ties, ties, rows_full;
     int32_t index_x;
     int32_t mat_sym;
-};
+    int32_t depot_diag0, id_bits, dem_bits;
+    int32_t layout_x;
+};
+constexpr int32_t SF_WSPEC_KEY_WORDS_V3 = 23;
 constexpr int32_t SF_WSPEC_KEY_WORDS_V2 = 22;
 constexpr int32_t SF_WSPEC_KEY_WORDS_V1 = 18;
 enum { SF_WSPEC_X_MODEL = 1, SF_WSPEC_X_LA = 2, SF_WSPEC_X_LIMIT = 4, SF_WSPEC_X_PERM = 8, SF_WSPEC_X_EXPLICIT = 16, SF_WSPEC_X_ALL = 31 };
 enum { SF_WSPEC_X_NO_WIDE = 32, SF_WSPEC_X_TIE_KEY = 64, SF_WSPEC_X_NO_TIES = 128, SF_WSPEC_X_ROWS_FULL = 256, SF_WSPEC_X_INDEX_ALL = 480 };
 enum { SF_WSPEC_X_SYM_ROWS = 512, SF_WSPEC_X_LEG_REAIM = 1024, SF_WSPEC_X_LEG_ALL = 1536 };
+enum { SF_WSPEC_X_SENTINEL = 2048, SF_WSPEC_X_DEMAND_WORD = 4096, SF_WSPEC_X_LAYOUT_ALL = 6144 };
 constexpr int32_t SF_WSPEC_X_DEFAULT = SF_WSPEC_X_MODEL | SF_WSPEC_X_LA | SF_WSPEC_X_PERM;
 constexpr int32_t SF_WSPEC_X_INDEX_DEFAULT = SF_WSPEC_X_NO_WIDE | SF_WSPEC_X_TIE_KEY | SF_WSPEC_X_ROWS_FULL;
 constexpr int32_t SF_WSPEC_X_LEG_DEFAULT = SF_WSPEC_X_SYM_ROWS;
+constexpr int32_t SF_WSPEC_X_LAYOUT_DEFAULT = SF_WSPEC_X_SENTINEL;
 static int32_t wave_spec_extras() {
     const char* e = std::getenv("SF_AMD_WAVE_SPEC_EXTRAS");
-    return e ? (std::atoi(e) & (SF_WSPEC_X_ALL | SF_WSPEC_X_INDEX_ALL | SF_WSPEC_X_LEG_ALL)) : (SF_WSPEC_X_DEFAULT | SF_WSPEC_X_INDEX_DEFAULT | SF_WSPEC_X_LEG_DEFAULT);
+    return e ? (std::atoi(e) & (SF_WSPEC_X_ALL | SF_WSPEC_X_INDEX_ALL | SF_WSPEC_X_LEG_ALL | SF_WSPEC_X_LAYOUT_ALL))
+             : (SF_WSPEC_X_DEFAULT | SF_WSPEC_X_INDEX_DEFAULT | SF_WSPEC_X_LEG_DEFAULT | SF_WSPEC_X_LAYOUT_DEFAULT);
 }
 
 struct WaveSpecIndexGate {
@@ -50,14 +57,31 @@
     return a;
 }
 static int32_t wave_spec_leg_allowed(int32_t mat_sym) { return SF_WSPEC_X_LEG_REAIM | (mat_sym ? SF_WSPEC_X_SYM_ROWS : 0); }
+struct WaveSpecLayoutGate {
+    int32_t V, dim, n_cap, k0, k1;
+    int32_t depot_diag0, id_bits, dem_bits;
+};
+static size_t wave_spec_sentinel_slice(int32_t V, int32_t n_cap, int32_t dim, int32_t max_k) { return WCarve(V, n_cap, dim, max_k, true, false, true).total; }
+static size_t wave_spec_planned_slice(int32_t V, int32_t n_cap, int32_t dim, int32_t max_k) { return WCarve(V, n_cap, dim, max_k, true, false).total; }
+static int32_t wave_spec_layout_allowed(const WaveSpecLayoutGate& g) {
+    int32_t a = 0;
+    const int32_t max_k = g.k0 > g.k1 ? g.k0 : g.k1;
+    if (g.depot_diag0 == 1 && g.V >= 1 && g.V + 1 <= 65536 && g.n_cap >= 0 && (int64_t)g.n_cap + g.V + 2 <= 65536 &&
+        wave_spec_sentinel_slice(g.V, g.n_cap, g.dim, max_k) <= wave_spec_planned_slice(g.V, g.n_cap, g.dim, max_k))
+        a |= SF_WSPEC_X_SENTINEL;
+    if (g.id_bits >= 1 && g.dem_bits >= 1 && g.dim >= 1 && g.id_bits == route_word_bits((uint32_t)(g.dim - 1)) && g.id_bits + g.dem_bits <= 16) a |= SF_WSPEC_X_DEMAND_WORD;
+    return a;
+}
 template <class Model, class Params>
-static WaveSpecKey wave_spec_key(int32_t levels, int32_t wpe, const Model& m, const Params& q, const NbrFacts& nf, int32_t mat_sym, int32_t extras) {
+static WaveSpecKey wave_spec_key(int32_t levels, int32_t wpe, const Model& m, const Params& q, const NbrFacts& nf, int32_t mat_sym, const RouteWordFacts& rw, int32_t extras) {
     WaveSpecKey k{};
     k.levels = levels, k.wpe = wpe, k.V = m.V, k.dim = m.dim, k.n_cap = m.n_cap, k.k0 = q.leaf[0].max_nearby, k.k1 = q.leaf[1].max_nearby;
     k.wide_ties = nf.tie_max >= 64, k.ties = nf.tie_max >= 2, k.rows_full = nf.rows_full != 0;
     k.index_x = extras & SF_WSPEC_X_INDEX_ALL & wave_spec_index_allowed(WaveSpecIndexGate{k.V, k.dim, k.n_cap, k.wide_ties, k.ties, k.rows_full});
     k.mat_sym = mat_sym != 0;
     k.index_x |= extras & SF_WSPEC_X_LEG_ALL & wave_spec_leg_allowed(k.mat_sym);
+    k.depot_diag0 = rw.depot_diag0 != 0, k.id_bits = rw.id_bits, k.dem_bits = rw.dem_bits;
+    k.layout_x = extras & SF_WSPEC_X_LAYOUT_ALL & wave_spec_layout_allowed(WaveSpecLayoutGate{k.V, k.dim, k.n_cap, k.k0, k.k1, k.depot_diag0, k.id_bits, k.dem_bits});
     extras &= SF_WSPEC_X_ALL;
     auto fits = [](int64_t v) { return v >= INT32_MIN && v <= INT32_MAX; };
     if ((extras & SF_WSPEC_X_MODEL) && !(fits(m.capacity) && fits(m.cap_weight) && fits(m.dist_weight))) extras &= ~SF_WSPEC_X_MODEL;
@@ -132,6 +156,8 @@
     if (k.index_x & SF_WSPEC_X_ROWS_FULL) o.push_back(word("SF_SPEC_ROWS_FULL", 1));
     if (k.index_x & SF_WSPEC_X_SYM_ROWS) o.push_back(word("SF_SPEC_SYM_ROWS", 1));
     if (k.index_x & SF_WSPEC_X_LEG_REAIM) o.push_back(word("SF_SPEC_LEG_REAIM", 1));
+    if (k.layout_x & SF_WSPEC_X_SENTINEL) o.push_back(word("SF_SPEC_SENTINEL", 1));
+    if (k.layout_x & SF_WSPEC_X_DEMAND_WORD) o.push_back(word("SF_SPEC_DEMAND_WORD", k.id_bits));
     if (wave_spec_no_sym()) o.push_back("-DSF_WAVE_SYM=0");
     return o;
 }
@@ -143,7 +169,9 @@
            (!(k.extras & SF_WSPEC_X_LA) || k.la_size >= 1) && (!(k.extras & SF_WSPEC_X_LIMIT) || k.limit >= 1) &&
            (k.wide_ties | k.ties | k.rows_full | 1) == 1 && (!k.wide_ties || k.ties) &&
            (k.mat_sym | 1) == 1 &&
-           (k.index_x & ~(wave_spec_index_allowed(WaveSpecIndexGate{k.V, k.dim, k.n_cap, k.wide_ties, k.ties, k.rows_full}) | wave_spec_leg_allowed(k.mat_sym))) == 0;
+           (k.index_x & ~(wave_spec_index_allowed(WaveSpecIndexGate{k.V, k.dim, k.n_cap, k.wide_ties, k.ties, k.rows_full}) | wave_spec_leg_allowed(k.mat_sym))) == 0 &&
+           (k.depot_diag0 | 1) == 1 && k.id_bits >= 0 && k.id_bits <= 32 && k.dem_bits >= 0 && k.dem_bits <= 32 &&
+           (k.layout_x & ~wave_spec_layout_allowed(WaveSpecLayoutGate{k.V, k.dim, k.n_cap, k.k0, k.k1, k.depot_diag0, k.id_bits, k.dem_bits})) == 0;
 }
 
 struct WaveSpecRtc {
```

New measurement: 89.00 billion (median of 6 runs). Within noise of the previous version (+1.0%).
